# iden3/snarkjs

Hardware: NVIDIA B200
Metric: groth16_proofs_per_sec (higher is better)
Workload: dtype u32x8 (256-bit modular integers, 32-bit limbs)

## Files before the change

profiles/tune_pair.py:

```python
import os, sys
sys.path.insert(0, os.path.dirname(os.path.dirname(os.path.abspath(__file__))))
import numpy as np
import snarkjs_b200
from snarkjs_b200 import synth
c = snarkjs_b200.getCurveFromName("bn128")
lib, h = c.lib, c.handle
n = 1 << 20
rng = np.random.default_rng(1)
sc = rng.integers(0, 256, size=n * 32, dtype=np.uint8); sc.reshape(n, 32)[:, 31] &= 0x1f
for grp in (1, 2):
    bases = synth.gen_points(c, grp, 7, n)
    G = c.G1 if grp == 1 else c.G2
    hb = G.registerBases(bases)
    ref = None
    for off, rounds in ((1, 0), (0, 1), (0, 2), (0, 3), (0, 4), (0, 6)):
        lib.sb_set_tuning(4, off); lib.sb_set_tuning(5, rounds)
        for _ in range(3):
            out = G.multiExpRegistered(hb, sc)
        if ref is None: ref = out.tobytes()
        assert out.tobytes() == ref
        print(f"G{grp} pairing {'off' if off else 'R<=%d' % rounds}: pre-stage {lib.sb_last_stat(h, grp - 1):.3f} ms, msm device total {c.last_ms(2):.3f} ms")
```

snarkjs_b200/csrc/api.cu:

```cuda
#include <cstdio>
#include <cstdlib>
#include <cstring>
#include <string>
#include <vector>
#include <map>
#include <algorithm>
#include <mutex>
#include <future>
#include <thread>
#include <dlfcn.h>
#include <nccl.h>
#include <fcntl.h>
#include <unistd.h>
#include <sys/mman.h>
#include <sys/stat.h>
#include "../../include/snarkb200.h"
#include "ec.cuh"
#include "msm.cuh"
#include "msm_entry.h"
#include "fr_entry.h"

using namespace sb;
namespace sb { double calibrate(int what, cudaStream_t stream); extern int g_ntt_tile_log; }

namespace {

struct DevBuf {
    void* p = nullptr; size_t cap = 0;
    void* get(size_t bytes) {
        if (bytes > cap) { if (p) cudaFree(p); p = nullptr; cap = 0; if (cudaMalloc(&p, bytes ? bytes : 16) != cudaSuccess) return nullptr; cap = bytes; }
        return p;
    }
    void release() { if (p) cudaFree(p); p = nullptr; cap = 0; }
};

struct GroupOps {
    int (*buckets)(const void*, const MsmSorted&, MsmScratch&, cudaStream_t, void*, MsmLaunchStats*, cudaStream_t, cudaEvent_t);
    void (*combine)(const uint8_t*, const MsmGeom&, uint8_t*);
    void (*add)(uint8_t*, const uint8_t*);
    void (*to_jacobian)(const uint8_t*, uint8_t*);
    void (*to_affine)(const uint8_t*, uint8_t*);
    void (*from_affine)(const uint8_t*, uint8_t*);
    void (*times)(const uint8_t*, const uint8_t*, int, uint8_t*);
    int (*gen_points)(const uint8_t*, uint64_t, uint64_t, void*, cudaStream_t);
    int (*precompute)(const void*, uint64_t, int, int, void*, cudaStream_t);
    uint32_t xyzz_bytes;
    uint32_t aff_bytes;
};
#define SB_GROUP_OPS(NAME, AFF) GroupOps{NAME##_buckets, NAME##_combine, NAME##_add, NAME##_to_jacobian, NAME##_to_affine, NAME##_from_affine, NAME##_times, NAME##_gen_points, NAME##_precompute, NAME##_xyzz_bytes(), AFF}

struct NttTab { DevBuf lo, hi; int h = 0; };
struct PreTab { DevBuf lo, hi; int h = 0; std::string key; };

struct BaseSet { int group = 0; uint64_t n = 0; void* d = nullptr; void* table = nullptr; MsmGeom gp{}; };

struct Groth16Key {
    uint32_t nVars = 0, nPublic = 0, domainSize = 0; int power = 0;
    std::vector<uint8_t> alpha1, beta1, beta2, gamma2, delta1, delta2;
    void *dA = nullptr, *dB1 = nullptr, *dB2 = nullptr, *dC = nullptr, *dH = nullptr;
    void *tA = nullptr, *tB1 = nullptr, *tB2 = nullptr, *tC = nullptr, *tH = nullptr;
    MsmGeom gpW{}, gpH{};
    int shard = 0, n_shards = 1; uint64_t wlo = 0, wcnt = 0, hlo = 0, hcnt = 0;
    uint64_t* d_rowptr = nullptr; uint32_t* d_sig = nullptr; void* d_coef = nullptr; uint64_t nCoef = 0;
    bool witness_resident = false;
    void *dW = nullptr, *dA_T = nullptr, *dB_T = nullptr, *dC_T = nullptr, *dTmp = nullptr, *dTmp2 = nullptr, *dTmp3 = nullptr, *dWsum = nullptr;
};

}

namespace { struct PlonkKeyDev; void plonk_free_key(PlonkKeyDev*); }
namespace { struct FflonkKeyDev; void fflonk_free_key(FflonkKeyDev*); }

static constexpr size_t STAGE_BYTES = 8u << 20;

struct sb_ctx {
    std::recursive_mutex mu;
    int curve = 0, device = 0;
    cudaStream_t stream = nullptr;
    std::string err;
    uint32_t n8q = 32;
    GroupOps g1, g2;
    MsmScratch sort_scratch, bucket_scratch;
    MsmScratch sort_scratch2, bscr[5];
    cudaStream_t aux[6] = {nullptr, nullptr, nullptr, nullptr, nullptr, nullptr};
    cudaEvent_t pev[16];
    uint8_t* pinned = nullptr;
    uint8_t* stage[2] = {nullptr, nullptr};
    cudaEvent_t stage_ev[2];
    MsmLaunchStats stats;
    uint64_t launches = 0;
    DevBuf io[4];
    std::map<int, NttTab> ntt_fwd, ntt_inv;
    DevBuf wr_fwd, wr_inv;
    std::map<int, DevBuf> ninv;
    std::vector<PreTab*> pre_cache;
    std::vector<BaseSet> bases;
    std::vector<Groth16Key*> keys;
    std::vector<PlonkKeyDev*> plonk_keys;
    std::vector<FflonkKeyDev*> fflonk_keys;
    cudaEvent_t ev[8];
    float last_ms[8] = {0};
    int fr_s = 0, fr_bits = 254;
    std::vector<std::vector<uint8_t>> roots;
    std::vector<uint8_t> nqr, shift;
    std::vector<uint8_t> gen1, gen2;
    cudaEvent_t prof_ev[256];
    double stat[16] = {0};
    ncclComm_t comm = nullptr; int rank = 0, world = 1;
    void* d_xchg = nullptr; uint8_t* h_xchg = nullptr;
};

namespace {

thread_local const sb_ctx* t_err_ctx = nullptr;
thread_local std::string t_err;
int fail(sb_ctx* c, int code, const std::string& msg) { if (c) { c->err = msg; t_err_ctx = c; t_err = msg; } return code; }
#define SB_LOCK(c) std::unique_lock<std::recursive_mutex> _sb_lk; if (c) _sb_lk = std::unique_lock<std::recursive_mutex>((c)->mu)
int cuda_fail(sb_ctx* c, cudaError_t e, const char* where) {
    return fail(c, e == cudaErrorMemoryAllocation ? SB_ERR_NOMEM : SB_ERR_CUDA, std::string(where) + ": " + cudaGetErrorString(e));
}
#define CU(c, call) do { cudaError_t _e = (call); if (_e != cudaSuccess) return cuda_fail(c, _e, #call); } while (0)

int g_stage_enabled = 1;
bool host_is_pinned(const void* p) {
    cudaPointerAttributes a;
    if (cudaPointerGetAttributes(&a, p) != cudaSuccess) { cudaGetLastError(); return false; }
    return a.type == cudaMemoryTypeHost;
}
cudaError_t h2d(sb_ctx* c, void* dst, const void* src, size_t bytes) {
    if (!bytes) return cudaSuccess;
    if (!g_stage_enabled || bytes < (1u << 20) || !c->stage[0] || !c->stage[1] || host_is_pinned(src))
        return cudaMemcpyAsync(dst, src, bytes, cudaMemcpyHostToDevice, c->stream);
    size_t off = 0; int k = 0; cudaError_t e = cudaSuccess;
    while (off < bytes && e == cudaSuccess) {
        const int b = k & 1; const size_t n = std::min(STAGE_BYTES, bytes - off);
        if (k >= 2) e = cudaEventSynchronize(c->stage_ev[b]);
        if (e != cudaSuccess) break;
        memcpy(c->stage[b], (const uint8_t*)src + off, n);
        e = cudaMemcpyAsync((uint8_t*)dst + off, c->stage[b], n, cudaMemcpyHostToDevice, c->stream);
        if (e == cudaSuccess) e = cudaEventRecord(c->stage_ev[b], c->stream);
        off += n; k++;
    }
    if (e == cudaSuccess) e = cudaEventSynchronize(c->stage_ev[0]);
    if (e == cudaSuccess && k > 1) e = cudaEventSynchronize(c->stage_ev[1]);
    return e;
}
cudaError_t d2h(sb_ctx* c, void* dst, const void* src, size_t bytes) {
    if (!bytes) return cudaSuccess;
    if (!g_stage_enabled || bytes < (1u << 20) || !c->stage[0] || !c->stage[1] || host_is_pinned(dst)) {
        cudaError_t e = cudaMemcpyAsync(dst, src, bytes, cudaMemcpyDeviceToHost, c->stream);
        return e == cudaSuccess ? cudaStreamSynchronize(c->stream) : e;
    }
    size_t off = 0, prev_off = 0, prev_n = 0; int k = 0; cudaError_t e = cudaSuccess;
    while (off < bytes && e == cudaSuccess) {
        const int b = k & 1; const size_t n = std::min(STAGE_BYTES, bytes - off);
        e = cudaMemcpyAsync(c->stage[b], (const uint8_t*)src + off, n, cudaMemcpyDeviceToHost, c->stream);
        if (e == cudaSuccess) e = cudaEventRecord(c->stage_ev[b], c->stream);
        if (e == cudaSuccess && k >= 1) { e = cudaEventSynchronize(c->stage_ev[b ^ 1]); if (e == cudaSuccess) memcpy((uint8_t*)dst + prev_off, c->stage[b ^ 1], prev_n); }
        prev_off = off; prev_n = n; off += n; k++;
    }
    if (e == cudaSuccess && k >= 1) { const int b = (k - 1) & 1; e = cudaEventSynchronize(c->stage_ev[b]); if (e == cudaSuccess) memcpy((uint8_t*)dst + prev_off, c->stage[b], prev_n); }
    return e;
}

template <class P> struct HostFr {
    typedef Fp<P> F;
    static F from_u32(uint32_t x) { F a = F::zero(); a.v[0] = x; return F::to_mont(a); }
    static void roots(int& s, std::vector<F>& w, F& nqr, F& shift) {
        const int N = P::N;
        uint32_t pm1[N]; for (int i = 0; i < N; i++) pm1[i] = P::p(i); pm1[0] -= 1;
        uint32_t half[N]; for (int i = 0; i < N; i++) half[i] = (pm1[i] >> 1) | (i + 1 < N ? pm1[i + 1] << 31 : 0);
        F negone = F::neg(F::one());
        nqr = from_u32(2);
        while (!(F::pow(nqr, half, N) == negone)) nqr = F::add(nqr, F::one());
        shift = F::sqr(nqr);
        uint32_t t[N]; memcpy(t, pm1, sizeof t); s = 0;
        while (!(t[0] & 1)) { for (int i = 0; i < N; i++) t[i] = (t[i] >> 1) | (i + 1 < N ? t[i + 1] << 31 : 0); s++; }
        w.assign(s + 1, F::zero());
        w[s] = F::pow(nqr, t, N);
        for (int i = s - 1; i >= 0; i--) w[i] = F::sqr(w[i + 1]);
    }
    static void pow_tables(const F& base, const F& scale, int h, uint64_t nhi, std::vector<F>& lo, std::vector<F>& hi) {
        lo.resize((size_t)1 << h); hi.resize(nhi ? nhi : 1);
        F t = F::one();
        for (size_t e = 0; e < lo.size(); e++) { lo[e] = t; t = F::mul(t, base); }
        F step = t;
        t = scale;
        for (size_t e = 0; e < hi.size(); e++) { hi[e] = t; t = F::mul(t, step); }
    }
};

template <class P> int init_roots(sb_ctx* c) {
    typedef Fp<P> F;
    std::vector<F> w; F nqr, shift; int s;
    HostFr<P>::roots(s, w, nqr, shift);
    c->fr_s = s;
    c->roots.resize(s + 1);
    for (int i = 0; i <= s; i++) c->roots[i].assign((uint8_t*)&w[i], (uint8_t*)&w[i] + 32);
    c->nqr.assign((uint8_t*)&nqr, (uint8_t*)&nqr + 32);
    c->shift.assign((uint8_t*)&shift, (uint8_t*)&shift + 32);
    F wd = w[NTT_DMAX], wdi = F::inv(wd);
    std::vector<F> lo, hi;
    HostFr<P>::pow_tables(wd, F::one(), NTT_DMAX - 1, 1, lo, hi);
    if (!c->wr_fwd.get(lo.size() * 32)) return SB_ERR_NOMEM;
    cudaMemcpy(c->wr_fwd.p, lo.data(), lo.size() * 32, cudaMemcpyHostToDevice);
    HostFr<P>::pow_tables(wdi, F::one(), NTT_DMAX - 1, 1, lo, hi);
    if (!c->wr_inv.get(lo.size() * 32)) return SB_ERR_NOMEM;
    cudaMemcpy(c->wr_inv.p, lo.data(), lo.size() * 32, cudaMemcpyHostToDevice);
    return 0;
}

template <class P> int build_ntt_tab(sb_ctx* c, int L, bool inverse, NttTab& tab) {
    typedef Fp<P> F;
    F w; memcpy(&w, c->roots[L].data(), 32);
    if (inverse) w = F::inv(w);
    int h = (L + 1) / 2;
    std::vector<F> lo, hi;
    HostFr<P>::pow_tables(w, F::one(), h, (uint64_t)1 << (L - h), lo, hi);
    tab.h = h;
    if (!tab.lo.get(lo.size() * 32) || !tab.hi.get(hi.size() * 32)) return SB_ERR_NOMEM;
    cudaMemcpy(tab.lo.p, lo.data(), lo.size() * 32, cudaMemcpyHostToDevice);
    cudaMemcpy(tab.hi.p, hi.data(), hi.size() * 32, cudaMemcpyHostToDevice);
    return 0;
}

int get_ntt_tab(sb_ctx* c, int L, bool inverse, FrNttTables* out) {
    auto& m = inverse ? c->ntt_inv : c->ntt_fwd;
    auto it = m.find(L);
    if (it == m.end()) {
        NttTab& t = m[L];
        int rc = c->curve == SB_BN254 ? build_ntt_tab<BnFr>(c, L, inverse, t) : build_ntt_tab<BlsFr>(c, L, inverse, t);
        if (rc) { m.erase(L); return fail(c, rc, "ntt table allocation failed"); }
        it = m.find(L);
    }
    out->tw_lo = it->second.lo.p; out->tw_hi = it->second.hi.p; out->h = it->second.h;
    out->wr = inverse ? c->wr_inv.p : c->wr_fwd.p;
    return 0;
}

template <class P> void ninv_bytes(int L, uint8_t* out) {
    typedef Fp<P> F;
    F two = F::add(F::one(), F::one()), n = F::one();
    for (int i = 0; i < L; i++) n = F::mul(n, two);
    F r = F::inv(n); memcpy(out, &r, 32);
}
const void* get_ninv(sb_ctx* c, int L) {
    auto it = c->ninv.find(L);
    if (it == c->ninv.end()) {
        uint8_t b[32];
        if (c->curve == SB_BN254) ninv_bytes<BnFr>(L, b); else ninv_bytes<BlsFr>(L, b);
        DevBuf& d = c->ninv[L];
        if (!d.get(32)) return nullptr;
        cudaMemcpy(d.p, b, 32, cudaMemcpyHostToDevice);
        it = c->ninv.find(L);
    }
    return it->second.p;
}

template <class P> int build_pre(sb_ctx* c, uint64_t n, const uint8_t* first, const uint8_t* inc, PreTab& t) {
    typedef Fp<P> F;
    int bits = 0; while (((uint64_t)1 << bits) < n) bits++;
    int h = (bits + 1) / 2;
    F f, i; memcpy(&f, first, 32); memcpy(&i, inc, 32);
    std::vector<F> lo, hi;
    HostFr<P>::pow_tables(i, f, h, (n + ((uint64_t)1 << h) - 1) >> h, lo, hi);
    t.h = h;
    if (!t.lo.get(lo.size() * 32) || !t.hi.get(hi.size() * 32)) return SB_ERR_NOMEM;
    cudaMemcpy(t.lo.p, lo.data(), lo.size() * 32, cudaMemcpyHostToDevice);
    cudaMemcpy(t.hi.p, hi.data(), hi.size() * 32, cudaMemcpyHostToDevice);
    return 0;
}
int get_pre(sb_ctx* c, uint64_t n, const uint8_t* first, const uint8_t* inc, FrPre* out) {
    std::string key((const char*)&n, 8); key.append((const char*)first, 32); key.append((const char*)inc, 32);
    for (PreTab* t : c->pre_cache) if (t->key == key) { out->lo = t->lo.p; out->hi = t->hi.p; out->h = t->h; return 0; }
    PreTab* t = new PreTab(); t->key = key;
    int rc = c->curve == SB_BN254 ? build_pre<BnFr>(c, n, first, inc, *t) : build_pre<BlsFr>(c, n, first, inc, *t);
    if (rc) { delete t; return fail(c, rc, "apply-key table allocation failed"); }
    if (c->pre_cache.size() >= 16) { delete c->pre_cache.front(); c->pre_cache.erase(c->pre_cache.begin()); }
    c->pre_cache.push_back(t);
    out->lo = t->lo.p; out->hi = t->hi.p; out->h = t->h;
    return 0;
}

template <class P> void hex_to_mont(const char* hex, uint8_t* out) {
    typedef Fp<P> F; F a = F::zero();
    int len = (int)strlen(hex);
    for (int i = 0; i < len; i++) {
        char ch = hex[len - 1 - i];
        uint32_t d = (ch >= '0' && ch <= '9') ? ch - '0' : (ch >= 'a' && ch <= 'f') ? ch - 'a' + 10 : ch - 'A' + 10;
        a.v[i / 8] |= d << (4 * (i % 8));
    }
    a = F::to_mont(a); memcpy(out, &a, sizeof a);
}
void init_generators(sb_ctx* c) {
    if (c->curve == SB_BN254) {
        c->gen1.resize(64); c->gen2.resize(128);
        hex_to_mont<BnFq>("1", c->gen1.data()); hex_to_mont<BnFq>("2", c->gen1.data() + 32);
        hex_to_mont<BnFq>("1800deef121f1e76426a00665e5c4479674322d4f75edadd46debd5cd992f6ed", c->gen2.data());
        hex_to_mont<BnFq>("198e9393920d483a7260bfb731fb5d25f1aa493335a9e71297e485b7aef312c2", c->gen2.data() + 32);
        hex_to_mont<BnFq>("12c85ea5db8c6deb4aab71808dcb408fe3d1e7690c43d37b4ce6cc0166fa7daa", c->gen2.data() + 64);
        hex_to_mont<BnFq>("090689d0585ff075ec9e99ad690c3395bc4b313370b38ef355acdadcd122975b", c->gen2.data() + 96);
    } else {
        c->gen1.resize(96); c->gen2.resize(192);
        hex_to_mont<BlsFq>("17f1d3a73197d7942695638c4fa9ac0fc3688c4f9774b905a14e3a3f171bac586c55e83ff97a1aeffb3af00adb22c6bb", c->gen1.data());
        hex_to_mont<BlsFq>("08b3f481e3aaa0f1a09e30ed741d8ae4fcf5e095d5d00af600db18cb2c04b3edd03cc744a2888ae40caa232946c5e7e1", c->gen1.data() + 48);
        hex_to_mont<BlsFq>("024aa2b2f08f0a91260805272dc51051c6e47ad4fa403b02b4510b647ae3d1770bac0326a805bbefd48056c8c121bdb8", c->gen2.data());
        hex_to_mont<BlsFq>("13e02b6052719f607dacd3a088274f65596bd0d09920b61ab5da61bbdc7f5049334cf11213945d57e5ac7d055d042b7e", c->gen2.data() + 48);
        hex_to_mont<BlsFq>("0ce5d527727d6e118cc9cdc6da2e351aadfd9baa8cbdd3a76d429a695160d12c923ac9cc3baca289e193548608b82801", c->gen2.data() + 96);
        hex_to_mont<BlsFq>("0606c4a02ea734cc32acd2b02bc28b99cb3e287e85a763af267492ab572e99ab3f370d275cec1da1aaa9075ff05f79be", c->gen2.data() + 144);
    }
}

void prof_begin(sb_ctx* c) { c->stats.ev = c->prof_ev; c->stats.nev = 256; c->stats.used = 0; for (double& d : c->stat) d = 0; }
void prof_end(sb_ctx* c) {
    for (int i = 0; i + 1 < c->stats.used; i += 2) {
        float ms = 0; if (cudaEventElapsedTime(&ms, c->prof_ev[i], c->prof_ev[i + 1]) != cudaSuccess) { cudaGetLastError(); continue; }
        const int g = c->stats.tag[i / 2];
        if (g == PROF_ACC_G1) { c->stat[0] += ms; c->stat[2] += 1; c->stat[9] += ms; }
        else if (g == PROF_ACC_G2) { c->stat[1] += ms; c->stat[3] += 1; c->stat[10] += ms; }
        else if (g == PROF_SORT) c->stat[8] += ms;
        else if (g >= PROF_FOLD && g <= PROF_JOIN) c->stat[11 + (g - PROF_FOLD)] += ms;
    }
    c->stats.ev = nullptr; c->stats.used = 0;
}

bool want_precomp(sb_ctx* c, uint64_t n) {
    if (g_msm_tuning[3] != 0 || n < (1ull << 12)) return false;
    MsmGeom g = msm_geometry_precomp(n, 32, c->fr_bits);
    return (uint64_t)g.W * n < (1ull << 31);
}
int build_table(sb_ctx* c, const GroupOps& G, const void* d_bases, uint64_t n, void** table, MsmGeom* gp) {
    MsmGeom g = msm_geometry_precomp(n, 32, c->fr_bits);
    cudaError_t e = cudaMalloc(table, (size_t)g.W * n * G.aff_bytes);
    if (e != cudaSuccess) { *table = nullptr; return cuda_fail(c, e, "precompute table allocation"); }
    int rc = G.precompute(d_bases, n, g.c, g.W, *table, c->stream); c->launches++;
    if (rc) return cuda_fail(c, (cudaError_t)rc, "k_precompute");
    e = cudaStreamSynchronize(c->stream);
    if (e != cudaSuccess) return cuda_fail(c, e, "k_precompute");
    *gp = g;
    return 0;
}

void tick(sb_ctx* c, int i) { cudaEventRecord(c->ev[i], c->stream); }
float elapsed(sb_ctx* c, int a, int b) { float ms = 0; cudaEventElapsedTime(&ms, c->ev[a], c->ev[b]); return ms; }

int msm_dev_accumulate(sb_ctx* c, const GroupOps& G, const void* d_bases, const uint8_t* d_scalars, uint32_t sbytes, uint64_t n,
                       uint8_t* acc_xyzz, const MsmGeom* gp = nullptr, uint64_t first = 0) {
    const uint64_t MAXC = 1ull << (g_msm_tuning[6] > 0 ? g_msm_tuning[6] : 23);
    for (uint64_t off = 0; off < n; off += MAXC) {
        uint64_t cn = std::min(MAXC, n - off);
        MsmGeom g = msm_geometry(cn, sbytes, c->fr_bits);
        if (gp) {
            g = *gp; g.first = first + off; g.W = (int)((8 * sbytes + 1 + g.c - 1) / g.c);
        }
        MsmSorted s;
        int rc = msm_sort_entries(d_scalars + off * sbytes, sbytes, cn, g, c->sort_scratch, c->stream, &s, &c->stats);
        if (rc) return cuda_fail(c, (cudaError_t)rc, "msm_sort_entries");
        void* d_wsum = c->io[3].get((size_t)g.wsum_points() * G.xyzz_bytes);
        if (!d_wsum) return fail(c, SB_ERR_NOMEM, "out of device memory");
        c->stats.cur_tag = (&G == &c->g1) ? SB_G1 : SB_G2;
        rc = G.buckets(gp ? d_bases : (const void*)((const uint8_t*)d_bases + off * G.aff_bytes), s, c->bucket_scratch, c->stream, d_wsum, &c->stats, nullptr, nullptr);
        if (rc) return cuda_fail(c, (cudaError_t)rc, "msm_buckets");
        std::vector<uint8_t> ws((size_t)g.wsum_points() * G.xyzz_bytes);
        uint64_t entries = 0;
        CU(c, cudaMemcpyAsync(ws.data(), d_wsum, ws.size(), cudaMemcpyDeviceToHost, c->stream));
        CU(c, cudaMemcpyAsync(&entries, s.counts, 8, cudaMemcpyDeviceToHost, c->stream));
        CU(c, cudaStreamSynchronize(c->stream));
        c->stat[(&G == &c->g1) ? 4 : 5] += (double)entries;
        G.combine(ws.data(), g, acc_xyzz);
    }
    return 0;
}

int msm_host_inputs(sb_ctx* c, int group, const uint8_t* bases, const void* d_bases_opt, const uint8_t* scalars, uint32_t sbytes,
                    uint64_t n, uint8_t* out_jac, uint8_t* out_partial, const MsmGeom* gp = nullptr, uint64_t first = 0) {
    if (!c) return SB_ERR_ARG;
    const GroupOps& G = group == SB_G1 ? c->g1 : c->g2;
    std::vector<uint8_t> acc(G.xyzz_bytes, 0);
    if (n) {
        if (sbytes == 0 || sbytes > 64) return fail(c, SB_ERR_ARG, "Scalar size does not match");
        cudaSetDevice(c->device);
        tick(c, 0);
        const void* d_bases = d_bases_opt;
        if (!d_bases) {
            void* p = c->io[0].get(n * G.aff_bytes);
            if (!p) return fail(c, SB_ERR_NOMEM, "out of device memory");
            CU(c, h2d(c, p, bases, n * G.aff_bytes));
            d_bases = p;
        }
        uint8_t* d_sc = (uint8_t*)c->io[1].get(n * sbytes);
        if (!d_sc) return fail(c, SB_ERR_NOMEM, "out of device memory");
        CU(c, h2d(c, d_sc, scalars, n * sbytes));
        tick(c, 1);
        prof_begin(c);
        int rc = msm_dev_accumulate(c, G, d_bases, d_sc, sbytes, n, acc.data(), gp, first);
        if (rc) return rc;
        tick(c, 2);
        cudaEventSynchronize(c->ev[2]);
        prof_end(c);
        c->last_ms[0] = elapsed(c, 0, 2); c->last_ms[1] = elapsed(c, 0, 1); c->last_ms[2] = elapsed(c, 1, 2);
    }
    if (out_partial) memcpy(out_partial, acc.data(), acc.size());
    if (out_jac) G.to_jacobian(acc.data(), out_jac);
    return 0;
}

struct Section { uint64_t pos = 0, len = 0; bool present = false; };
int parse_binfile(sb_ctx* c, const uint8_t* d, uint64_t len, const char* magic, uint32_t max_version, std::map<uint32_t, Section>& secs) {
    if (len < 12 || memcmp(d, magic, 4) != 0) return fail(c, SB_ERR_FORMAT, std::string(magic) + ": Invalid File format");
    uint32_t ver, nsec; memcpy(&ver, d + 4, 4); memcpy(&nsec, d + 8, 4);
    if (ver > max_version) return fail(c, SB_ERR_FORMAT, "Version not supported");
    uint64_t pos = 12;
    for (uint32_t i = 0; i < nsec; i++) {
        if (len - pos < 12) return fail(c, SB_ERR_FORMAT, "Invalid file size");
        uint32_t id; uint64_t sl; memcpy(&id, d + pos, 4); memcpy(&sl, d + pos + 4, 8); pos += 12;
        if (sl > len - pos) return fail(c, SB_ERR_FORMAT, "Invalid file size");
        if (secs[id].present) return fail(c, SB_ERR_FORMAT, "Section Duplicated " + std::to_string(id));
        secs[id].pos = pos; secs[id].len = sl; secs[id].present = true;
        pos += sl;
    }
    if (pos != len) return fail(c, SB_ERR_FORMAT, "Invalid file size");
    return 0;
}

bool modulus_matches(const uint8_t* p, uint32_t n8, int curve, bool scalar_field) {
    uint32_t limbs[12] = {0};
    if (curve == SB_BN254) { if (n8 != 32) return false; for (int i = 0; i < 8; i++) limbs[i] = scalar_field ? BnFr::p(i) : BnFq::p(i); }
    else if (scalar_field) { if (n8 != 32) return false; for (int i = 0; i < 8; i++) limbs[i] = BlsFr::p(i); }
    else { if (n8 != 48) return false; for (int i = 0; i < 12; i++) limbs[i] = BlsFq::p(i); }
    return memcmp(p, limbs, n8) == 0;
}

void free_key(Groth16Key* k) {
    for (void* p : {k->tA, k->tB1, k->tB2, k->tC, k->tH, k->dA, k->dB1, k->dB2, k->dC, k->dH, (void*)k->d_rowptr, (void*)k->d_sig, k->d_coef, k->dW, k->dA_T, k->dB_T, k->dC_T, k->dTmp, k->dTmp2, k->dTmp3, k->dWsum})
        if (p) cudaFree(p);
    delete k;
}

template <class PR> static void fr_from_mont_bytes(const uint8_t* in, uint8_t* out) { Fp<PR> a; memcpy(&a, in, 32); a = Fp<PR>::from_mont(a); memcpy(out, &a, 32); }
template <class PR> static void fr_neg_mul_bytes(const uint8_t* r, const uint8_t* s, uint8_t* out) { Fp<PR> a, b; memcpy(&a, r, 32); memcpy(&b, s, 32); a = Fp<PR>::neg(Fp<PR>::mul(a, b)); memcpy(out, &a, 32); }

}

extern "C" {

const char* sb_version(void) { return "snarkb200 0.2 (sm_100a)"; }
int sb_comm_destroy(sb_ctx* c);

int sb_create(int curve, int device_id, sb_ctx** out) {
    if (!out || (curve != SB_BN254 && curve != SB_BLS12_381)) return SB_ERR_ARG;
    int ndev = 0;
    if (cudaGetDeviceCount(&ndev) != cudaSuccess || ndev == 0) return SB_ERR_NODEVICE;
    if (device_id < 0 || device_id >= ndev) return SB_ERR_ARG;
    if (cudaSetDevice(device_id) != cudaSuccess) return SB_ERR_CUDA;
    sb_ctx* c = new sb_ctx();
    c->curve = curve; c->device = device_id;
    c->n8q = curve == SB_BN254 ? 32 : 48;
    c->fr_bits = curve == SB_BN254 ? 254 : 255;
    if (curve == SB_BN254) { c->g1 = SB_GROUP_OPS(bn254_g1, 64); c->g2 = SB_GROUP_OPS(bn254_g2, 128); }
    else { c->g1 = SB_GROUP_OPS(bls12381_g1, 96); c->g2 = SB_GROUP_OPS(bls12381_g2, 192); }
    if (cudaStreamCreate(&c->stream) != cudaSuccess) { delete c; return SB_ERR_CUDA; }
    for (auto& e : c->ev) cudaEventCreate(&e);
    for (auto& e : c->prof_ev) cudaEventCreate(&e);
    for (auto& e : c->pev) cudaEventCreateWithFlags(&e, cudaEventDisableTiming);
    { int lo = 0, hi = 0; cudaDeviceGetStreamPriorityRange(&lo, &hi);
      for (auto& st : c->aux) cudaStreamCreateWithPriority(&st, cudaStreamDefault, hi); }
    if (cudaHostAlloc((void**)&c->pinned, 256 * 1024, cudaHostAllocDefault) != cudaSuccess) c->pinned = nullptr;
    for (int i = 0; i < 2; i++) { if (cudaHostAlloc((void**)&c->stage[i], STAGE_BYTES, cudaHostAllocDefault) != cudaSuccess) c->stage[i] = nullptr; cudaEventCreateWithFlags(&c->stage_ev[i], cudaEventDisableTiming); }
    init_generators(c);
    int rc = curve == SB_BN254 ? init_roots<BnFr>(c) : init_roots<BlsFr>(c);
    if (rc == 0 && fr_configure(curve) != 0) rc = SB_ERR_CUDA;
    if (rc) { sb_destroy(c); return rc; }
    *out = c;
    return SB_OK;
}

void sb_destroy(sb_ctx* c) {
    if (!c) return;
    sb_comm_destroy(c);
    cudaSetDevice(c->device);
    cudaStreamSynchronize(c->stream);
    for (auto* k : c->keys) if (k) free_key(k);
    for (auto* k : c->plonk_keys) if (k) plonk_free_key(k);
    for (auto* k : c->fflonk_keys) if (k) fflonk_free_key(k);
    for (auto& b : c->bases) { if (b.d) cudaFree(b.d); if (b.table) cudaFree(b.table); }
    for (auto* t : c->pre_cache) { t->lo.release(); t->hi.release(); delete t; }
    for (auto& kv : c->ntt_fwd) { kv.second.lo.release(); kv.second.hi.release(); }
    for (auto& kv : c->ntt_inv) { kv.second.lo.release(); kv.second.hi.release(); }
    for (auto& kv : c->ninv) kv.second.release();
    c->wr_fwd.release(); c->wr_inv.release();
    for (auto& b : c->io) b.release();
    c->sort_scratch.release(); c->bucket_scratch.release();
    for (auto& e : c->ev) cudaEventDestroy(e);
    for (auto& e : c->prof_ev) cudaEventDestroy(e);
    for (auto& e : c->pev) cudaEventDestroy(e);
    for (auto& st : c->aux) { if (st) { cudaStreamSynchronize(st); cudaStreamDestroy(st); } }
    if (c->pinned) cudaFreeHost(c->pinned);
    for (int i = 0; i < 2; i++) { if (c->stage[i]) cudaFreeHost(c->stage[i]); cudaEventDestroy(c->stage_ev[i]); }
    c->sort_scratch2.release(); for (auto& b : c->bscr) b.release();
    cudaStreamDestroy(c->stream);
    delete c;
}

const char* sb_last_error(sb_ctx* c) {
    if (!c) return "null context";
    if (t_err_ctx == c) return t_err.c_str();
    SB_LOCK(c); t_err_ctx = c; t_err = c->err; return t_err.c_str();
}
uint64_t sb_launch_count(sb_ctx* c) { SB_LOCK(c); return c ? c->launches + (uint64_t)c->stats.launches : 0; }
float sb_last_ms(sb_ctx* c, int which) { SB_LOCK(c); return (c && which >= 0 && which < 8) ? c->last_ms[which] : 0.f; }
int sb_sync(sb_ctx* c) { SB_LOCK(c); if (!c) return SB_ERR_ARG; cudaSetDevice(c->device); CU(c, cudaStreamSynchronize(c->stream)); return 0; }

int sb_msm_g1_affine(sb_ctx* c, const uint8_t* bases, const uint8_t* scalars, uint32_t sb, uint64_t n, uint8_t* out) { SB_LOCK(c);
    return msm_host_inputs(c, SB_G1, bases, nullptr, scalars, sb, n, out, nullptr);
}
int sb_msm_g2_affine(sb_ctx* c, const uint8_t* bases, const uint8_t* scalars, uint32_t sb, uint64_t n, uint8_t* out) { SB_LOCK(c);
    return msm_host_inputs(c, SB_G2, bases, nullptr, scalars, sb, n, out, nullptr);
}

int sb_bases_register(sb_ctx* c, int group, const uint8_t* bases, uint64_t n, uint64_t* handle) { SB_LOCK(c);
    if (!c || !handle || (group != SB_G1 && group != SB_G2)) return SB_ERR_ARG;
    cudaSetDevice(c->device);
    const GroupOps& G = group == SB_G1 ? c->g1 : c->g2;
    BaseSet b; b.group = group; b.n = n;
    CU(c, cudaMalloc(&b.d, n ? n * G.aff_bytes : 16));
    CU(c, cudaMemcpy(b.d, bases, n * G.aff_bytes, cudaMemcpyHostToDevice));
    if (want_precomp(c, n)) { int rc = build_table(c, G, b.d, n, &b.table, &b.gp); if (rc) { cudaFree(b.d); return rc; } }
    c->bases.push_back(b);
    *handle = c->bases.size();
    return 0;
}
int sb_bases_release(sb_ctx* c, uint64_t h) { SB_LOCK(c);
    if (!c || h == 0 || h > c->bases.size() || !c->bases[h - 1].d) return fail(c, SB_ERR_ARG, "invalid bases handle");
    cudaSetDevice(c->device);
    cudaFree(c->bases[h - 1].d); c->bases[h - 1].d = nullptr; c->bases[h - 1].n = 0;
    if (c->bases[h - 1].table) { cudaFree(c->bases[h - 1].table); c->bases[h - 1].table = nullptr; }
    return 0;
}
static int msm_registered_impl(sb_ctx* c, uint64_t h, uint64_t first, const uint8_t* scalars, uint32_t sb, uint64_t n, uint8_t* out, uint8_t* partial) {
    if (!c || h == 0 || h > c->bases.size() || !c->bases[h - 1].d) return fail(c, SB_ERR_ARG, "invalid bases handle");
    const BaseSet& b = c->bases[h - 1];
    if (first + n > b.n) return fail(c, SB_ERR_ARG, "registered base range out of bounds");
    const GroupOps& G = b.group == SB_G1 ? c->g1 : c->g2;
    if (b.table && sb >= 1 && sb <= 32)
        return msm_host_inputs(c, b.group, nullptr, b.table, scalars, sb, n, out, partial, &b.gp, first);
    return msm_host_inputs(c, b.group, nullptr, (const uint8_t*)b.d + first * G.aff_bytes, scalars, sb, n, out, partial);
}
int sb_msm_registered(sb_ctx* c, uint64_t h, uint64_t first, const uint8_t* scalars, uint32_t sb, uint64_t n, uint8_t* out) { SB_LOCK(c);
    return msm_registered_impl(c, h, first, scalars, sb, n, out, nullptr);
}
int sb_msm_registered_partial(sb_ctx* c, uint64_t h, uint64_t first, const uint8_t* scalars, uint32_t sb, uint64_t n, uint8_t* partial) { SB_LOCK(c);
    return msm_registered_impl(c, h, first, scalars, sb, n, nullptr, partial);
}
uint32_t sb_msm_partial_bytes(sb_ctx* c, int group) { return c ? (group == SB_G1 ? c->g1.xyzz_bytes : c->g2.xyzz_bytes) : 0; }
int sb_msm_sum_partials(sb_ctx* c, int group, const uint8_t* partials, int count, uint8_t* out) { SB_LOCK(c);
    if (!c || (group != SB_G1 && group != SB_G2) || count < 0) return SB_ERR_ARG;
    const GroupOps& G = group == SB_G1 ? c->g1 : c->g2;
    std::vector<uint8_t> acc(G.xyzz_bytes, 0);
    for (int i = 0; i < count; i++) G.add(acc.data(), partials + (size_t)i * G.xyzz_bytes);
    G.to_jacobian(acc.data(), out);
    return 0;
}

int sb_msm_dev(sb_ctx* c, int group, const void* bases_dev, const void* scalars_dev, uint32_t sb, uint64_t n, uint8_t* out) { SB_LOCK(c);
    if (!c || (group != SB_G1 && group != SB_G2)) return SB_ERR_ARG;
    cudaSetDevice(c->device);
    const GroupOps& G = group == SB_G1 ? c->g1 : c->g2;
    std::vector<uint8_t> acc(G.xyzz_bytes, 0);
    tick(c, 0);
    prof_begin(c);
    if (n) { int rc = msm_dev_accumulate(c, G, bases_dev, (const uint8_t*)scalars_dev, sb, n, acc.data()); if (rc) return rc; }
    tick(c, 1); cudaEventSynchronize(c->ev[1]); c->last_ms[0] = elapsed(c, 0, 1);
    prof_end(c);
    G.to_jacobian(acc.data(), out);
    return 0;
}

static int ntt_dev(sb_ctx* c, void* a, void* b, uint64_t n, int inverse, const FrPre* pre, bool scale, void** result) {
    if (n == 0 || (n & (n - 1))) return fail(c, SB_ERR_ARG, "fft must be multiple of 2");
    int L = 0; while (((uint64_t)1 << L) < n) L++;
    if (L > c->fr_s) return fail(c, SB_ERR_ARG, "fft size exceeds the 2-adicity of Fr (fftExt path not supported)");
    if (L == 0) { *result = a; return 0; }
    FrNttTables tb;
    int rc = get_ntt_tab(c, L, inverse != 0, &tb); if (rc) return rc;
    const void* post = nullptr;
    if (inverse && scale) { post = get_ninv(c, L); if (!post) return fail(c, SB_ERR_NOMEM, "out of device memory"); }
    int launches = 0;
    ProfScope pn(&c->stats, PROF_NTT, c->stream);
    rc = fr_ntt(c->curve, a, b, L, &tb, pre, post, c->stream, result, &launches);
    pn.end();
    c->launches += launches;
    if (rc) return cuda_fail(c, (cudaError_t)rc, "fr_ntt");
    return 0;
}

int sb_ntt_fr(sb_ctx* c, const uint8_t* in, uint64_t n, int inverse, uint8_t* out) { SB_LOCK(c);
    if (!c) return SB_ERR_ARG;
    if (n == 0 || (n & (n - 1))) return fail(c, SB_ERR_ARG, "fft must be multiple of 2");
    cudaSetDevice(c->device);
    void* a = c->io[0].get(n * 32); void* b = c->io[1].get(n * 32);
    if (!a || !b) return fail(c, SB_ERR_NOMEM, "out of device memory");
    tick(c, 0);
    CU(c, h2d(c, a, in, n * 32));
    tick(c, 1);
    void* res = nullptr;
    int rc = ntt_dev(c, a, b, n, inverse, nullptr, true, &res); if (rc) return rc;
    tick(c, 2);
    CU(c, d2h(c, out, res, n * 32));
    tick(c, 3);
    CU(c, cudaStreamSynchronize(c->stream));
    c->last_ms[0] = elapsed(c, 0, 3); c->last_ms[1] = elapsed(c, 0, 1); c->last_ms[2] = elapsed(c, 1, 2); c->last_ms[3] = elapsed(c, 2, 3);
    return 0;
}
int sb_ntt_fr_dev(sb_ctx* c, void* data, void* scratch, uint64_t n, int inverse, void** result) { SB_LOCK(c);
    if (!c || !result) return SB_ERR_ARG;
    cudaSetDevice(c->device);
    tick(c, 0);
    int rc = ntt_dev(c, data, scratch, n, inverse, nullptr, true, result); if (rc) return rc;
    tick(c, 1);
    CU(c, cudaStreamSynchronize(c->stream));
    c->last_ms[0] = elapsed(c, 0, 1);
    return 0;
}

int sb_fr_batch_apply_key(sb_ctx* c, const uint8_t* in, uint64_t n, const uint8_t first[32], const uint8_t inc[32], uint8_t* out) { SB_LOCK(c);
    if (!c) return SB_ERR_ARG;
    if (n == 0) return 0;
    cudaSetDevice(c->device);
    FrPre pre; int rc = get_pre(c, n, first, inc, &pre); if (rc) return rc;
    void* a = c->io[0].get(n * 32); void* b = c->io[1].get(n * 32);
    if (!a || !b) return fail(c, SB_ERR_NOMEM, "out of device memory");
    CU(c, h2d(c, a, in, n * 32));
    rc = fr_apply_key(c->curve, a, b, n, &pre, c->stream); c->launches++;
    if (rc) return cuda_fail(c, (cudaError_t)rc, "fr_apply_key");
    CU(c, d2h(c, out, b, n * 32));
    return 0;
}
static int convert_impl(sb_ctx* c, const uint8_t* in, uint64_t n, uint8_t* out, int to_mont) {
    if (!c) return SB_ERR_ARG;
    if (n == 0) return 0;
    cudaSetDevice(c->device);
    void* a = c->io[0].get(n * 32); void* b = c->io[1].get(n * 32);
    if (!a || !b) return fail(c, SB_ERR_NOMEM, "out of device memory");
    CU(c, h2d(c, a, in, n * 32));
    int rc = fr_convert(c->curve, a, b, n, to_mont, c->stream); c->launches++;
    if (rc) return cuda_fail(c, (cudaError_t)rc, "fr_convert");
    CU(c, d2h(c, out, b, n * 32));
    return 0;
}
int sb_fr_batch_to_montgomery(sb_ctx* c, const uint8_t* in, uint64_t n, uint8_t* out) { SB_LOCK(c); return convert_impl(c, in, n, out, 1); }
int sb_fr_batch_from_montgomery(sb_ctx* c, const uint8_t* in, uint64_t n, uint8_t* out) { SB_LOCK(c); return convert_impl(c, in, n, out, 0); }

int sb_qap_join_abc(sb_ctx* c, const uint8_t* a, const uint8_t* b, const uint8_t* cc, uint64_t n, uint8_t* out) { SB_LOCK(c);
    if (!c) return SB_ERR_ARG;
    if (n == 0) return 0;
    cudaSetDevice(c->device);
    void* da = c->io[0].get(n * 32); void* db = c->io[1].get(n * 32); void* dc = c->io[2].get(n * 32); void* dout = c->io[3].get(n * 32);
    if (!da || !db || !dc || !dout) return fail(c, SB_ERR_NOMEM, "out of device memory");
    CU(c, h2d(c, da, a, n * 32));
    CU(c, h2d(c, db, b, n * 32));
    CU(c, h2d(c, dc, cc, n * 32));
    int rc = fr_join_abc(c->curve, da, db, dc, dout, n, c->stream); c->launches++;
    if (rc) return cuda_fail(c, (cudaError_t)rc, "fr_join_abc");
    CU(c, d2h(c, out, dout, n * 32));
    return 0;
}

int sb_fr_root(sb_ctx* c, int what, uint8_t out[32]) { SB_LOCK(c);
    if (!c) return SB_ERR_ARG;
    if (what == -1) memcpy(out, c->shift.data(), 32);
    else if (what == -2) memcpy(out, c->nqr.data(), 32);
    else if (what >= 0 && what <= c->fr_s) memcpy(out, c->roots[what].data(), 32);
    else return fail(c, SB_ERR_ARG, "root index out of range");
    return c->fr_s;
}

int sb_set_tuning(int key, int value) {
    if (key == 8) { g_stage_enabled = value; return 0; }
    if (key == 7) { if (value < 10 || value > 12) return SB_ERR_ARG; g_ntt_tile_log = value; return 0; }
    if (key == 9) { g_msm_tuning[7] = value; return 0; }
    if (key == 12) { g_msm_tuning[10] = value; return 0; }
    if (key == 11) { g_msm_tuning[9] = value; return 0; }
    if (key == 10) { g_msm_tuning[8] = value; return 0; }
    if (key < 0 || key >= 7) return SB_ERR_ARG; g_msm_tuning[key] = value; return 0;
}
double sb_last_stat(sb_ctx* c, int which) { SB_LOCK(c); return (c && which >= 0 && which < 16) ? c->stat[which] : 0.0; }
double sb_calibrate(sb_ctx* c, int what) { SB_LOCK(c); if (!c) return -1; cudaSetDevice(c->device); return calibrate(what, c->stream); }
int sb_gen_points(sb_ctx* c, int group, uint64_t seed, uint64_t n, uint8_t* out) { SB_LOCK(c);
    if (!c || (group != SB_G1 && group != SB_G2)) return SB_ERR_ARG;
    cudaSetDevice(c->device);
    const GroupOps& G = group == SB_G1 ? c->g1 : c->g2;
    void* d = c->io[0].get(n * G.aff_bytes);
    if (!d) return fail(c, SB_ERR_NOMEM, "out of device memory");
    int rc = G.gen_points(group == SB_G1 ? c->gen1.data() : c->gen2.data(), seed, n, d, c->stream); c->launches++;
    if (rc) return cuda_fail(c, (cudaError_t)rc, "gen_points");
    CU(c, d2h(c, out, d, n * G.aff_bytes));
    return 0;
}
int sb_generator(sb_ctx* c, int group, uint8_t* out) { SB_LOCK(c);
    if (!c || (group != SB_G1 && group != SB_G2)) return SB_ERR_ARG;
    const std::vector<uint8_t>& g = group == SB_G1 ? c->gen1 : c->gen2;
    memcpy(out, g.data(), g.size()); return 0;
}

void* sb_dev_alloc(sb_ctx* c, uint64_t bytes) { SB_LOCK(c); if (!c) return nullptr; cudaSetDevice(c->device); void* p = nullptr; if (cudaMalloc(&p, bytes ? bytes : 16) != cudaSuccess) return nullptr; return p; }
int sb_dev_free(sb_ctx* c, void* p) { SB_LOCK(c); if (!c) return SB_ERR_ARG; cudaSetDevice(c->device); CU(c, cudaFree(p)); return 0; }
int sb_dev_upload(sb_ctx* c, void* dst, const uint8_t* src, uint64_t bytes) { SB_LOCK(c); if (!c) return SB_ERR_ARG; cudaSetDevice(c->device); CU(c, h2d(c, dst, src, bytes)); CU(c, cudaStreamSynchronize(c->stream)); return 0; }
int sb_dev_download(sb_ctx* c, uint8_t* dst, const void* src, uint64_t bytes) { SB_LOCK(c); if (!c) return SB_ERR_ARG; cudaSetDevice(c->device); CU(c, d2h(c, dst, src, bytes)); return 0; }

struct ZkeySource {
    const uint8_t* z = nullptr; uint64_t zlen = 0; FILE* f = nullptr;
    std::vector<uint8_t> small[5];
};
static int zkey_section_table(sb_ctx* c, ZkeySource& src, std::map<uint32_t, Section>& secs) {
    if (src.z) return parse_binfile(c, src.z, src.zlen, "zkey", 2, secs);
    uint8_t hd[12];
    if (fseek(src.f, 0, SEEK_END)) return fail(c, SB_ERR_FORMAT, "zkey: seek failed");
    const uint64_t flen = (uint64_t)ftell(src.f);
    fseek(src.f, 0, SEEK_SET);
    if (fread(hd, 1, 12, src.f) != 12 || memcmp(hd, "zkey", 4) != 0) return fail(c, SB_ERR_FORMAT, "zkey: Invalid File format");
    uint32_t ver, nsec; memcpy(&ver, hd + 4, 4); memcpy(&nsec, hd + 8, 4);
    if (ver > 2) return fail(c, SB_ERR_FORMAT, "Version not supported");
    uint64_t pos = 12;
    for (uint32_t i = 0; i < nsec; i++) {
        if (fseek(src.f, (long)pos, SEEK_SET) || fread(hd, 1, 12, src.f) != 12) return fail(c, SB_ERR_FORMAT, "Invalid file size");
        uint32_t id; uint64_t sl; memcpy(&id, hd, 4); memcpy(&sl, hd + 4, 8); pos += 12;
        if (pos > flen || sl > flen - pos) return fail(c, SB_ERR_FORMAT, "Invalid file size");
        if (secs[id].present) return fail(c, SB_ERR_FORMAT, "Section Duplicated " + std::to_string(id));
        secs[id].pos = pos; secs[id].len = sl; secs[id].present = true; pos += sl;
    }
    if (pos != flen) return fail(c, SB_ERR_FORMAT, "Invalid file size");
    return 0;
}
static const uint8_t* zkey_host_section(ZkeySource& src, const std::map<uint32_t, Section>& secs, uint32_t id, int slot) {
    const Section& s = secs.at(id);
    if (src.z) return src.z + s.pos;
    src.small[slot].resize(s.len ? s.len : 1);
    if (fseek(src.f, (long)s.pos, SEEK_SET) || fread(src.small[slot].data(), 1, s.len, src.f) != s.len) return nullptr;
    return src.small[slot].data();
}
static cudaError_t zkey_to_device(sb_ctx* c, ZkeySource& src, const std::map<uint32_t, Section>& secs, uint32_t id, uint64_t off, uint64_t len, void* dst) {
    if (!len) return cudaSuccess;
    const Section& s = secs.at(id);
    if (src.z) return cudaMemcpy(dst, src.z + s.pos + off, len, cudaMemcpyHostToDevice);
    const size_t CH = 16u << 20;
    uint8_t* pin[2] = {nullptr, nullptr}; cudaEvent_t ev[2];
    cudaError_t e = cudaHostAlloc((void**)&pin[0], CH, cudaHostAllocDefault); if (e != cudaSuccess) return e;
    e = cudaHostAlloc((void**)&pin[1], CH, cudaHostAllocDefault); if (e != cudaSuccess) { cudaFreeHost(pin[0]); return e; }
    cudaEventCreateWithFlags(&ev[0], cudaEventDisableTiming); cudaEventCreateWithFlags(&ev[1], cudaEventDisableTiming);
    if (fseek(src.f, (long)(s.pos + off), SEEK_SET)) e = cudaErrorUnknown;
    uint64_t done = 0; int b = 0; bool used[2] = {false, false};
    while (e == cudaSuccess && done < len) {
        const size_t n = (size_t)std::min<uint64_t>(CH, len - done);
        if (used[b]) e = cudaEventSynchronize(ev[b]);
        if (e == cudaSuccess && fread(pin[b], 1, n, src.f) != n) e = cudaErrorUnknown;
        if (e == cudaSuccess) e = cudaMemcpyAsync((uint8_t*)dst + done, pin[b], n, cudaMemcpyHostToDevice, c->stream);
        if (e == cudaSuccess) { cudaEventRecord(ev[b], c->stream); used[b] = true; }
        done += n; b ^= 1;
    }
    cudaStreamSynchronize(c->stream);
    cudaEventDestroy(ev[0]); cudaEventDestroy(ev[1]); cudaFreeHost(pin[0]); cudaFreeHost(pin[1]);
    return e;
}

static int groth16_load_impl(sb_ctx* c, ZkeySource& src, int shard, int n_shards, uint64_t* handle) {
    if (!c || (!src.z && !src.f) || !handle || n_shards < 1 || shard < 0 || shard >= n_shards) return SB_ERR_ARG;
    cudaSetDevice(c->device);
    std::map<uint32_t, Section> secs;
    int rc = zkey_section_table(c, src, secs); if (rc) return rc;
    for (uint32_t id : {1u, 2u, 4u, 5u, 6u, 7u, 8u, 9u}) if (!secs[id].present) return fail(c, SB_ERR_FORMAT, "Missing section " + std::to_string(id));
    const uint8_t* s1 = zkey_host_section(src, secs, 1, 0);
    if (!s1 || secs[1].len < 4) return fail(c, SB_ERR_FORMAT, "zkey: short read");
    uint32_t proto; memcpy(&proto, s1, 4);
    if (proto != 1) return fail(c, SB_ERR_FORMAT, "zkey file is not groth16");
    const uint8_t* h = zkey_host_section(src, secs, 2, 1); uint64_t hl = secs[2].len;
    if (!h) return fail(c, SB_ERR_FORMAT, "zkey: short read");
    const uint32_t n8q = c->n8q, n8r = 32;
    const uint64_t need = 4 + n8q + 4 + n8r + 12 + 3 * 2 * n8q + 3 * 4 * n8q;
    if (hl < need) return fail(c, SB_ERR_FORMAT, "zkey header too short");
    uint32_t v; memcpy(&v, h, 4);
    if (v != n8q || !modulus_matches(h + 4, n8q, c->curve, false)) return fail(c, SB_ERR_FORMAT, "zkey curve does not match the context curve");
    memcpy(&v, h + 4 + n8q, 4);
    if (v != n8r || !modulus_matches(h + 8 + n8q, n8r, c->curve, true)) return fail(c, SB_ERR_FORMAT, "zkey curve does not match the context curve");
    Groth16Key* k = new Groth16Key();
    const uint8_t* q = h + 8 + n8q + n8r;
    memcpy(&k->nVars, q, 4); memcpy(&k->nPublic, q + 4, 4); memcpy(&k->domainSize, q + 8, 4); q += 12;
    const uint32_t sG1 = 2 * n8q, sG2 = 4 * n8q;
    k->alpha1.assign(q, q + sG1); q += sG1; k->beta1.assign(q, q + sG1); q += sG1;
    k->beta2.assign(q, q + sG2); q += sG2; k->gamma2.assign(q, q + sG2); q += sG2;
    k->delta1.assign(q, q + sG1); q += sG1; k->delta2.assign(q, q + sG2);
    const uint64_t n = k->domainSize, nv = k->nVars;
    if (n == 0 || (n & (n - 1))) { delete k; return fail(c, SB_ERR_FORMAT, "domain size is not a power of two"); }
    while (((uint64_t)1 << k->power) < n) k->power++;
    if (k->power > c->fr_s) { delete k; return fail(c, SB_ERR_FORMAT, "Circuit too big for this curve"); }
    if (nv < (uint64_t)k->nPublic + 1) { delete k; return fail(c, SB_ERR_FORMAT, "invalid zkey header"); }
    if (secs[5].len != nv * sG1 || secs[6].len != nv * sG1 || secs[7].len != nv * sG2 ||
        secs[8].len != (nv - k->nPublic - 1) * sG1 || secs[9].len != n * sG1) { delete k; return fail(c, SB_ERR_FORMAT, "zkey section size mismatch"); }
    const uint8_t* s4 = zkey_host_section(src, secs, 4, 2);
    if (!s4 || secs[4].len < 4) { delete k; return fail(c, SB_ERR_FORMAT, "zkey: short read"); }
    uint32_t ncoef; memcpy(&ncoef, s4, 4);
    const uint64_t sCoef = 12 + n8r;
    if (secs[4].len != 4 + ncoef * sCoef) { delete k; return fail(c, SB_ERR_FORMAT, "zkey coefficient section size mismatch"); }
    const uint8_t* cf = s4 + 4;
    std::vector<uint64_t> rowptr(2 * n + 1, 0);
    for (uint64_t i = 0; i < ncoef; i++) {
        uint32_t m, cc, s; memcpy(&m, cf + i * sCoef, 4); memcpy(&cc, cf + i * sCoef + 4, 4); memcpy(&s, cf + i * sCoef + 8, 4);
        if (m > 1 || cc >= n || s >= nv) { delete k; return fail(c, SB_ERR_FORMAT, "zkey coefficient out of range"); }
        rowptr[m * n + cc + 1]++;
    }
    for (uint64_t i = 0; i < 2 * n; i++) rowptr[i + 1] += rowptr[i];
    std::vector<uint64_t> cursor(rowptr.begin(), rowptr.end() - 1);
    std::vector<uint32_t> sig(ncoef ? ncoef : 1); std::vector<uint8_t> coef((size_t)(ncoef ? ncoef : 1) * 32);
    for (uint64_t i = 0; i < ncoef; i++) {
        uint32_t m, cc, s; memcpy(&m, cf + i * sCoef, 4); memcpy(&cc, cf + i * sCoef + 4, 4); memcpy(&s, cf + i * sCoef + 8, 4);
        uint64_t p = cursor[m * n + cc]++;
        sig[p] = s; memcpy(&coef[p * 32], cf + i * sCoef + 12, 32);
    }
    k->nCoef = ncoef;
    cudaError_t e = cudaSuccess;
    auto up = [&](void** d, const void* src, size_t bytes, size_t alloc) {
        if (e != cudaSuccess) return;
        e = cudaMalloc(d, alloc ? alloc : 16); if (e != cudaSuccess) return;
        if (bytes) e = cudaMemcpy(*d, src, bytes, cudaMemcpyHostToDevice);
    };
    k->shard = shard; k->n_shards = n_shards;
    sb_shard_range(nv, shard, n_shards, &k->wlo, &k->wcnt);
    sb_shard_range(n, shard, n_shards, &k->hlo, &k->hcnt);
    const uint64_t wlo = k->wlo, wcnt = k->wcnt, hlo = k->hlo, hcnt = k->hcnt;
    auto upsec = [&](void** d, uint32_t id, uint64_t off, uint64_t len) {
        if (e != cudaSuccess) return;
        e = cudaMalloc(d, len ? len : 16); if (e != cudaSuccess) return;
        e = zkey_to_device(c, src, secs, id, off, len, *d);
    };
    upsec(&k->dA, 5, wlo * sG1, wcnt * sG1);
    upsec(&k->dB1, 6, wlo * sG1, wcnt * sG1);
    upsec(&k->dB2, 7, wlo * sG2, wcnt * sG2);
    if (e == cudaSuccess) {
        const uint64_t np1 = (uint64_t)k->nPublic + 1;
        e = cudaMalloc(&k->dC, wcnt ? wcnt * sG1 : 16);
        if (e == cudaSuccess && wcnt) e = cudaMemset(k->dC, 0, wcnt * sG1);
        const uint64_t g0 = std::max(wlo, np1), g1 = wlo + wcnt;
        if (e == cudaSuccess && g1 > g0) e = zkey_to_device(c, src, secs, 8, (g0 - np1) * sG1, (g1 - g0) * sG1, (uint8_t*)k->dC + (g0 - wlo) * sG1);
    }
    upsec(&k->dH, 9, hlo * sG1, hcnt * sG1);
    up((void**)&k->d_rowptr, rowptr.data(), rowptr.size() * 8, rowptr.size() * 8);
    up((void**)&k->d_sig, sig.data(), (size_t)ncoef * 4, (size_t)ncoef * 4);
    up(&k->d_coef, coef.data(), (size_t)ncoef * 32, (size_t)ncoef * 32);
    up(&k->dW, nullptr, 0, (nv + 64) * 32);
    up(&k->dA_T, nullptr, 0, n * 32); up(&k->dB_T, nullptr, 0, n * 32); up(&k->dC_T, nullptr, 0, n * 32); up(&k->dTmp, nullptr, 0, n * 32);
    up(&k->dTmp2, nullptr, 0, n * 32); up(&k->dTmp3, nullptr, 0, n * 32);
    up(&k->dWsum, nullptr, 0, 8 * 80 * 4 * 96);
    if (e != cudaSuccess) { free_key(k); return cuda_fail(c, e, "sb_groth16_load upload"); }
    if (want_precomp(c, wcnt) && want_precomp(c, hcnt)) {
        int rc2 = build_table(c, c->g1, k->dA, wcnt, &k->tA, &k->gpW);
        if (!rc2) rc2 = build_table(c, c->g1, k->dB1, wcnt, &k->tB1, &k->gpW);
        if (!rc2) rc2 = build_table(c, c->g2, k->dB2, wcnt, &k->tB2, &k->gpW);
        if (!rc2) rc2 = build_table(c, c->g1, k->dC, wcnt, &k->tC, &k->gpW);
        if (!rc2) rc2 = build_table(c, c->g1, k->dH, hcnt, &k->tH, &k->gpH);
        if (rc2) { free_key(k); return rc2; }
    }
    c->keys.push_back(k);
    *handle = c->keys.size();
    return 0;
}

int sb_groth16_load(sb_ctx* c, const uint8_t* z, uint64_t zlen, uint64_t* handle) { SB_LOCK(c);
    if (!z) return SB_ERR_ARG;
    ZkeySource src; src.z = z; src.zlen = zlen; return groth16_load_impl(c, src, 0, 1, handle);
}
int sb_groth16_load_sharded(sb_ctx* c, const uint8_t* z, uint64_t zlen, int shard, int n_shards, uint64_t* handle) { SB_LOCK(c);
    if (!z) return SB_ERR_ARG;
    ZkeySource src; src.z = z; src.zlen = zlen; return groth16_load_impl(c, src, shard, n_shards, handle);
}

int sb_groth16_load_file(sb_ctx* c, const char* path, uint64_t* handle) { SB_LOCK(c);
    if (!c || !path) return SB_ERR_ARG;
    cudaSetDevice(c->device);
    FILE* f = fopen(path, "rb");
    if (!f) return fail(c, SB_ERR_FORMAT, std::string("cannot open ") + path);
    ZkeySource src; src.f = f;
    int rc = groth16_load_impl(c, src, 0, 1, handle);
    fclose(f);
    return rc;
}

static Groth16Key* get_key(sb_ctx* c, uint64_t h) { return (c && h >= 1 && h <= c->keys.size()) ? c->keys[h - 1] : nullptr; }

int sb_groth16_info(sb_ctx* c, uint64_t h, uint32_t* nv, uint32_t* np, uint32_t* ds) { SB_LOCK(c);
    Groth16Key* k = get_key(c, h); if (!k) return fail(c, SB_ERR_ARG, "invalid groth16 handle");
    if (nv) *nv = k->nVars; if (np) *np = k->nPublic; if (ds) *ds = k->domainSize;
    return 0;
}
int sb_groth16_release(sb_ctx* c, uint64_t h) { SB_LOCK(c);
    Groth16Key* k = get_key(c, h); if (!k) return fail(c, SB_ERR_ARG, "invalid groth16 handle");
    cudaSetDevice(c->device); free_key(k); c->keys[h - 1] = nullptr; return 0;
}
uint32_t sb_groth16_partials_bytes(sb_ctx* c) { return c ? 4 * c->g1.xyzz_bytes + c->g2.xyzz_bytes : 0; }

struct NcclApi {
    void* so = nullptr;
    ncclResult_t (*GetUniqueId)(ncclUniqueId*) = nullptr;
    ncclResult_t (*CommInitRank)(ncclComm_t*, int, ncclUniqueId, int) = nullptr;
    ncclResult_t (*CommDestroy)(ncclComm_t) = nullptr;
    ncclResult_t (*AllGather)(const void*, void*, size_t, ncclDataType_t, ncclComm_t, cudaStream_t) = nullptr;
    ncclResult_t (*Send)(const void*, size_t, ncclDataType_t, int, ncclComm_t, cudaStream_t) = nullptr;
    ncclResult_t (*Recv)(void*, size_t, ncclDataType_t, int, ncclComm_t, cudaStream_t) = nullptr;
    ncclResult_t (*GroupStart)() = nullptr;
    ncclResult_t (*GroupEnd)() = nullptr;
    const char* (*GetErrorString)(ncclResult_t) = nullptr;
};
static NcclApi* nccl_api(std::string* why) {
    static std::mutex mu; static NcclApi api; static bool tried = false; static std::string err;
    std::lock_guard<std::mutex> lk(mu);
    if (!tried) {
        tried = true;
        const char* env = getenv("SB_NCCL_LIB");
        void* so = env ? dlopen(env, RTLD_NOW | RTLD_LOCAL) : nullptr;
        if (!so) so = dlopen("libnccl.so.2", RTLD_NOW | RTLD_NOLOAD);
        if (!so) so = dlopen("libnccl.so.2", RTLD_NOW | RTLD_LOCAL);
        if (!so) so = dlopen("libnccl.so", RTLD_NOW | RTLD_LOCAL);
        if (!so) err = std::string("cannot load libnccl.so.2: ") + dlerror();
        else {
            api.so = so;
            bool ok = true;
            auto sym = [&](const char* n) { void* p = dlsym(so, n); if (!p) { ok = false; err = std::string("libnccl: missing symbol ") + n; } return p; };
            api.GetUniqueId = (decltype(api.GetUniqueId))sym("ncclGetUniqueId");
            api.CommInitRank = (decltype(api.CommInitRank))sym("ncclCommInitRank");
            api.CommDestroy = (decltype(api.CommDestroy))sym("ncclCommDestroy");
            api.AllGather = (decltype(api.AllGather))sym("ncclAllGather");
            api.Send = (decltype(api.Send))sym("ncclSend");
            api.Recv = (decltype(api.Recv))sym("ncclRecv");
            api.GroupStart = (decltype(api.GroupStart))sym("ncclGroupStart");
            api.GroupEnd = (decltype(api.GroupEnd))sym("ncclGroupEnd");
            api.GetErrorString = (decltype(api.GetErrorString))sym("ncclGetErrorString");
            if (!ok) api.so = nullptr;
        }
    }
    if (!api.so) { if (why) *why = err; return nullptr; }
    return &api;
}
#define NC(c, api, call) do { ncclResult_t _r = (call); if (_r != ncclSuccess) return fail(c, SB_ERR_CUDA, std::string(#call) + ": " + (api)->GetErrorString(_r)); } while (0)

int sb_comm_unique_id(uint8_t out[128]) {
    static_assert(sizeof(ncclUniqueId) == 128, "ncclUniqueId is 128 bytes");
    if (!out) return SB_ERR_ARG;
    NcclApi* nc = nccl_api(nullptr); if (!nc) return SB_ERR_CUDA;
    ncclUniqueId id; if (nc->GetUniqueId(&id) != ncclSuccess) return SB_ERR_CUDA;
    memcpy(out, &id, 128); return 0;
}
int sb_comm_init_rank(sb_ctx* c, int world, int rank, const uint8_t id_bytes[128]) { SB_LOCK(c);
    if (!c || !id_bytes || world < 1 || world > 64 || rank < 0 || rank >= world) return fail(c, SB_ERR_ARG, "invalid communicator arguments");
    if (c->comm) return fail(c, SB_ERR_ARG, "context already belongs to a communicator");
    std::string why; NcclApi* nc = nccl_api(&why); if (!nc) return fail(c, SB_ERR_CUDA, why);
    cudaSetDevice(c->device);
    ncclUniqueId id; memcpy(&id, id_bytes, 128);
    NC(c, nc, nc->CommInitRank(&c->comm, world, id, rank));
    c->rank = rank; c->world = world;
    const size_t pb = (size_t)sb_groth16_partials_bytes(c);
    CU(c, cudaMalloc(&c->d_xchg, pb * world));
    CU(c, cudaHostAlloc((void**)&c->h_xchg, pb * (world + 1), cudaHostAllocDefault));
    return 0;
}
int sb_comm_info(sb_ctx* c, int* rank, int* world) { SB_LOCK(c);
    if (!c) return SB_ERR_ARG;
    if (rank) *rank = c->rank; if (world) *world = c->comm ? c->world : 0;
    return 0;
}
int sb_comm_destroy(sb_ctx* c) { SB_LOCK(c);
    if (!c) return SB_ERR_ARG;
    if (c->comm) {
        cudaSetDevice(c->device); cudaStreamSynchronize(c->stream);
        if (NcclApi* nc = nccl_api(nullptr)) nc->CommDestroy(c->comm);
        c->comm = nullptr; c->rank = 0; c->world = 1;
        if (c->d_xchg) cudaFree(c->d_xchg); if (c->h_xchg) cudaFreeHost(c->h_xchg);
        c->d_xchg = nullptr; c->h_xchg = nullptr;
    }
    return 0;
}
int sb_dist_chain_owner(int chain, int world) { return world > 0 ? chain % world : 0; }

struct ProofScalars { uint8_t rp[32], sp[32]; };

static int groth16_device(sb_ctx* c, Groth16Key* k, const uint8_t* witness, uint64_t n_witness, int shard, int n_shards, uint8_t* partials,
                          const ProofScalars* ps = nullptr, bool dist = false) {
    if (witness && n_witness != k->nVars) return fail(c, SB_ERR_ARG, "Invalid witness length. Circuit: " + std::to_string(k->nVars) + ", witness: " + std::to_string(n_witness));
    cudaSetDevice(c->device);
    const uint64_t n = k->domainSize, nv = k->nVars;
    const int cv = c->curve;
    NcclApi* nc = nullptr;
    if (dist) {
        if (!c->comm) return fail(c, SB_ERR_ARG, "context has no communicator: call sb_comm_init_rank first");
        nc = nccl_api(nullptr);
        shard = c->rank; n_shards = c->world;
    }
    const int world = n_shards, rank = shard;
    int rc;
    tick(c, 0);
    if (witness) {
        k->witness_resident = false;
        if (dist && world > 1) {
            const uint64_t per = (nv + world - 1) / world, lo = std::min(nv, per * (uint64_t)rank), cnt = std::min(nv - lo, per);
            CU(c, h2d(c, (uint8_t*)k->dW + lo * 32, witness + lo * 32, cnt * 32));
            NC(c, nc, nc->AllGather((const uint8_t*)k->dW + per * rank * 32, k->dW, per * 32, ncclUint8, c->comm, c->stream));
        } else CU(c, h2d(c, k->dW, witness, nv * 32));
        k->witness_resident = true;
    } else if (!k->witness_resident) return fail(c, SB_ERR_ARG, "no witness resident for this proving key: call sb_groth16_prove first");
    tick(c, 1);
    prof_begin(c);
    auto range_of = [&](uint64_t total, int sh, uint64_t& lo, uint64_t& cnt) { sb_shard_range(total, sh, n_shards, &lo, &cnt); };
    uint64_t wlo, wcnt; range_of(nv, rank, wlo, wcnt);
    uint64_t hlo, hcnt; range_of(n, rank, hlo, hcnt);
    auto owner = [&](int j) { return (dist && world > 1) ? sb_dist_chain_owner(j, world) : rank; };
    void* bufs[3] = {k->dA_T, k->dB_T, k->dC_T}; void* scr[3] = {k->dTmp, k->dTmp2, k->dTmp3};
    const int np = fr_ntt_passes(k->power);
    void* odd[3]; void* tmp;
    { const bool x_scr = (np & 1) != 0;
      for (int j = 0; j < 3; j++) { void* X = x_scr ? scr[j] : bufs[j]; void* Y = x_scr ? bufs[j] : scr[j]; odd[j] = (np & 1) ? Y : X; }
      tmp = (odd[0] == bufs[0]) ? scr[0] : bufs[0]; }
    auto run_qap_ntt = [&]() -> int {
        int my[3], m = 0;
        for (int j = 0; j < 3; j++) if (owner(j) == rank) my[m++] = j;
        if (m) {
            { ProfScope pq(&c->stats, PROF_QAP, c->stream);
              rc = fr_qap_rows(cv, k->d_rowptr, k->d_sig, k->d_coef, k->dW, k->dA_T, k->dB_T, k->dC_T, n, c->stream); c->launches++;
              pq.end(); }
            if (rc) return cuda_fail(c, (cudaError_t)rc, "fr_qap_rows");
            const uint8_t* inc = (k->power == c->fr_s) ? c->shift.data() : c->roots[k->power + 1].data();
            uint8_t ninv[32];
            if (cv == SB_BN254) ninv_bytes<BnFr>(k->power, ninv); else ninv_bytes<BlsFr>(k->power, ninv);
            FrPre pre; rc = get_pre(c, n, ninv, inc, &pre); if (rc) return rc;
            void* a[3]; void* b[3];
            for (int i = 0; i < m; i++) { a[i] = bufs[my[i]]; b[i] = scr[my[i]]; }
            FrNttTables tbi, tbf;
            rc = get_ntt_tab(c, k->power, true, &tbi); if (rc) return rc;
            rc = get_ntt_tab(c, k->power, false, &tbf); if (rc) return rc;
            int side = 0, launches = 0;
            ProfScope pn(&c->stats, PROF_NTT, c->stream);
            rc = fr_ntt_batch(cv, a, b, m, k->power, &tbi, nullptr, nullptr, c->stream, &side, &launches);
            if (rc) return cuda_fail(c, (cudaError_t)rc, "fr_ntt_batch");
            void** src = side ? b : a; void** dst = side ? a : b;
            int side2 = 0;
            rc = fr_ntt_batch(cv, src, dst, m, k->power, &tbf, &pre, nullptr, c->stream, &side2, &launches);
            if (rc) return cuda_fail(c, (cudaError_t)rc, "fr_ntt_batch");
            pn.end();
            c->launches += launches;
            void** res = side2 ? dst : src;
            for (int i = 0; i < m; i++) if (res[i] != odd[my[i]]) return fail(c, SB_ERR_CUDA, "internal: NTT result buffer mismatch");
        }
        if (dist && world > 1) {
            NC(c, nc, nc->GroupStart());
            for (int j = 0; j < 3; j++) {
                const int o = owner(j);
                if (o == rank) {
                    for (int q = 0; q < world; q++) {
                        if (q == rank) continue;
                        uint64_t qlo, qcnt; range_of(n, q, qlo, qcnt);
                        if (qcnt) NC(c, nc, nc->Send((const uint8_t*)odd[j] + qlo * 32, qcnt * 32, ncclUint8, q, c->comm, c->stream));
                    }
                } else if (hcnt) NC(c, nc, nc->Recv((uint8_t*)odd[j] + hlo * 32, hcnt * 32, ncclUint8, o, c->comm, c->stream));
            }
            NC(c, nc, nc->GroupEnd());
        }
        if (hcnt) {
            ProfScope pj(&c->stats, PROF_JOIN, c->stream);
            rc = fr_join_abc(cv, (const uint8_t*)odd[0] + hlo * 32, (const uint8_t*)odd[1] + hlo * 32, (const uint8_t*)odd[2] + hlo * 32,
                             (uint8_t*)tmp + hlo * 32, hcnt, c->stream); c->launches++;
            pj.end();
            if (rc) return cuda_fail(c, (cudaError_t)rc, "fr_join_abc");
        }
        return 0;
    };
    const GroupOps& G1 = c->g1; const GroupOps& G2 = c->g2;
    uint8_t* pA = partials; uint8_t* pB1 = pA + G1.xyzz_bytes; uint8_t* pC = pB1 + G1.xyzz_bytes; uint8_t* pH = pC + G1.xyzz_bytes; uint8_t* pB2 = pH + G1.xyzz_bytes;
    memset(partials, 0, 4 * G1.xyzz_bytes + G2.xyzz_bytes);
    std::vector<uint8_t> sA(G1.xyzz_bytes, 0), rB1(G1.xyzz_bytes, 0);
    const uint64_t MAXC = 1ull << (g_msm_tuning[6] > 0 ? g_msm_tuning[6] : 23);
    const bool local = k->n_shards > 1;
    if (local && (shard != k->shard || n_shards != k->n_shards)) return fail(c, SB_ERR_ARG, "proving key was loaded for a different shard");
    const uint64_t wb = local ? 0 : wlo, hb = local ? 0 : hlo;
    const bool overlapped = wcnt <= MAXC && hcnt <= MAXC && wcnt > 0 && hcnt > 0 && c->pinned;
    if (dist && world > 1 && !overlapped) return fail(c, SB_ERR_ARG, "distributed proving needs at least one point per rank and shards of at most 2^23 points");
    if (overlapped) {
        const bool serial = g_msm_tuning[2] != 0;
        cudaStream_t s0 = c->stream;
        cudaStream_t sN = serial ? s0 : c->aux[5];
        MsmGeom gw = msm_geometry(wcnt, 32, c->fr_bits), gh = msm_geometry(hcnt, 32, c->fr_bits);
        const bool pre = k->tA != nullptr;
        if (pre) { gw = k->gpW; gw.first = wb; gh = k->gpH; gh.first = hb; }
        const size_t w1 = (size_t)gw.wsum_points() * G1.xyzz_bytes, w2 = (size_t)gw.wsum_points() * G2.xyzz_bytes, wh = (size_t)gh.wsum_points() * G1.xyzz_bytes;
        if (3 * w1 + w2 + wh + 64 > 256 * 1024 || 3 * w1 + w2 + wh > (size_t)8 * 80 * 4 * 96) return fail(c, SB_ERR_ARG, "window buffer too small");
        uint8_t* dws = (uint8_t*)k->dWsum; uint8_t* hws = c->pinned;
        uint64_t* hcounts = (uint64_t*)(c->pinned + 3 * w1 + w2 + wh);
        CU(c, cudaEventRecord(c->pev[0], s0));
        if (sN != s0) CU(c, cudaStreamWaitEvent(sN, c->pev[0], 0));
        cudaStream_t saved = c->stream; c->stream = sN;
        rc = run_qap_ntt();
        MsmSorted sh;
        if (!rc) { rc = msm_sort_entries((const uint8_t*)tmp + hlo * 32, 32, hcnt, gh, c->sort_scratch2, sN, &sh, &c->stats); if (rc) rc = cuda_fail(c, (cudaError_t)rc, "msm_sort_entries"); }
        c->stream = saved;
        if (rc) return rc;
        CU(c, cudaEventRecord(c->pev[1], sN));
        MsmSorted sw;
        rc = msm_sort_entries((const uint8_t*)k->dW + wlo * 32, 32, wcnt, gw, c->sort_scratch, s0, &sw, &c->stats);
        if (rc) return cuda_fail(c, (cudaError_t)rc, "msm_sort_entries");
        tick(c, 2);
        struct Job { const GroupOps* G; const void* bases; size_t off; size_t len; uint8_t* dst; int tag; const MsmSorted* srt; const MsmGeom* g; };
        Job jobs[5] = {{&G1, pre ? k->tA : (const void*)((const uint8_t*)k->dA + wb * G1.aff_bytes), 0, w1, pA, SB_G1, &sw, &gw},
                       {&G1, pre ? k->tB1 : (const void*)((const uint8_t*)k->dB1 + wb * G1.aff_bytes), w1, w1, pB1, SB_G1, &sw, &gw},
                       {&G2, pre ? k->tB2 : (const void*)((const uint8_t*)k->dB2 + wb * G2.aff_bytes), 3 * w1, w2, pB2, SB_G2, &sw, &gw},
                       {&G1, pre ? k->tC : (const void*)((const uint8_t*)k->dC + wb * G1.aff_bytes), 2 * w1, w1, pC, SB_G1, &sw, &gw},
                       {&G1, pre ? k->tH : (const void*)((const uint8_t*)k->dH + hb * G1.aff_bytes), 3 * w1 + w2, wh, pH, SB_G1, &sh, &gh}};
        for (int i = 0; i < 5; i++) {
            cudaStream_t st = serial ? s0 : c->aux[i];
            if (i == 4 && sN != s0) CU(c, cudaStreamWaitEvent(s0, c->pev[1], 0));
            c->stats.cur_tag = jobs[i].tag;
            rc = jobs[i].G->buckets(jobs[i].bases, *jobs[i].srt, c->bscr[i], s0, dws + jobs[i].off, &c->stats, st, c->pev[8 + i]);
            if (rc) return cuda_fail(c, (cudaError_t)rc, "msm_buckets");
            CU(c, cudaMemcpyAsync(hws + jobs[i].off, dws + jobs[i].off, jobs[i].len, cudaMemcpyDeviceToHost, st));
            if (i == 0) CU(c, cudaMemcpyAsync(&hcounts[0], sw.counts, 8, cudaMemcpyDeviceToHost, st));
            if (i == 4) CU(c, cudaMemcpyAsync(&hcounts[1], sh.counts, 8, cudaMemcpyDeviceToHost, st));
            CU(c, cudaEventRecord(c->pev[2 + i], st));
        }
        tick(c, 3);
        for (int i = 0; i < 5; i++) {
            CU(c, cudaEventSynchronize(c->pev[2 + i]));
            jobs[i].G->combine(hws + jobs[i].off, *jobs[i].g, jobs[i].dst);
            if (ps && i == 0) G1.times(pA, ps->sp, 32, sA.data());
            if (ps && i == 1) G1.times(pB1, ps->rp, 32, rB1.data());
        }
        if (!serial) { for (int i = 0; i < 5; i++) CU(c, cudaStreamWaitEvent(s0, c->pev[2 + i], 0)); CU(c, cudaStreamWaitEvent(s0, c->pev[1], 0)); }
        c->stat[4] += 3.0 * (double)hcounts[0] + (double)hcounts[1]; c->stat[5] += (double)hcounts[0];
    } else {
    rc = run_qap_ntt(); if (rc) return rc;
    tick(c, 2);
    for (uint64_t off = 0; off < wcnt; off += MAXC) {
        uint64_t cn = std::min(MAXC, wcnt - off), base = wb + off;
        MsmGeom g = msm_geometry(cn, 32, c->fr_bits);
        MsmSorted s;
        rc = msm_sort_entries((const uint8_t*)k->dW + (wlo + off) * 32, 32, cn, g, c->sort_scratch, c->stream, &s, &c->stats);
        if (rc) return cuda_fail(c, (cudaError_t)rc, "msm_sort_entries");
        uint8_t* ws = (uint8_t*)k->dWsum;
        size_t w1 = (size_t)g.wsum_points() * G1.xyzz_bytes, w2 = (size_t)g.wsum_points() * G2.xyzz_bytes;
        if (3 * w1 + w2 > (size_t)8 * 80 * 4 * 96) return fail(c, SB_ERR_ARG, "window buffer too small");
        c->stats.cur_tag = SB_G1;
        rc = G1.buckets((const uint8_t*)k->dA + base * G1.aff_bytes, s, c->bucket_scratch, c->stream, ws, &c->stats, nullptr, nullptr); if (rc) return cuda_fail(c, (cudaError_t)rc, "msm A");
        rc = G1.buckets((const uint8_t*)k->dB1 + base * G1.aff_bytes, s, c->bucket_scratch, c->stream, ws + w1, &c->stats, nullptr, nullptr); if (rc) return cuda_fail(c, (cudaError_t)rc, "msm B1");
        rc = G1.buckets((const uint8_t*)k->dC + base * G1.aff_bytes, s, c->bucket_scratch, c->stream, ws + 2 * w1, &c->stats, nullptr, nullptr); if (rc) return cuda_fail(c, (cudaError_t)rc, "msm C");
        c->stats.cur_tag = SB_G2;
        rc = G2.buckets((const uint8_t*)k->dB2 + base * G2.aff_bytes, s, c->bucket_scratch, c->stream, ws + 3 * w1, &c->stats, nullptr, nullptr); if (rc) return cuda_fail(c, (cudaError_t)rc, "msm B2");
        std::vector<uint8_t> hw(3 * w1 + w2);
        uint64_t entries = 0;
        CU(c, cudaMemcpyAsync(hw.data(), ws, hw.size(), cudaMemcpyDeviceToHost, c->stream));
        CU(c, cudaMemcpyAsync(&entries, s.counts, 8, cudaMemcpyDeviceToHost, c->stream));
        CU(c, cudaStreamSynchronize(c->stream));
        c->stat[4] += 3.0 * (double)entries; c->stat[5] += (double)entries;
        G1.combine(hw.data(), g, pA); G1.combine(hw.data() + w1, g, pB1); G1.combine(hw.data() + 2 * w1, g, pC); G2.combine(hw.data() + 3 * w1, g, pB2);
    }
    tick(c, 3);
    if (hcnt) {
        rc = msm_dev_accumulate(c, G1, (const uint8_t*)k->dH + hb * G1.aff_bytes, (const uint8_t*)tmp + hlo * 32, 32, hcnt, pH);
        if (rc) return rc;
    }
    if (ps) { G1.times(pA, ps->sp, 32, sA.data()); G1.times(pB1, ps->rp, 32, rB1.data()); }
    }
    if (ps) {
        G1.add(pC, pH); G1.add(pC, sA.data()); G1.add(pC, rB1.data());
        memset(pB1, 0, G1.xyzz_bytes); memset(pH, 0, G1.xyzz_bytes);
    }
    tick(c, 4);
    cudaEventSynchronize(c->ev[4]);
    prof_end(c);
    c->last_ms[0] = elapsed(c, 0, 4); c->last_ms[1] = elapsed(c, 0, 1); c->last_ms[2] = elapsed(c, 1, 2); c->last_ms[3] = elapsed(c, 2, 3); c->last_ms[4] = elapsed(c, 3, 4);
    return 0;
}


struct VkPoints { const uint8_t *alpha1, *beta1, *beta2, *delta1, *delta2; };
static void plain_scalars(int curve, const uint8_t r[32], const uint8_t s[32], uint8_t rp[32], uint8_t sp[32], uint8_t rsp[32], bool negate_rs) {
    uint8_t rs[32];
    if (curve == SB_BN254) {
        fr_from_mont_bytes<BnFr>(r, rp); fr_from_mont_bytes<BnFr>(s, sp);
        Fp<BnFr> a, b; memcpy(&a, r, 32); memcpy(&b, s, 32); a = Fp<BnFr>::mul(a, b); if (negate_rs) a = Fp<BnFr>::neg(a); memcpy(rs, &a, 32);
        fr_from_mont_bytes<BnFr>(rs, rsp);
    } else {
        fr_from_mont_bytes<BlsFr>(r, rp); fr_from_mont_bytes<BlsFr>(s, sp);
        Fp<BlsFr> a, b; memcpy(&a, r, 32); memcpy(&b, s, 32); a = Fp<BlsFr>::mul(a, b); if (negate_rs) a = Fp<BlsFr>::neg(a); memcpy(rs, &a, 32);
        fr_from_mont_bytes<BlsFr>(rs, rsp);
    }
}
static int groth16_assemble_host(int curve, const GroupOps& G1, const GroupOps& G2, const VkPoints& vk, const uint8_t* partials,
                                 const uint8_t r[32], const uint8_t s[32], uint8_t* proof);
static int groth16_assemble(sb_ctx* c, Groth16Key* k, const uint8_t* partials, const uint8_t r[32], const uint8_t s[32], uint8_t* proof) {
    VkPoints vk{k->alpha1.data(), k->beta1.data(), k->beta2.data(), k->delta1.data(), k->delta2.data()};
    return groth16_assemble_host(c->curve, c->g1, c->g2, vk, partials, r, s, proof);
}
static int groth16_assemble_host(int curve, const GroupOps& G1, const GroupOps& G2, const VkPoints& vk, const uint8_t* partials,
                                 const uint8_t r[32], const uint8_t s[32], uint8_t* proof) {
    const uint32_t x1 = G1.xyzz_bytes, x2 = G2.xyzz_bytes;
    std::vector<uint8_t> A(partials, partials + x1), B1(partials + x1, partials + 2 * x1), C(partials + 2 * x1, partials + 3 * x1),
        H(partials + 3 * x1, partials + 4 * x1), B2(partials + 4 * x1, partials + 4 * x1 + x2);
    uint8_t rp[32], sp[32], rsp[32];
    plain_scalars(curve, r, s, rp, sp, rsp, true);
    std::vector<uint8_t> t1(x1), t2(x2), d1(x1), d2(x2), pt(x1), pt2(x2);
    G1.from_affine(vk.delta1, d1.data()); G2.from_affine(vk.delta2, d2.data());
    G1.from_affine(vk.alpha1, pt.data()); G1.add(A.data(), pt.data());
    G1.times(d1.data(), rp, 32, t1.data()); G1.add(A.data(), t1.data());
    G2.from_affine(vk.beta2, pt2.data()); G2.add(B2.data(), pt2.data());
    G2.times(d2.data(), sp, 32, t2.data()); G2.add(B2.data(), t2.data());
    G1.from_affine(vk.beta1, pt.data()); G1.add(B1.data(), pt.data());
    G1.times(d1.data(), sp, 32, t1.data()); G1.add(B1.data(), t1.data());
    G1.add(C.data(), H.data());
    G1.times(A.data(), sp, 32, t1.data()); G1.add(C.data(), t1.data());
    G1.times(B1.data(), rp, 32, t1.data()); G1.add(C.data(), t1.data());
    G1.times(d1.data(), rsp, 32, t1.data()); G1.add(C.data(), t1.data());
    G1.to_affine(A.data(), proof);
    G2.to_affine(B2.data(), proof + G1.aff_bytes);
    G1.to_affine(C.data(), proof + G1.aff_bytes + G2.aff_bytes);
    return 0;
}

struct FixedParts { std::vector<uint8_t> Fa, Fb, Fc; };
static FixedParts groth16_fixed_parts(int curve, const GroupOps& G1, const GroupOps& G2, const VkPoints vk, const uint8_t* r, const uint8_t* s) {
    const uint32_t x1 = G1.xyzz_bytes, x2 = G2.xyzz_bytes;
    uint8_t rp[32], sp[32], rsp[32];
    plain_scalars(curve, r, s, rp, sp, rsp, false);
    FixedParts f; f.Fa.assign(x1, 0); f.Fb.assign(x2, 0); f.Fc.assign(x1, 0);
    std::vector<uint8_t> a1(x1), b1(x1), d1(x1), b2(x2), d2(x2), t1(x1), t2(x2);
    G1.from_affine(vk.alpha1, a1.data()); G1.from_affine(vk.beta1, b1.data()); G1.from_affine(vk.delta1, d1.data());
    G2.from_affine(vk.beta2, b2.data()); G2.from_affine(vk.delta2, d2.data());
    std::future<void> g2 = std::async(std::launch::async, [&]() { G2.times(d2.data(), sp, 32, t2.data()); });
    G1.times(d1.data(), rp, 32, t1.data()); f.Fa = a1; G1.add(f.Fa.data(), t1.data());
    G1.times(a1.data(), sp, 32, f.Fc.data());
    G1.times(b1.data(), rp, 32, t1.data()); G1.add(f.Fc.data(), t1.data());
    G1.times(d1.data(), rsp, 32, t1.data()); G1.add(f.Fc.data(), t1.data());
    g2.get();
    f.Fb = b2; G2.add(f.Fb.data(), t2.data());
    return f;
}
static void groth16_finish_folded(const GroupOps& G1, const GroupOps& G2, const FixedParts& f, const uint8_t* partials, uint8_t* proof) {
    const uint32_t x1 = G1.xyzz_bytes, x2 = G2.xyzz_bytes;
    std::vector<uint8_t> A(partials, partials + x1), C(partials + 2 * x1, partials + 3 * x1), B2(partials + 4 * x1, partials + 4 * x1 + x2);
    G1.add(A.data(), f.Fa.data()); G2.add(B2.data(), f.Fb.data()); G1.add(C.data(), f.Fc.data());
    G1.to_affine(A.data(), proof);
    G2.to_affine(B2.data(), proof + G1.aff_bytes);
    G1.to_affine(C.data(), proof + G1.aff_bytes + G2.aff_bytes);
}
static int groth16_prove_folded(sb_ctx* c, Groth16Key* k, const uint8_t* witness, uint64_t n_witness, const uint8_t r[32], const uint8_t s[32], uint8_t* proof) {
    VkPoints vk{k->alpha1.data(), k->beta1.data(), k->beta2.data(), k->delta1.data(), k->delta2.data()};
    const int curve = c->curve; const GroupOps G1 = c->g1, G2 = c->g2;
    std::future<FixedParts> fixed = std::async(std::launch::async, [=]() { return groth16_fixed_parts(curve, G1, G2, vk, r, s); });
    ProofScalars ps; uint8_t rsp[32]; plain_scalars(curve, r, s, ps.rp, ps.sp, rsp, false);
    std::vector<uint8_t> partials(sb_groth16_partials_bytes(c));
    int rc = groth16_device(c, k, witness, n_witness, 0, 1, partials.data(), &ps, false);
    FixedParts f = fixed.get();
    if (rc) return rc;
    groth16_finish_folded(c->g1, c->g2, f, partials.data(), proof);
    return 0;
}

int sb_groth16_prove(sb_ctx* c, uint64_t h, const uint8_t* witness, uint64_t n_witness, const uint8_t r[32], const uint8_t s[32], uint8_t* proof) { SB_LOCK(c);
    Groth16Key* k = get_key(c, h); if (!k) return fail(c, SB_ERR_ARG, "invalid groth16 handle");
    if (k->n_shards > 1) return fail(c, SB_ERR_ARG, "proving key was loaded sharded: use sb_groth16_prove_shard + sb_groth16_finish");
    if (!witness || !r || !s || !proof) return fail(c, SB_ERR_ARG, "null argument");
    return groth16_prove_folded(c, k, witness, n_witness, r, s, proof);
}
int sb_groth16_prove_resident(sb_ctx* c, uint64_t h, const uint8_t r[32], const uint8_t s[32], uint8_t* proof) { SB_LOCK(c);
    Groth16Key* k = get_key(c, h); if (!k) return fail(c, SB_ERR_ARG, "invalid groth16 handle");
    if (k->n_shards > 1) return fail(c, SB_ERR_ARG, "proving key was loaded sharded: use sb_groth16_prove_shard + sb_groth16_finish");
    if (!r || !s || !proof) return fail(c, SB_ERR_ARG, "null argument");
    return groth16_prove_folded(c, k, nullptr, k->nVars, r, s, proof);
}
int sb_groth16_prove_shard(sb_ctx* c, uint64_t h, const uint8_t* witness, uint64_t n_witness, int shard, int n_shards, uint8_t* partials_out) { SB_LOCK(c);
    Groth16Key* k = get_key(c, h); if (!k) return fail(c, SB_ERR_ARG, "invalid groth16 handle");
    if (n_shards < 1 || shard < 0 || shard >= n_shards) return fail(c, SB_ERR_ARG, "invalid shard");
    return groth16_device(c, k, witness, n_witness, shard, n_shards, partials_out);
}
int sb_groth16_finish(sb_ctx* c, uint64_t h, const uint8_t* all, int n_shards, const uint8_t r[32], const uint8_t s[32], uint8_t* proof) { SB_LOCK(c);
    Groth16Key* k = get_key(c, h); if (!k) return fail(c, SB_ERR_ARG, "invalid groth16 handle");
    const GroupOps& G1 = c->g1; const GroupOps& G2 = c->g2;
    const uint32_t x1 = G1.xyzz_bytes, pb = sb_groth16_partials_bytes(c);
    std::vector<uint8_t> acc(pb, 0);
    for (int i = 0; i < n_shards; i++) {
        const uint8_t* p = all + (size_t)i * pb;
        for (int j = 0; j < 4; j++) G1.add(acc.data() + j * x1, p + j * x1);
        G2.add(acc.data() + 4 * x1, p + 4 * x1);
    }
    return groth16_assemble(c, k, acc.data(), r, s, proof);
}

int sb_groth16_prove_dist(sb_ctx* c, uint64_t h, const uint8_t* witness, uint64_t n_witness, const uint8_t r[32], const uint8_t s[32], uint8_t* proof) { SB_LOCK(c);
    Groth16Key* k = get_key(c, h); if (!k) return fail(c, SB_ERR_ARG, "invalid groth16 handle");
    if (!c->comm) return fail(c, SB_ERR_ARG, "context has no communicator: call sb_comm_init_rank first");
    if (!r || !s) return fail(c, SB_ERR_ARG, "null argument");
    NcclApi* nc = nccl_api(nullptr);
    VkPoints vk{k->alpha1.data(), k->beta1.data(), k->beta2.data(), k->delta1.data(), k->delta2.data()};
    const int curve = c->curve; const GroupOps G1 = c->g1, G2 = c->g2;
    std::future<FixedParts> fixed;
    if (proof) fixed = std::async(std::launch::async, [=]() { return groth16_fixed_parts(curve, G1, G2, vk, r, s); });
    ProofScalars ps; uint8_t rsp[32]; plain_scalars(curve, r, s, ps.rp, ps.sp, rsp, false);
    const size_t pb = sb_groth16_partials_bytes(c);
    uint8_t* mine = c->h_xchg + pb * c->world;
    int rc = groth16_device(c, k, witness, n_witness, c->rank, c->world, mine, &ps, true);
    if (rc) { if (proof) fixed.get(); return rc; }
    cudaError_t e = cudaMemcpyAsync((uint8_t*)c->d_xchg + pb * c->rank, mine, pb, cudaMemcpyHostToDevice, c->stream);
    ncclResult_t nr = ncclSuccess;
    if (e == cudaSuccess) nr = nc->AllGather((const uint8_t*)c->d_xchg + pb * c->rank, c->d_xchg, pb, ncclUint8, c->comm, c->stream);
    if (e == cudaSuccess && nr == ncclSuccess && proof) e = cudaMemcpyAsync(c->h_xchg, c->d_xchg, pb * c->world, cudaMemcpyDeviceToHost, c->stream);
    if (e == cudaSuccess) e = cudaStreamSynchronize(c->stream);
    if (proof) {
        FixedParts f = fixed.get();
        if (e == cudaSuccess && nr == ncclSuccess) {
            const uint32_t x1 = G1.xyzz_bytes;
            std::vector<uint8_t> acc(pb, 0);
            for (int i = 0; i < c->world; i++) {
                const uint8_t* p = c->h_xchg + (size_t)i * pb;
                G1.add(acc.data(), p); G1.add(acc.data() + 2 * x1, p + 2 * x1); G2.add(acc.data() + 4 * x1, p + 4 * x1);
            }
            groth16_finish_folded(G1, G2, f, acc.data(), proof);
        }
    }
    if (nr != ncclSuccess) return fail(c, SB_ERR_CUDA, std::string("ncclAllGather: ") + nc->GetErrorString(nr));
    if (e != cudaSuccess) return cuda_fail(c, e, "partial exchange");
    return 0;
}

int sb_create_multi(int curve, const int* device_ids, int n_devices, sb_ctx** out) {
    if (!device_ids || !out || n_devices < 1 || n_devices > 64) return SB_ERR_ARG;
    for (int i = 0; i < n_devices; i++) out[i] = nullptr;
    int rc = 0;
    for (int i = 0; i < n_devices && !rc; i++) rc = sb_create(curve, device_ids[i], &out[i]);
    uint8_t id[128];
    if (!rc && n_devices > 1) rc = sb_comm_unique_id(id);
    if (!rc && n_devices > 1) {
        std::vector<std::future<int>> f;
        for (int i = 0; i < n_devices; i++) f.push_back(std::async(std::launch::async, [=]() { return sb_comm_init_rank(out[i], n_devices, i, id); }));
        for (auto& x : f) { int r = x.get(); if (r && !rc) rc = r; }
    }
    if (rc) { for (int i = 0; i < n_devices; i++) { if (out[i]) sb_destroy(out[i]); out[i] = nullptr; } }
    return rc;
}
int sb_groth16_load_multi(sb_ctx* const* ctxs, int n, const uint8_t* zkey, uint64_t zkey_len, uint64_t* handles) {
    if (!ctxs || !zkey || !handles || n < 1) return SB_ERR_ARG;
    std::vector<std::future<int>> f;
    for (int i = 0; i < n; i++) f.push_back(std::async(std::launch::async, [=]() { return sb_groth16_load_sharded(ctxs[i], zkey, zkey_len, i, n, &handles[i]); }));
    int rc = 0; for (auto& x : f) { int r = x.get(); if (r && !rc) rc = r; }
    return rc;
}
int sb_groth16_prove_multi(sb_ctx* const* ctxs, const uint64_t* handles, int n, const uint8_t* witness, uint64_t n_witness,
                           const uint8_t r[32], const uint8_t s[32], uint8_t* proof_affine_out) {
    if (!ctxs || !handles || n < 1 || !proof_affine_out) return SB_ERR_ARG;
    if (n == 1) return sb_groth16_prove(ctxs[0], handles[0], witness, n_witness, r, s, proof_affine_out);
    std::vector<std::future<int>> f;
    for (int i = 0; i < n; i++)
        f.push_back(std::async(std::launch::async, [=]() { return sb_groth16_prove_dist(ctxs[i], handles[i], witness, n_witness, r, s, i == 0 ? proof_affine_out : nullptr); }));
    int rc = 0; for (auto& x : f) { int r2 = x.get(); if (r2 && !rc) rc = r2; }
    return rc;
}

static void host_ops(int curve, GroupOps& g1, GroupOps& g2) {
    if (curve == SB_BN254) { g1 = SB_GROUP_OPS(bn254_g1, 64); g2 = SB_GROUP_OPS(bn254_g2, 128); }
    else { g1 = SB_GROUP_OPS(bls12381_g1, 96); g2 = SB_GROUP_OPS(bls12381_g2, 192); }
}
int sb_host_sum_partials(int curve, int group, const uint8_t* partials, int count, uint8_t* out_jacobian) {
    if ((curve != SB_BN254 && curve != SB_BLS12_381) || (group != SB_G1 && group != SB_G2) || count < 0) return SB_ERR_ARG;
    GroupOps g1, g2; host_ops(curve, g1, g2);
    const GroupOps& G = group == SB_G1 ? g1 : g2;
    std::vector<uint8_t> acc(G.xyzz_bytes, 0);
    for (int i = 0; i < count; i++) G.add(acc.data(), partials + (size_t)i * G.xyzz_bytes);
    G.to_jacobian(acc.data(), out_jacobian);
    return 0;
}
int sb_host_partial_from_affine(int curve, int group, const uint8_t* affine, uint8_t* partial_out) {
    if ((curve != SB_BN254 && curve != SB_BLS12_381) || (group != SB_G1 && group != SB_G2)) return SB_ERR_ARG;
    GroupOps g1, g2; host_ops(curve, g1, g2);
    (group == SB_G1 ? g1 : g2).from_affine(affine, partial_out);
    return 0;
}
uint32_t sb_host_partial_bytes(int curve, int group) {
    GroupOps g1, g2; if (curve != SB_BN254 && curve != SB_BLS12_381) return 0; host_ops(curve, g1, g2);
    return group == SB_G1 ? g1.xyzz_bytes : g2.xyzz_bytes;
}
int sb_host_groth16_finish(int curve, const uint8_t* vk_alpha1, const uint8_t* vk_beta1, const uint8_t* vk_beta2,
                           const uint8_t* vk_delta1, const uint8_t* vk_delta2, const uint8_t* partials_all_ranks, int n_shards,
                           const uint8_t r[32], const uint8_t s[32], uint8_t* proof_affine_out) {
    if ((curve != SB_BN254 && curve != SB_BLS12_381) || n_shards < 1) return SB_ERR_ARG;
    GroupOps G1, G2; host_ops(curve, G1, G2);
    const uint32_t x1 = G1.xyzz_bytes, pb = 4 * G1.xyzz_bytes + G2.xyzz_bytes;
    std::vector<uint8_t> acc(pb, 0);
    for (int i = 0; i < n_shards; i++) {
        const uint8_t* p = partials_all_ranks + (size_t)i * pb;
        for (int j = 0; j < 4; j++) G1.add(acc.data() + j * x1, p + j * x1);
        G2.add(acc.data() + 4 * x1, p + 4 * x1);
    }
    VkPoints vk{vk_alpha1, vk_beta1, vk_beta2, vk_delta1, vk_delta2};
    return groth16_assemble_host(curve, G1, G2, vk, acc.data(), r, s, proof_affine_out);
}
void sb_shard_range(uint64_t total, int shard, int n_shards, uint64_t* first, uint64_t* count) {
    uint64_t per = (total + n_shards - 1) / n_shards, lo = std::min(total, per * (uint64_t)shard);
    *first = lo; *count = std::min(total - lo, per);
}

int sb_groth16_prove_wtns(sb_ctx* c, uint64_t h, const uint8_t* w, uint64_t wlen, const uint8_t r[32], const uint8_t s[32], uint8_t* proof) { SB_LOCK(c);
    Groth16Key* k = get_key(c, h); if (!k) return fail(c, SB_ERR_ARG, "invalid groth16 handle");
    std::map<uint32_t, Section> secs;
    int rc = parse_binfile(c, w, wlen, "wtns", 2, secs); if (rc) return rc;
    if (!secs[1].present || !secs[2].present) return fail(c, SB_ERR_FORMAT, "Missing section");
    const uint8_t* hd = w + secs[1].pos;
    if (secs[1].len < 4) return fail(c, SB_ERR_FORMAT, "wtns header too short");
    uint32_t n8; memcpy(&n8, hd, 4);
    if (secs[1].len < 8 + (uint64_t)n8) return fail(c, SB_ERR_FORMAT, "wtns header too short");
    if (!modulus_matches(hd + 4, n8, c->curve, true)) return fail(c, SB_ERR_ARG, "Curve of the witness does not match the curve of the proving key");
    uint32_t nw; memcpy(&nw, hd + 4 + n8, 4);
    if (secs[2].len != (uint64_t)nw * n8) return fail(c, SB_ERR_FORMAT, "Invalid witness section size");
    return sb_groth16_prove(c, h, w + secs[2].pos, nw, r, s, proof);
}

}

#include "api_plonk.inl"
#include "api_fflonk.inl"

extern "C" {

int sb_plonk_load(sb_ctx* c, const uint8_t* zkey, uint64_t len, uint64_t* handle) { SB_LOCK(c);
    if (!c || !zkey || !handle) return SB_ERR_ARG;
    cudaSetDevice(c->device);
    return c->curve == SB_BN254 ? plonk_load_impl<BnFr>(c, zkey, len, handle) : plonk_load_impl<BlsFr>(c, zkey, len, handle);
}
static int load_mapped(sb_ctx* c, const char* path, uint64_t* handle, int (*load)(sb_ctx*, const uint8_t*, uint64_t, uint64_t*)) {
    if (!c || !path || !handle) return SB_ERR_ARG;
    int fd = open(path, O_RDONLY);
    if (fd < 0) return fail(c, SB_ERR_FORMAT, std::string("cannot open ") + path);
    struct stat st;
    if (fstat(fd, &st) != 0 || st.st_size <= 0) { close(fd); return fail(c, SB_ERR_FORMAT, std::string("cannot stat ") + path); }
    void* p = mmap(nullptr, (size_t)st.st_size, PROT_READ, MAP_PRIVATE, fd, 0);
    close(fd);
    if (p == MAP_FAILED) return fail(c, SB_ERR_FORMAT, std::string("cannot map ") + path);
    madvise(p, (size_t)st.st_size, MADV_SEQUENTIAL);
    int rc = load(c, (const uint8_t*)p, (uint64_t)st.st_size, handle);
    munmap(p, (size_t)st.st_size);
    return rc;
}
int sb_plonk_load_file(sb_ctx* c, const char* path, uint64_t* handle) { SB_LOCK(c); return load_mapped(c, path, handle, sb_plonk_load); }
static PlonkKeyDev* get_plonk_key(sb_ctx* c, uint64_t h) { return (c && h >= 1 && h <= c->plonk_keys.size()) ? c->plonk_keys[h - 1] : nullptr; }
int sb_plonk_info(sb_ctx* c, uint64_t h, uint32_t* n_vars, uint32_t* n_public, uint32_t* domain_size, uint32_t* n_additions) { SB_LOCK(c);
    PlonkKeyDev* k = get_plonk_key(c, h); if (!k) return fail(c, SB_ERR_ARG, "invalid plonk handle");
    if (n_vars) *n_vars = k->z.nVars; if (n_public) *n_public = k->z.nPublic; if (domain_size) *domain_size = k->z.n; if (n_additions) *n_additions = k->z.nAdditions;
    return 0;
}
uint32_t sb_plonk_proof_bytes(sb_ctx* c) { return c ? 9 * c->g1.aff_bytes + 6 * 32 : 0; }
int sb_plonk_prove(sb_ctx* c, uint64_t h, const uint8_t* witness, uint64_t n_witness, const uint8_t* blinders, uint8_t* proof) { SB_LOCK(c);
    PlonkKeyDev* k = get_plonk_key(c, h); if (!k) return fail(c, SB_ERR_ARG, "invalid plonk handle");
    if (!witness || !blinders || !proof) return fail(c, SB_ERR_ARG, "null argument");
    cudaSetDevice(c->device);
    return c->curve == SB_BN254 ? plonk_prove_impl<BnFq, BnFr>(c, k, witness, n_witness, blinders, proof)
                                : plonk_prove_impl<BlsFq, BlsFr>(c, k, witness, n_witness, blinders, proof);
}
int sb_plonk_prove_resident(sb_ctx* c, uint64_t h, const uint8_t* blinders, uint8_t* proof) { SB_LOCK(c);
    PlonkKeyDev* k = get_plonk_key(c, h); if (!k) return fail(c, SB_ERR_ARG, "invalid plonk handle");
    if (!blinders || !proof) return fail(c, SB_ERR_ARG, "null argument");
    if (!k->n_wit_resident) return fail(c, SB_ERR_ARG, "no witness resident for this proving key: call sb_plonk_prove first");
    cudaSetDevice(c->device);
    return c->curve == SB_BN254 ? plonk_prove_impl<BnFq, BnFr>(c, k, nullptr, 0, blinders, proof)
                                : plonk_prove_impl<BlsFq, BlsFr>(c, k, nullptr, 0, blinders, proof);
}
int sb_plonk_release(sb_ctx* c, uint64_t h) { SB_LOCK(c);
    PlonkKeyDev* k = get_plonk_key(c, h); if (!k) return fail(c, SB_ERR_ARG, "invalid plonk handle");
    cudaSetDevice(c->device); cudaStreamSynchronize(c->stream);
    plonk_free_key(k); c->plonk_keys[h - 1] = nullptr;
    return 0;
}

int sb_fflonk_load(sb_ctx* c, const uint8_t* zkey, uint64_t len, uint64_t* handle) { SB_LOCK(c);
    if (!c || !zkey || !handle) return SB_ERR_ARG;
    if (c->curve != SB_BN254) return fail(c, SB_ERR_ARG, "fflonk is defined on bn128 only (src/fflonk_setup.js:534-557)");
    cudaSetDevice(c->device);
    return fflonk_load_impl<BnFr>(c, zkey, len, handle);
}
int sb_fflonk_load_file(sb_ctx* c, const char* path, uint64_t* handle) { SB_LOCK(c); return load_mapped(c, path, handle, sb_fflonk_load); }
static FflonkKeyDev* get_fflonk_key(sb_ctx* c, uint64_t h) { return (c && h >= 1 && h <= c->fflonk_keys.size()) ? c->fflonk_keys[h - 1] : nullptr; }
int sb_fflonk_info(sb_ctx* c, uint64_t h, uint32_t* n_vars, uint32_t* n_public, uint32_t* domain_size, uint32_t* n_additions) { SB_LOCK(c);
    FflonkKeyDev* k = get_fflonk_key(c, h); if (!k) return fail(c, SB_ERR_ARG, "invalid fflonk handle");
    if (n_vars) *n_vars = k->z.nVars; if (n_public) *n_public = k->z.nPublic; if (domain_size) *domain_size = k->z.n; if (n_additions) *n_additions = k->z.nAdditions;
    return 0;
}
uint32_t sb_fflonk_proof_bytes(sb_ctx* c) { return c ? 4 * c->g1.aff_bytes + 16 * 32 : 0; }
int sb_fflonk_prove(sb_ctx* c, uint64_t h, const uint8_t* witness, uint64_t n_witness, const uint8_t* blinders, uint8_t* proof) { SB_LOCK(c);
    FflonkKeyDev* k = get_fflonk_key(c, h); if (!k) return fail(c, SB_ERR_ARG, "invalid fflonk handle");
    if (!witness || !blinders || !proof) return fail(c, SB_ERR_ARG, "null argument");
    cudaSetDevice(c->device);
    return fflonk_prove_impl<BnFq, BnFr>(c, k, witness, n_witness, blinders, proof);
}
int sb_fflonk_prove_resident(sb_ctx* c, uint64_t h, const uint8_t* blinders, uint8_t* proof) { SB_LOCK(c);
    FflonkKeyDev* k = get_fflonk_key(c, h); if (!k) return fail(c, SB_ERR_ARG, "invalid fflonk handle");
    if (!blinders || !proof) return fail(c, SB_ERR_ARG, "null argument");
    if (!k->n_wit_resident) return fail(c, SB_ERR_ARG, "no witness resident for this proving key: call sb_fflonk_prove first");
    cudaSetDevice(c->device);
    return fflonk_prove_impl<BnFq, BnFr>(c, k, nullptr, 0, blinders, proof);
}
int sb_fflonk_release(sb_ctx* c, uint64_t h) { SB_LOCK(c);
    FflonkKeyDev* k = get_fflonk_key(c, h); if (!k) return fail(c, SB_ERR_ARG, "invalid fflonk handle");
    cudaSetDevice(c->device); cudaStreamSynchronize(c->stream);
    fflonk_free_key(k); c->fflonk_keys[h - 1] = nullptr;
    return 0;
}

}
```

snarkjs_b200/csrc/msm.cuh:

```cuda
#pragma once
#include <cuda_runtime.h>
#include "ec.cuh"
#include "msm_geom.h"

namespace sb {

static constexpr int MSM_SEG = 32;
static constexpr int MSM_ACC_THREADS = 128;
static constexpr int MSM_RED_CHUNK = 16;
static constexpr uint32_t MSM_INVALID_KEY = 0xffffffffu;
static constexpr int MSM_COUNTS_SEG = 8;


__host__ inline MsmGeom msm_choose(uint64_t n, uint32_t scalar_bytes, int fr_bits, bool precomp) {
    int eff = (int)(8 * scalar_bytes) < fr_bits ? (int)(8 * scalar_bytes) : fr_bits;
    int best_c = 3; double best = 1e300;
    for (int c = 3; c <= 22; c++) {
        int weff = (eff + 1 + c - 1) / c, top = eff + 1 - (weff - 1) * c;
        if (weff > 1 && top < c - 5) continue;
        double buckets = (precomp ? 1.0 : (double)weff) * (double)(1u << (c - 1));
        double cost = (double)weff * (double)n * 10.0 + buckets * 60.0;
        if (cost < best) { best = cost; best_c = c; }
    }
    MsmGeom g; g.c = best_c; g.W = (int)((8 * scalar_bytes + 1 + best_c - 1) / best_c); g.B = 1u << (best_c - 1);
    return g;
}
__host__ inline MsmGeom msm_geometry_precomp(uint64_t n_set, uint32_t scalar_bytes, int fr_bits = 254) {
    int l2 = 0; while ((1ull << (l2 + 1)) <= n_set) l2++;
    int cmax = l2; if (cmax > 22) cmax = 22; if (cmax < 8) cmax = 8;
    int c = 8;
    for (int cc = cmax; cc >= 8; cc--) {
        int weff = (fr_bits + 1 + cc - 1) / cc, top = fr_bits + 1 - (weff - 1) * cc;
        if (weff > 1 && top < cc - 5) continue;
        c = cc; break;
    }
    MsmGeom g; g.c = c; g.W = (int)((8 * scalar_bytes + 1 + c - 1) / c); g.B = 1u << (c - 1);
    g.precomp = 1; g.stride = n_set; g.first = 0;
    return g;
}
__host__ inline MsmGeom msm_geometry(uint64_t n, uint32_t scalar_bytes, int fr_bits = 254) {
    return msm_choose(n, scalar_bytes, fr_bits, false);
}

template <class F> __device__ __forceinline__ void load_affine(const Affine<F>* __restrict__ bases, uint32_t idx, F& x, F& y) {
    constexpr int NV = sizeof(F) / 16;
    const uint4* p = reinterpret_cast<const uint4*>(bases + idx);
    uint4* dx = reinterpret_cast<uint4*>(&x);
    uint4* dy = reinterpret_cast<uint4*>(&y);
#pragma unroll
    for (int k = 0; k < NV; k++) dx[k] = __ldg(p + k);
#pragma unroll
    for (int k = 0; k < NV; k++) dy[k] = __ldg(p + NV + k);
}
template <class T> __device__ __forceinline__ void store_vec(T* dst, const T& v) {
    constexpr int NV = sizeof(T) / 16;
    const uint4* s = reinterpret_cast<const uint4*>(&v);
    uint4* d = reinterpret_cast<uint4*>(dst);
#pragma unroll
    for (int k = 0; k < NV; k++) d[k] = s[k];
}
template <class T> __device__ __forceinline__ T load_vec(const T* src) {
    constexpr int NV = sizeof(T) / 16;
    T v; const uint4* s = reinterpret_cast<const uint4*>(src);
    uint4* d = reinterpret_cast<uint4*>(&v);
#pragma unroll
    for (int k = 0; k < NV; k++) d[k] = s[k];
    return v;
}

template <class P> __device__ __forceinline__ Fp<P> PairInvF(const Fp<P>& a) { return Fp<P>::inv_binary(a); }
template <class P> __device__ __forceinline__ Fp2<P> PairInvF(const Fp2<P>& a) { return Fp2<P>::inv(a); }

template <class F, int MINB>
__global__ void __launch_bounds__(MSM_ACC_THREADS, MINB)
k_accumulate(const Affine<F>* __restrict__ bases, const uint32_t* __restrict__ keys, const uint32_t* __restrict__ vals,
             const uint64_t* __restrict__ counts, XYZZ<F>* __restrict__ buckets,
             XYZZ<F>* __restrict__ heads, uint32_t* __restrict__ head_keys) {
    const uint64_t M = counts[0];
    const uint32_t seg = (uint32_t)counts[MSM_COUNTS_SEG];
    uint64_t t = blockIdx.x * (uint64_t)blockDim.x + threadIdx.x;
    uint64_t lo = t * seg;
    if (lo >= M) return;
    uint64_t hi = lo + seg < M ? lo + seg : M;
    const F one = F::one();
    XYZZ<F> acc = XYZZ<F>::inf();
    uint32_t cur = keys[lo];
    bool first = true;
    for (uint64_t e = lo; e < hi; e++) {
        uint32_t k = keys[e], v = vals ? vals[e] : (uint32_t)e;
        if (k != cur) {
            if (first) { store_vec(heads + t, acc); head_keys[t] = cur; first = false; }
            else store_vec(buckets + cur, acc);
            acc = XYZZ<F>::inf(); cur = k;
        }
        F px, py;
        load_affine<F>(bases, v & 0x7fffffffu, px, py);
        if (!(px.is_zero() & py.is_zero())) {
            py = F::cneg(py, (v >> 31) != 0);
            acc.add_affine(px, py, one);
        }
    }
    if (first) { store_vec(heads + t, acc); head_keys[t] = cur; }
    else store_vec(buckets + cur, acc);
}

template <class T> struct fp2_param;
template <class P> struct fp2_param<Fp2<P>> { typedef P type; };
template <class P, int MINB>
__global__ void __launch_bounds__(MSM_ACC_THREADS, MINB)
k_accumulate_pair(const Affine<Fp2<P>>* __restrict__ bases, const uint32_t* __restrict__ keys, const uint32_t* __restrict__ vals,
                  const uint64_t* __restrict__ counts, XYZZ<Fp2<P>>* __restrict__ buckets,
                  XYZZ<Fp2<P>>* __restrict__ heads, uint32_t* __restrict__ head_keys) {
    typedef Fp2L<P> F; typedef Fp<P> B;
    const uint64_t M = counts[0];
    const uint32_t seg = (uint32_t)counts[MSM_COUNTS_SEG];
    const uint64_t t = (blockIdx.x * (uint64_t)blockDim.x + threadIdx.x) >> 1;
    const uint32_t par = threadIdx.x & 1u;
    uint64_t lo = t * seg;
    if (lo >= M) return;
    uint64_t hi = lo + seg < M ? lo + seg : M;
    const F one = F::one();
    XYZZ<F> acc = XYZZ<F>::inf();
    auto put = [&](XYZZ<Fp2<P>>* dst, const XYZZ<F>& a) {
        B* q = reinterpret_cast<B*>(dst);
        store_vec(q + par, a.x.m); store_vec(q + 2 + par, a.y.m); store_vec(q + 4 + par, a.zz.m); store_vec(q + 6 + par, a.zzz.m);
    };
    uint32_t cur = keys[lo];
    bool first = true;
    for (uint64_t e = lo; e < hi; e++) {
        uint32_t k = keys[e], v = vals ? vals[e] : (uint32_t)e;
        if (k != cur) {
            if (first) { put(heads + t, acc); if (!par) head_keys[t] = cur; first = false; }
            else put(buckets + cur, acc);
            acc = XYZZ<F>::inf(); cur = k;
        }
        F px, py;
        {
            constexpr int NV = sizeof(B) / 16;
            const uint4* p = reinterpret_cast<const uint4*>(reinterpret_cast<const B*>(bases + (v & 0x7fffffffu)) + par);
            uint4* dx = reinterpret_cast<uint4*>(&px.m); uint4* dy = reinterpret_cast<uint4*>(&py.m);
#pragma unroll
            for (int i = 0; i < NV; i++) dx[i] = __ldg(p + i);
#pragma unroll
            for (int i = 0; i < NV; i++) dy[i] = __ldg(p + 2 * NV + i);
        }
        if (!(px.is_zero() & py.is_zero())) {
            py = F::cneg(py, (v >> 31) != 0);
            acc.add_affine(px, py, one);
        }
    }
    if (first) { put(heads + t, acc); if (!par) head_keys[t] = cur; }
    else put(buckets + cur, acc);
}

static constexpr int MSM_SHORT_RUN = 8;
template <class F>
__global__ void __launch_bounds__(MSM_ACC_THREADS)
k_fold_short(const XYZZ<F>* __restrict__ heads, const uint32_t* __restrict__ keys_in, uint32_t* __restrict__ keys_out,
             const uint64_t* __restrict__ counts, XYZZ<F>* __restrict__ buckets) {
    const uint64_t M = counts[1];
    uint64_t t = blockIdx.x * (uint64_t)blockDim.x + threadIdx.x;
    if (t >= M) return;
    const uint32_t k = keys_in[t];
    uint64_t start = t; int back = 0;
    while (start > 0 && back < MSM_SHORT_RUN && keys_in[start - 1] == k) { start--; back++; }
    bool is_short = back < MSM_SHORT_RUN;
    uint64_t len = 0;
    if (is_short) {
        len = 1;
        while (start + len < M && len <= (uint64_t)MSM_SHORT_RUN && keys_in[start + len] == k) len++;
        is_short = len <= (uint64_t)MSM_SHORT_RUN;
    }
    keys_out[t] = is_short ? MSM_INVALID_KEY : k;
    if (!is_short || start != t) return;
    XYZZ<F> acc = load_vec(buckets + k);
    for (uint64_t e = 0; e < len; e++) { XYZZ<F> p = load_vec(heads + t + e); acc.add(p); }
    store_vec(buckets + k, acc);
}

template <class F>
__global__ void __launch_bounds__(MSM_ACC_THREADS)
k_fold(const XYZZ<F>* __restrict__ in, const uint32_t* __restrict__ in_keys, const uint64_t* __restrict__ counts, int level,
       XYZZ<F>* __restrict__ buckets, XYZZ<F>* __restrict__ heads, uint32_t* __restrict__ head_keys) {
    const uint64_t M = counts[level];
    const bool last = M <= MSM_SEG;
    uint64_t t = blockIdx.x * (uint64_t)blockDim.x + threadIdx.x;
    uint64_t lo = t * MSM_SEG;
    if (lo >= M) return;
    uint64_t hi = lo + MSM_SEG < M ? lo + MSM_SEG : M;
    XYZZ<F> acc = XYZZ<F>::inf();
    uint32_t cur = in_keys[lo];
    bool first = !last;
    auto flush = [&]() {
        if (first) { store_vec(heads + t, acc); head_keys[t] = cur; first = false; }
        else if (cur != MSM_INVALID_KEY) { XYZZ<F> b = load_vec(buckets + cur); b.add(acc); store_vec(buckets + cur, b); }
    };
    for (uint64_t e = lo; e < hi; e++) {
        uint32_t k = in_keys[e];
        if (k != cur) { flush(); acc = XYZZ<F>::inf(); cur = k; }
        if (k != MSM_INVALID_KEY) { XYZZ<F> p = load_vec(in + e); acc.add(p); }
    }
    flush();
}

template <class F>
__global__ void __launch_bounds__(128)
k_reduce(const XYZZ<F>* __restrict__ buckets, MsmGeom g, XYZZ<F>* __restrict__ partials, uint32_t ctas_per_window) {
    extern __shared__ uint4 smem_raw[];
    XYZZ<F>* sm = reinterpret_cast<XYZZ<F>*>(smem_raw);
    const uint32_t w = blockIdx.x / ctas_per_window, cta = blockIdx.x % ctas_per_window;
    const uint32_t L = g.B < (uint32_t)MSM_RED_CHUNK ? g.B : MSM_RED_CHUNK;
    const uint32_t chunks = g.B / L;
    const uint32_t j = cta * blockDim.x + threadIdx.x;
    XYZZ<F> part = XYZZ<F>::inf();
    if (j < chunks) {
        const XYZZ<F>* bk = buckets + (uint64_t)w * g.B + (uint64_t)j * L;
        XYZZ<F> run = XYZZ<F>::inf(), sum = XYZZ<F>::inf();
        for (int b = (int)L - 1; b >= 0; b--) {
            XYZZ<F> p = load_vec(bk + b);
            run.add(p);
            sum.add(run);
        }
        uint32_t k = j * L;
        if (k) {
            int top = 31 - __clz(k);
            part = run;
            for (int bit = top - 1; bit >= 0; bit--) {
                part = XYZZ<F>::dbl(part);
                if ((k >> bit) & 1) part.add(run);
            }
        }
        part.add(sum);
    }
    store_vec(sm + threadIdx.x, part);
    __syncthreads();
    for (uint32_t s = blockDim.x >> 1; s > 0; s >>= 1) {
        if (threadIdx.x < s) {
            XYZZ<F> a = load_vec(sm + threadIdx.x), b = load_vec(sm + threadIdx.x + s);
            a.add(b);
            store_vec(sm + threadIdx.x, a);
        }
        __syncthreads();
    }
    if (threadIdx.x == 0) store_vec(partials + (uint64_t)w * ctas_per_window + cta, load_vec(sm));
}

template <class F>
__device__ __forceinline__ void combine_children(const XYZZ<F>* Rin, const XYZZ<F>* Sin, int m, int log_n, XYZZ<F>& Rout, XYZZ<F>& Sout) {
    XYZZ<F> t = XYZZ<F>::inf(), acc = XYZZ<F>::inf(), ssum = load_vec(Sin);
    for (int i = m - 1; i >= 1; i--) {
        XYZZ<F> r = load_vec(Rin + i), s = load_vec(Sin + i);
        t.add(r); acc.add(t); ssum.add(s);
    }
    for (int k = 0; k < log_n; k++) acc = XYZZ<F>::dbl(acc);
    ssum.add(acc);
    XYZZ<F> r0 = load_vec(Rin); t.add(r0);
    Rout = t; Sout = ssum;
}

static constexpr int RED2_L = 16, RED2_THREADS = 128, RED2_BUCKETS = RED2_L * RED2_THREADS;

template <class F>
__global__ void __launch_bounds__(RED2_THREADS)
k_reduce2(const XYZZ<F>* __restrict__ buckets, MsmGeom g, XYZZ<F>* __restrict__ outR, XYZZ<F>* __restrict__ outS) {
    extern __shared__ uint4 smem_raw[];
    XYZZ<F>* sm = reinterpret_cast<XYZZ<F>*>(smem_raw);
    XYZZ<F>* R1 = sm; XYZZ<F>* S1 = sm + 128; XYZZ<F>* R2 = sm + 256; XYZZ<F>* S2 = sm + 272; XYZZ<F>* R3 = sm + 288; XYZZ<F>* S3 = sm + 292;
    const uint32_t tid = threadIdx.x;
    const XYZZ<F>* bk = buckets + (uint64_t)blockIdx.x * RED2_BUCKETS + (uint64_t)tid * RED2_L;
    {
        XYZZ<F> run = XYZZ<F>::inf(), sum = XYZZ<F>::inf();
        for (int b = RED2_L - 1; b >= 0; b--) { XYZZ<F> p = load_vec(bk + b); run.add(p); sum.add(run); }
        store_vec(R1 + tid, run); store_vec(S1 + tid, sum);
    }
    __syncthreads();
    if (tid < 16) { XYZZ<F> r, s; combine_children<F>(R1 + 8 * tid, S1 + 8 * tid, 8, 4, r, s); store_vec(R2 + tid, r); store_vec(S2 + tid, s); }
    __syncthreads();
    if (tid < 4) { XYZZ<F> r, s; combine_children<F>(R2 + 4 * tid, S2 + 4 * tid, 4, 7, r, s); store_vec(R3 + tid, r); store_vec(S3 + tid, s); }
    __syncthreads();
    if (tid == 0) { XYZZ<F> r, s; combine_children<F>(R3, S3, 4, 9, r, s); store_vec(outR + blockIdx.x, r); store_vec(outS + blockIdx.x, s); }
}

template <class F>
__global__ void __launch_bounds__(128)
k_window_sum2(const XYZZ<F>* __restrict__ inR, const XYZZ<F>* __restrict__ inS, uint32_t NC, XYZZ<F>* __restrict__ out) {
    extern __shared__ uint4 smem_raw[];
    XYZZ<F>* sm = reinterpret_cast<XYZZ<F>*>(smem_raw);
    const uint32_t tid = threadIdx.x;
    const XYZZ<F>* Rin = inR + (uint64_t)blockIdx.x * NC; const XYZZ<F>* Sin = inS + (uint64_t)blockIdx.x * NC;
    uint32_t n = NC; int log_block = 11;
    int ping = 0;
    while (n > 1) {
        const uint32_t m = n >= 8 ? 8 : n, parents = n / m;
        XYZZ<F>* Rout = sm + ping * 256; XYZZ<F>* Sout = Rout + 128;
        for (uint32_t p = tid; p < parents; p += blockDim.x) {
            XYZZ<F> r, s; combine_children<F>(Rin + (uint64_t)p * m, Sin + (uint64_t)p * m, (int)m, log_block, r, s);
            store_vec(Rout + p, r); store_vec(Sout + p, s);
        }
        __syncthreads();
        Rin = Rout; Sin = Sout; n = parents; ping ^= 1;
        log_block += (m == 8 ? 3 : m == 4 ? 2 : 1);
    }
    if (tid == 0) store_vec(out + blockIdx.x, load_vec(Sin));
}

template <class F>
__global__ void __launch_bounds__(32)
k_window_sum(const XYZZ<F>* __restrict__ partials, uint32_t per_window, XYZZ<F>* __restrict__ out) {
    extern __shared__ uint4 smem_raw[];
    XYZZ<F>* sm = reinterpret_cast<XYZZ<F>*>(smem_raw);
    XYZZ<F> acc = XYZZ<F>::inf();
    for (uint32_t i = threadIdx.x; i < per_window; i += 32) { XYZZ<F> p = load_vec(partials + (uint64_t)blockIdx.x * per_window + i); acc.add(p); }
    store_vec(sm + threadIdx.x, acc);
    __syncwarp();
    for (uint32_t s = 16; s > 0; s >>= 1) {
        if (threadIdx.x < s) { XYZZ<F> a = load_vec(sm + threadIdx.x), b = load_vec(sm + threadIdx.x + s); a.add(b); store_vec(sm + threadIdx.x, a); }
        __syncwarp();
    }
    if (threadIdx.x == 0) store_vec(out + blockIdx.x, load_vec(sm));
}

template <class F> __device__ __noinline__ void padd(XYZZ<F>& a, const XYZZ<F>& b) { a.add(b); }

struct AxisJob { const void* in; void* out; uint64_t total; uint32_t S; uint32_t log_inner; };

template <class F>
__global__ void __launch_bounds__(128)
k_axis_sum(AxisJob j0, AxisJob j1) {
    const AxisJob j = blockIdx.y ? j1 : j0;
    const uint64_t gid = blockIdx.x * (uint64_t)blockDim.x + threadIdx.x;
    if (gid >= j.total) return;
    const uint64_t o = gid >> j.log_inner, i = gid & ((1ull << j.log_inner) - 1);
    const XYZZ<F>* p = (const XYZZ<F>*)j.in + ((o * j.S) << j.log_inner) + i;
    XYZZ<F> acc = load_vec(p);
#pragma unroll 1
    for (uint32_t s = 1; s < j.S; s++) { XYZZ<F> v = load_vec(p + ((uint64_t)s << j.log_inner)); acc.add(v); }
    store_vec((XYZZ<F>*)j.out + gid, acc);
}

template <class F> __device__ __forceinline__ XYZZ<F> shfl_down_pt(const XYZZ<F>& v, int d) {
    constexpr int NW32 = sizeof(XYZZ<F>) / 4;
    union U { XYZZ<F> p; uint32_t w[NW32]; __device__ U() {} };
    U a, r; a.p = v;
#pragma unroll
    for (int k = 0; k < NW32; k++) r.w[k] = __shfl_down_sync(0xffffffffu, a.w[k], d);
    return r.p;
}
template <class F> __device__ __forceinline__ void warp_weighted_sum(XYZZ<F> v, XYZZ<F>& T, XYZZ<F>& W) {
    const int lane = threadIdx.x & 31;
#pragma unroll 1
    for (int d = 1; d < 32; d <<= 1) { XYZZ<F> o = shfl_down_pt<F>(v, d); if (lane + d < 32) v.add(o); }
    T = v;
    XYZZ<F> x = lane ? v : XYZZ<F>::inf();
#pragma unroll 1
    for (int d = 16; d >= 1; d >>= 1) { XYZZ<F> o = shfl_down_pt<F>(x, d); if (lane < d) x.add(o); }
    W = x;
}
template <class F> __device__ __forceinline__ XYZZ<F> warp_sum(XYZZ<F> x) {
    const int lane = threadIdx.x & 31;
#pragma unroll 1
    for (int d = 16; d >= 1; d >>= 1) { XYZZ<F> o = shfl_down_pt<F>(x, d); if (lane < d) x.add(o); }
    return x;
}

template <class F>
__global__ void __launch_bounds__(128)
k_ws_chunks(const XYZZ<F>* __restrict__ vecR, uint32_t lenR, const XYZZ<F>* __restrict__ vecC, uint32_t lenC, uint32_t NW, XYZZ<F>* __restrict__ tw) {
    const uint32_t nR = (lenR + 31) / 32, nC = (lenC + 31) / 32, per = nR + nC;
    const uint32_t wid = blockIdx.x * (blockDim.x >> 5) + (threadIdx.x >> 5), lane = threadIdx.x & 31;
    if (wid >= NW * per) return;
    const uint32_t w = wid / per, jj = wid % per;
    const bool isR = jj < nR;
    const uint32_t j = isR ? jj : jj - nR, len = isR ? lenR : lenC, idx = j * 32 + lane;
    const XYZZ<F>* vec = (isR ? vecR : vecC) + (uint64_t)w * len;
    XYZZ<F> v = XYZZ<F>::inf();
    if (idx < len) v = load_vec(vec + idx);
    XYZZ<F> T, W;
    warp_weighted_sum<F>(v, T, W);
    if (lane == 0) { store_vec(tw + 2 * (uint64_t)wid, T); store_vec(tw + 2 * (uint64_t)wid + 1, W); }
}

template <class F>
__global__ void __launch_bounds__(128)
k_ws_final(const XYZZ<F>* __restrict__ tw, uint32_t nR, uint32_t nC, XYZZ<F>* __restrict__ out) {
    const uint32_t warp = threadIdx.x >> 5, lane = threadIdx.x & 31, per = nR + nC;
    const XYZZ<F>* base = tw + 2 * (uint64_t)blockIdx.x * per;
    const bool r_side = warp < 2;
    const uint32_t cnt = r_side ? nR : nC, off = r_side ? 0 : nR;
    XYZZ<F> v = XYZZ<F>::inf();
    if (lane < cnt) v = load_vec(base + 2 * (uint64_t)(off + lane) + (warp & 1));
    XYZZ<F>* o = out + 5 * (uint64_t)blockIdx.x;
    if ((warp & 1) == 0) {
        XYZZ<F> tot, res;
        warp_weighted_sum<F>(v, tot, res);
        if (lane == 0) { store_vec(o + (r_side ? 0 : 2), res); if (!r_side) store_vec(o + 4, tot); }
    } else {
        XYZZ<F> res = warp_sum<F>(v);
        if (lane == 0) store_vec(o + (r_side ? 1 : 3), res);
    }
}

template <class F>
__global__ void __launch_bounds__(128)
k_axis_tree(AxisJob j0, AxisJob j1) {
    const AxisJob j = blockIdx.y ? j1 : j0;
    const uint64_t wid = blockIdx.x * (uint64_t)(blockDim.x >> 5) + (threadIdx.x >> 5);
    const uint32_t lane = threadIdx.x & 31;
    if (wid >= j.total) return;
    const uint64_t o = wid >> j.log_inner, i = wid & ((1ull << j.log_inner) - 1);
    const XYZZ<F>* p = (const XYZZ<F>*)j.in + ((o * j.S) << j.log_inner) + i;
    XYZZ<F> acc = XYZZ<F>::inf();
#pragma unroll 1
    for (uint32_t s = lane; s < j.S; s += 32) { XYZZ<F> v = load_vec(p + ((uint64_t)s << j.log_inner)); acc.add(v); }
    acc = warp_sum<F>(acc);
    if (lane == 0) store_vec((XYZZ<F>*)j.out + wid, acc);
}

static constexpr int WS_COL_BITS = 10;
struct WsPlan {
    bool ok = false;
    int m = 0, er = 0, ec = 0;
    int levels = 0; int br[8] = {0}, bc[8] = {0};
    uint32_t lenR = 0, lenC = 0, nR = 0, nC = 0;
    size_t rowA = 0, rowB = 0, colA = 0, colB = 0, tw = 0;
    size_t elems() const { return rowA + rowB + colA + colB + tw + 8; }
};
__host__ inline WsPlan ws_plan(const MsmGeom& g) {
    WsPlan p; const int cbits = g.c - 1; const size_t NW = g.windows();
    if (cbits > 2 * WS_COL_BITS || cbits < 0) return p;
    p.ok = true;
    if (cbits > WS_COL_BITS) { p.m = WS_COL_BITS; p.er = p.m; p.ec = cbits - p.m; p.lenR = 1u << p.ec; p.lenC = 1u << p.m; }
    else { p.lenR = 0; p.lenC = g.B; }
    int rr = p.er, rc = p.ec;
    for (int l = 0; l < 2 && (rr > 0 || rc > 0); l++) {
        p.levels++;
        p.br[l] = l == 0 ? (rr < 3 ? rr : 3) : rr; p.bc[l] = l == 0 ? (rc < 3 ? rc : 3) : rc; rr -= p.br[l]; rc -= p.bc[l];
        const size_t orow = p.br[l] ? (NW * g.B) >> (p.er - rr) : 0, ocol = p.bc[l] ? (NW * g.B) >> (p.ec - rc) : 0;
        if (l & 1) { p.rowB = orow; p.colB = ocol; } else { p.rowA = orow; p.colA = ocol; }
    }
    p.nR = (p.lenR + 31) / 32; p.nC = (p.lenC + 31) / 32;
    p.tw = 2 * NW * (p.nR + p.nC);
    return p;
}
__host__ inline size_t msm_reduce_scratch_elems(const MsmGeom& g) {
    const uint32_t NW = g.windows();
    const uint32_t L = g.B < (uint32_t)MSM_RED_CHUNK ? g.B : MSM_RED_CHUNK;
    const uint32_t ctas_per_window = (g.B / L + 127) / 128;
    const size_t legacy = (size_t)2 * NW * ctas_per_window;
    const WsPlan p = ws_plan(g);
    return (p.ok && p.elems() > legacy) ? p.elems() : legacy;
}

template <class F>
__global__ void __launch_bounds__(128) k_precompute(const Affine<F>* __restrict__ bases, uint64_t n, int c, int W, Affine<F>* __restrict__ table) {
    uint64_t i = blockIdx.x * (uint64_t)blockDim.x + threadIdx.x;
    if (i >= n) return;
    Affine<F> a = load_vec(bases + i);
    store_vec(table + i, a);
    if (a.is_inf()) {
        for (int w = 1; w < W; w++) store_vec(table + (uint64_t)w * n + i, a);
        return;
    }
    XYZZ<F> p; p.x = a.x; p.y = a.y; p.zz = F::one(); p.zzz = F::one();
    for (int w = 1; w < W; w++) {
        for (int j = 0; j < c; j++) p = XYZZ<F>::dbl(p);
        Affine<F> o;
        if (p.is_inf()) { o.x = F::zero(); o.y = F::zero(); }
        else { F t = PairInvF(F::mul(p.zz, p.zzz)); o.x = F::mul(p.x, F::mul(t, p.zzz)); o.y = F::mul(p.y, F::mul(t, p.zz)); p.x = o.x; p.y = o.y; p.zz = F::one(); p.zzz = F::one(); }
        store_vec(table + (uint64_t)w * n + i, o);
    }
}

__host__ __device__ inline uint64_t splitmix64(uint64_t x) {
    x += 0x9E3779B97F4A7C15ull; x = (x ^ (x >> 30)) * 0xBF58476D1CE4E5B9ull; x = (x ^ (x >> 27)) * 0x94D049BB133111EBull; return x ^ (x >> 31);
}
static constexpr uint64_t GEN_CHUNK = 4096;
template <class F>
__global__ void __launch_bounds__(128) k_gen_points(Affine<F> g, uint64_t seed, uint64_t n, Affine<F>* __restrict__ out) {
    uint64_t i = blockIdx.x * (uint64_t)blockDim.x + threadIdx.x;
    if (i >= n) return;
    const uint64_t c = i / GEN_CHUNK, j = i % GEN_CHUNK;
    const uint64_t k0 = (seed ^ 0x9E3779B97F4A7C15ull) + c * 0xD1B54A32D192ED03ull, kd = seed * 2654435761ull + 12345ull;
    uint64_t lo = j * kd, hi = __umul64hi(j, kd);
    lo += k0; hi += lo < k0 ? 1 : 0;
    const F one = F::one();
    XYZZ<F> r = XYZZ<F>::inf();
    for (int bit = 79; bit >= 0; bit--) {
        r = XYZZ<F>::dbl(r);
        const uint64_t wd = bit >= 64 ? hi : lo;
        if ((wd >> (bit & 63)) & 1) r.add_affine(g.x, g.y, one);
    }
    Affine<F> a;
    if (r.is_inf()) { a.x = F::zero(); a.y = F::zero(); }
    else { F t = PairInvF(F::mul(r.zz, r.zzz)); a.x = F::mul(r.x, F::mul(t, r.zzz)); a.y = F::mul(r.y, F::mul(t, r.zz)); }
    store_vec(out + i, a);
}

}
#include "msm_pair.cuh"
namespace sb {

struct MsmScratch {
    void* p = nullptr; size_t cap = 0;
    void* get(size_t bytes) {
        if (bytes > cap) { if (p) cudaFree(p); p = nullptr; cap = 0; if (cudaMalloc(&p, bytes) != cudaSuccess) return nullptr; cap = bytes; }
        return p;
    }
    void release() { if (p) cudaFree(p); p = nullptr; cap = 0; }
};

extern int g_msm_tuning[12];

struct MsmLaunchStats {
    int launches = 0;
    cudaEvent_t* ev = nullptr; int nev = 0; int used = 0; int tag[128] = {0}; int cur_tag = 0;
};
enum { PROF_ACC_G1 = 1, PROF_ACC_G2 = 2, PROF_SORT = 3, PROF_FOLD = 4, PROF_REDUCE = 5, PROF_QAP = 6, PROF_NTT = 7, PROF_JOIN = 8 };
struct ProfScope {
    MsmLaunchStats* s; cudaStream_t st; int idx = -1;
    ProfScope(MsmLaunchStats* s_, int tag, cudaStream_t st_) : s(s_), st(st_) {
        if (s && s->ev && s->used + 2 <= s->nev && s->used / 2 < 128) { idx = s->used; s->used += 2; s->tag[idx / 2] = tag; cudaEventRecord(s->ev[idx], st); }
    }
    void end() { if (idx >= 0) { cudaEventRecord(s->ev[idx + 1], st); idx = -1; } }
    void end(cudaStream_t other) { st = other; end(); }
};

struct MsmSorted {
    const uint32_t* keys = nullptr; const uint32_t* vals = nullptr; const uint64_t* counts = nullptr;
    uint64_t n = 0, total = 0; MsmGeom g{};
    uint32_t seg_lo = MSM_SEG;
};

size_t msm_pair_scan_tmp_bytes(uint32_t NB);
int msm_pair_offsets(const uint32_t* keys, const uint64_t* counts, uint32_t NB, uint32_t* off, cudaStream_t stream);
int msm_pair_next_offsets(const uint32_t* off_in, uint32_t NB, uint32_t* sizes, uint32_t* off_out, void* tmp, size_t tmp_bytes, cudaStream_t stream);
int msm_pair_counts(const uint32_t* off, uint32_t NB, uint64_t* counts, cudaStream_t stream);

int msm_sort_entries(const uint8_t* d_scalars, uint32_t sbytes, uint64_t n, MsmGeom g, MsmScratch& scratch,
                     cudaStream_t stream, MsmSorted* out, MsmLaunchStats* stats);

template <class F>
int msm_buckets_impl(const Affine<F>* d_bases, const MsmSorted& s, MsmScratch& scratch, size_t scratch_off, cudaStream_t stream,
                     XYZZ<F>* d_wsum, MsmLaunchStats* stats, cudaStream_t tail_stream, cudaEvent_t ev_acc);

template <class F>
int msm_buckets(const Affine<F>* d_bases, const MsmSorted& s, MsmScratch& scratch, cudaStream_t stream,
                XYZZ<F>* d_wsum, MsmLaunchStats* stats, cudaStream_t tail_stream = nullptr, cudaEvent_t ev_acc = nullptr) {
    const MsmGeom g = s.g;
    const uint64_t NBl = (uint64_t)g.windows() * g.B;
    const double avg = NBl ? (double)s.total / (double)NBl : 0.0;
    if (g_msm_tuning[4] != 2 || avg < 4.0 || NBl >= (1ull << 31) || s.total >= (1ull << 31))
        return msm_buckets_impl<F>(d_bases, s, scratch, 0, stream, d_wsum, stats, tail_stream, ev_acc);
    const uint32_t NB = (uint32_t)NBl;
    int R = 1; while ((1u << R) < 2.0 * avg && R < 8) R++;
    if (g_msm_tuning[5] > 0 && g_msm_tuning[5] < R) R = g_msm_tuning[5];
    auto al = [](size_t x) { return (x + 255) & ~(size_t)255; };
    const uint64_t ub1 = (s.total + NB + 1) / 2;
    const size_t scan_tmp = msm_pair_scan_tmp_bytes(NB);
    const uint64_t pthreads = ((ub1 + PAIR_K - 1) / PAIR_K + PAIR_THREADS - 1) / PAIR_THREADS * PAIR_THREADS;
    size_t o_offA = 0, o_offB = o_offA + al((size_t)(NB + 1) * 4), o_sizes = o_offB + al((size_t)(NB + 1) * 4);
    size_t o_tmp = o_sizes + al((size_t)(NB + 1) * 4), o_cnt = o_tmp + al(scan_tmp);
    size_t o_PA = o_cnt + 256, o_PB = o_PA + al(ub1 * sizeof(Affine<F>)), o_KA = o_PB + al(ub1 * sizeof(Affine<F>));
    size_t o_KB = o_KA + al(ub1 * 4), o_L = o_KB + al(ub1 * 4), o_rest = o_L + al(pthreads * PAIR_K * sizeof(F));
    uint64_t ub = s.total; for (int r = 0; r < R; r++) ub = (ub + NB + 1) / 2;
    MsmSorted s2 = s; s2.total = ub; s2.vals = nullptr; s2.seg_lo = MSM_SEG;
    {
        const uint64_t heads0 = (ub + MSM_SEG - 1) / MSM_SEG, heads1 = (heads0 + MSM_SEG - 1) / MSM_SEG;
        const uint32_t L = g.B < (uint32_t)MSM_RED_CHUNK ? g.B : MSM_RED_CHUNK;
        const uint32_t ctas_per_window = (g.B / L + 127) / 128;
        size_t need = al(NBl * sizeof(XYZZ<F>)) + al(heads0 * sizeof(XYZZ<F>)) + al(heads0 * 4) + al(heads1 * sizeof(XYZZ<F>)) + al(heads1 * 4) +
                      al(heads0 * 4) + al(msm_reduce_scratch_elems(g) * sizeof(XYZZ<F>));
        need += need / 8 + (1u << 20);
        if (!scratch.get(o_rest + need)) return (int)cudaErrorMemoryAllocation;
    }
    uint8_t* base = (uint8_t*)scratch.p;
    uint32_t* offA = (uint32_t*)(base + o_offA); uint32_t* offB = (uint32_t*)(base + o_offB); uint32_t* sizes = (uint32_t*)(base + o_sizes);
    uint64_t* counts2 = (uint64_t*)(base + o_cnt);
    Affine<F>* P[2] = {(Affine<F>*)(base + o_PA), (Affine<F>*)(base + o_PB)};
    uint32_t* K[2] = {(uint32_t*)(base + o_KA), (uint32_t*)(base + o_KB)};
    F* Ls = (F*)(base + o_L);
    int launches = 0;
    ProfScope prof(stats, stats ? stats->cur_tag : 0, stream);
    int rc = msm_pair_offsets(s.keys, s.counts, NB, offA, stream); launches++;
    if (rc) return rc;
    const Affine<F>* src = d_bases; uint32_t* in = offA; uint32_t* out = offB;
    uint64_t ubr = s.total;
    for (int r = 0; r < R; r++) {
        rc = msm_pair_next_offsets(in, NB, sizes, out, base + o_tmp, scan_tmp, stream); launches += 3;
        if (rc) return rc;
        ubr = (ubr + NB + 1) / 2;
        const unsigned grid = (unsigned)(((ubr + PAIR_K - 1) / PAIR_K + PAIR_THREADS - 1) / PAIR_THREADS);
        if (r == 0) k_pair_round<F, true><<<grid, PAIR_THREADS, 0, stream>>>(src, s.vals, in, out, NB, P[0], K[0], Ls);
        else k_pair_round<F, false><<<grid, PAIR_THREADS, 0, stream>>>(src, nullptr, in, out, NB, P[r & 1], K[r & 1], Ls);
        launches++;
        src = P[r & 1]; s2.keys = K[r & 1];
        uint32_t* t = in; in = out; out = t;
    }
    rc = msm_pair_counts(in, NB, counts2, stream); launches++;
    if (rc) return rc;
    s2.counts = counts2;
    prof.end();
    if (stats) stats->launches += launches;
    cudaEvent_t* sev = stats ? stats->ev : nullptr; if (stats) stats->ev = nullptr;
    rc = msm_buckets_impl<F>(src, s2, scratch, o_rest, stream, d_wsum, stats, tail_stream, ev_acc);
    if (stats) stats->ev = sev;
    return rc;
}

template <class F>
int msm_buckets_impl(const Affine<F>* d_bases, const MsmSorted& s, MsmScratch& scratch, size_t scratch_off, cudaStream_t stream,
                     XYZZ<F>* d_wsum, MsmLaunchStats* stats, cudaStream_t tail_stream, cudaEvent_t ev_acc) {
    const MsmGeom g = s.g;
    const uint32_t NW = g.windows();
    const uint64_t nbuckets = (uint64_t)NW * g.B;
    const uint64_t heads0 = (s.total + s.seg_lo - 1) / s.seg_lo;
    const uint64_t heads1 = (heads0 + MSM_SEG - 1) / MSM_SEG;
    const uint32_t L = g.B < (uint32_t)MSM_RED_CHUNK ? g.B : MSM_RED_CHUNK;
    const uint32_t chunks = g.B / L;
    const uint32_t red_threads = 128;
    const uint32_t ctas_per_window = (chunks + red_threads - 1) / red_threads;
    auto al = [](size_t x) { return (x + 255) & ~(size_t)255; };
    size_t o_buckets = 0;
    size_t o_headsA = o_buckets + al(nbuckets * sizeof(XYZZ<F>)), o_hkA = o_headsA + al(heads0 * sizeof(XYZZ<F>));
    size_t o_headsB = o_hkA + al(heads0 * 4), o_hkB = o_headsB + al(heads1 * sizeof(XYZZ<F>));
    size_t o_hkM = o_hkB + al(heads1 * 4);
    size_t o_part = o_hkM + al(heads0 * 4);
    size_t bytes = o_part + al(msm_reduce_scratch_elems(g) * sizeof(XYZZ<F>));
    uint8_t* base = (uint8_t*)scratch.get(scratch_off + bytes);
    if (!base) return (int)cudaErrorMemoryAllocation;
    base += scratch_off;
    XYZZ<F>* buckets = (XYZZ<F>*)(base + o_buckets);
    XYZZ<F>* headsA = (XYZZ<F>*)(base + o_headsA); uint32_t* hkA = (uint32_t*)(base + o_hkA);
    XYZZ<F>* headsB = (XYZZ<F>*)(base + o_headsB); uint32_t* hkB = (uint32_t*)(base + o_hkB);
    XYZZ<F>* partials = (XYZZ<F>*)(base + o_part);
    uint32_t* hkM = (uint32_t*)(base + o_hkM);
    int launches = 0;
    cudaMemsetAsync(buckets, 0, nbuckets * sizeof(XYZZ<F>), stream);
    if (heads0) {
        ProfScope prof(stats, stats ? stats->cur_tag : 0, stream);
        {
            const unsigned grid = (unsigned)((heads0 + MSM_ACC_THREADS - 1) / MSM_ACC_THREADS);
            constexpr bool ext = sizeof(F) > 48 && (sizeof(F) % 64 == 0 || sizeof(F) == 96);
            if constexpr (ext) {
                typedef typename fp2_param<F>::type FP;
                const unsigned pgrid = (unsigned)((2 * heads0 + MSM_ACC_THREADS - 1) / MSM_ACC_THREADS);
                if (g_msm_tuning[9] == 4) k_accumulate_pair<FP, 4><<<pgrid, MSM_ACC_THREADS, 0, stream>>>(d_bases, s.keys, s.vals, s.counts, buckets, headsA, hkA);
                else if (g_msm_tuning[9] == 3) k_accumulate_pair<FP, 3><<<pgrid, MSM_ACC_THREADS, 0, stream>>>(d_bases, s.keys, s.vals, s.counts, buckets, headsA, hkA);
                else switch (g_msm_tuning[0]) {
                case 3: k_accumulate<F, 3><<<grid, MSM_ACC_THREADS, 0, stream>>>(d_bases, s.keys, s.vals, s.counts, buckets, headsA, hkA); break;
                case 4: k_accumulate<F, 4><<<grid, MSM_ACC_THREADS, 0, stream>>>(d_bases, s.keys, s.vals, s.counts, buckets, headsA, hkA); break;
                default: k_accumulate<F, 2><<<grid, MSM_ACC_THREADS, 0, stream>>>(d_bases, s.keys, s.vals, s.counts, buckets, headsA, hkA); break;
                }
            } else if constexpr (sizeof(F) > 32) {
                switch (g_msm_tuning[8]) {
                case 4: k_accumulate<F, 4><<<grid, MSM_ACC_THREADS, 0, stream>>>(d_bases, s.keys, s.vals, s.counts, buckets, headsA, hkA); break;
                case 3: k_accumulate<F, 3><<<grid, MSM_ACC_THREADS, 0, stream>>>(d_bases, s.keys, s.vals, s.counts, buckets, headsA, hkA); break;
                default: k_accumulate<F, 2><<<grid, MSM_ACC_THREADS, 0, stream>>>(d_bases, s.keys, s.vals, s.counts, buckets, headsA, hkA); break;
                }
            } else {
                switch (g_msm_tuning[10]) {
                case 3: k_accumulate<F, 3><<<grid, MSM_ACC_THREADS, 0, stream>>>(d_bases, s.keys, s.vals, s.counts, buckets, headsA, hkA); break;
                case 2: k_accumulate<F, 2><<<grid, MSM_ACC_THREADS, 0, stream>>>(d_bases, s.keys, s.vals, s.counts, buckets, headsA, hkA); break;
                default: k_accumulate<F, 4><<<grid, MSM_ACC_THREADS, 0, stream>>>(d_bases, s.keys, s.vals, s.counts, buckets, headsA, hkA); break;
                }
            }
            launches++;
        }
        prof.end();
        if (tail_stream && tail_stream != stream && ev_acc) {
            cudaEventRecord(ev_acc, stream); cudaStreamWaitEvent(tail_stream, ev_acc, 0); stream = tail_stream;
        }
        ProfScope pfold(stats, PROF_FOLD, stream);
        k_fold_short<F><<<(unsigned)((heads0 + MSM_ACC_THREADS - 1) / MSM_ACC_THREADS), MSM_ACC_THREADS, 0, stream>>>(
            headsA, hkA, hkM, s.counts, buckets); launches++;
        uint64_t m = heads0; int level = 1;
        XYZZ<F>* hin = headsA; uint32_t* kin = hkM; XYZZ<F>* hout = headsB; uint32_t* kout = hkB;
        while (true) {
            uint64_t threads = (m + MSM_SEG - 1) / MSM_SEG;
            k_fold<F><<<(unsigned)((threads + MSM_ACC_THREADS - 1) / MSM_ACC_THREADS), MSM_ACC_THREADS, 0, stream>>>(
                hin, kin, s.counts, level, buckets, hout, kout); launches++;
            if (m <= (uint64_t)MSM_SEG) break;
            m = threads; level++;
            XYZZ<F>* th = hin; hin = hout; hout = th; uint32_t* tk = kin; kin = kout; kout = tk;
            if (level >= 8) return (int)cudaErrorUnknown;
        }
        pfold.end();
    }
    if (!heads0 && tail_stream && tail_stream != stream && ev_acc) { cudaEventRecord(ev_acc, stream); cudaStreamWaitEvent(tail_stream, ev_acc, 0); stream = tail_stream; }
    ProfScope pred(stats, PROF_REDUCE, stream);
    const WsPlan wp = ws_plan(g);
    if (wp.ok && g_msm_tuning[1] == 0) {
        XYZZ<F>* rowb[2] = {partials, partials + wp.rowA};
        XYZZ<F>* colb[2] = {partials + wp.rowA + wp.rowB, partials + wp.rowA + wp.rowB + wp.colA};
        XYZZ<F>* tw = partials + wp.rowA + wp.rowB + wp.colA + wp.colB;
        const XYZZ<F>* rin = buckets; const XYZZ<F>* cin = buckets;
        int rr = wp.er, rc = wp.ec;
        for (int l = 0; l < wp.levels; l++) {
            AxisJob jr{nullptr, nullptr, 0, 1, 0}, jc{nullptr, nullptr, 0, 1, 0};
            if (wp.br[l]) { rr -= wp.br[l]; jr = AxisJob{rin, rowb[l & 1], (uint64_t)nbuckets >> (wp.er - rr), 1u << wp.br[l], (uint32_t)rr}; rin = rowb[l & 1]; }
            if (wp.bc[l]) { rc -= wp.bc[l]; jc = AxisJob{cin, colb[l & 1], (uint64_t)nbuckets >> (wp.ec - rc), 1u << wp.bc[l], (uint32_t)wp.m}; cin = colb[l & 1]; }
            const uint64_t mx = jr.total > jc.total ? jr.total : jc.total;
            if (l == 0) k_axis_sum<F><<<dim3((unsigned)((mx + 127) / 128), 2), 128, 0, stream>>>(jr, jc);
            else k_axis_tree<F><<<dim3((unsigned)((mx + 3) / 4), 2), 128, 0, stream>>>(jr, jc);
            launches++;
        }
        const uint32_t per = wp.nR + wp.nC;
        k_ws_chunks<F><<<(NW * per + 3) / 4, 128, 0, stream>>>(wp.lenR ? rin : nullptr, wp.lenR, cin, wp.lenC, NW, tw); launches++;
        k_ws_final<F><<<NW, 128, 0, stream>>>(tw, wp.nR, wp.nC, d_wsum); launches++;
    } else if (g.B >= (uint32_t)RED2_BUCKETS && g.B / RED2_BUCKETS <= 1024 && g_msm_tuning[1] == 2) {
        const uint32_t NC = g.B / RED2_BUCKETS;
        XYZZ<F>* pR = partials; XYZZ<F>* pS = partials + (size_t)NW * NC;
        static bool configured = false;
        if (!configured) {
            cudaFuncSetAttribute(k_reduce2<F>, cudaFuncAttributeMaxDynamicSharedMemorySize, (int)(296 * sizeof(XYZZ<F>)));
            cudaFuncSetAttribute(k_window_sum2<F>, cudaFuncAttributeMaxDynamicSharedMemorySize, (int)(512 * sizeof(XYZZ<F>)));
            configured = true;
        }
        k_reduce2<F><<<NW * NC, RED2_THREADS, 296 * sizeof(XYZZ<F>), stream>>>(buckets, g, pR, pS); launches++;
        k_window_sum2<F><<<NW, 128, 512 * sizeof(XYZZ<F>), stream>>>(pR, pS, NC, d_wsum); launches++;
    } else {
        k_reduce<F><<<NW * ctas_per_window, red_threads, red_threads * sizeof(XYZZ<F>), stream>>>(buckets, g, partials, ctas_per_window); launches++;
        k_window_sum<F><<<NW, 32, 32 * sizeof(XYZZ<F>), stream>>>(partials, ctas_per_window, d_wsum); launches++;
    }
    pred.end();
    if (stats) stats->launches += launches;
    return (int)cudaGetLastError();
}

}
```

snarkjs_b200/csrc/msm_pair.cuh:

```cuda
#pragma once
#include <cuda_runtime.h>
#include "ec.cuh"
#include "msm_geom.h"

namespace sb {

static constexpr int PAIR_K = 32;
static constexpr int PAIR_THREADS = 128;

__global__ void k_bucket_offsets(const uint32_t* __restrict__ keys, const uint64_t* __restrict__ counts, uint32_t NB, uint32_t* __restrict__ off);
__global__ void k_halve_sizes(const uint32_t* __restrict__ off, uint32_t NB, uint32_t* __restrict__ sizes);
__global__ void k_counts_from_offsets(const uint32_t* __restrict__ off, uint32_t NB, uint64_t* __restrict__ counts);

template <class F> struct PairInv;
template <class P> struct PairInv<Fp<P>> { __device__ static Fp<P> inv(const Fp<P>& a) { return Fp<P>::inv_binary(a); } };
template <class P> struct PairInv<Fp2<P>> { __device__ static Fp2<P> inv(const Fp2<P>& a) { return Fp2<P>::inv(a); } };

template <class F> __device__ __forceinline__ F pair_load_x(const Affine<F>* p) { return load_vec(&p->x); }
template <class F> __device__ __forceinline__ F pair_load_y(const Affine<F>* p) { return load_vec(&p->y); }

enum { PAIR_COPY = 0, PAIR_ADD = 1, PAIR_DBL = 2, PAIR_INF = 3, PAIR_TAKE2 = 4, PAIR_NONE = 5 };

template <class F, bool FIRST>
__device__ __forceinline__ const Affine<F>* pair_src(const Affine<F>* __restrict__ pts, const uint32_t* __restrict__ vals, uint32_t s, bool& neg) {
    if (FIRST) { uint32_t v = vals[s]; neg = (v >> 31) != 0; return pts + (v & 0x7fffffffu); }
    neg = false; return pts + s;
}

template <class F, bool FIRST>
__device__ __forceinline__ int pair_classify(const Affine<F>* __restrict__ pts, const uint32_t* __restrict__ vals, uint32_t s0, bool has_pair, F& den) {
    den = F::one();
    if (!has_pair) return PAIR_COPY;
    bool n1, n2;
    const Affine<F>* p1 = pair_src<F, FIRST>(pts, vals, s0, n1);
    const Affine<F>* p2 = pair_src<F, FIRST>(pts, vals, s0 + 1, n2);
    F x1 = pair_load_x<F>(p1), x2 = pair_load_x<F>(p2);
    if (x1.is_zero()) { if (pair_load_y<F>(p1).is_zero()) return PAIR_TAKE2; }
    if (x2.is_zero()) { if (pair_load_y<F>(p2).is_zero()) return PAIR_COPY; }
    if (x1 == x2) {
        F y1 = F::cneg(pair_load_y<F>(p1), n1), y2 = F::cneg(pair_load_y<F>(p2), n2);
        if (y1 == y2 && !y1.is_zero()) { den = F::dbl(y1); return PAIR_DBL; }
        return PAIR_INF;
    }
    den = F::sub(x2, x1);
    return PAIR_ADD;
}

template <class F, bool FIRST>
__global__ void __launch_bounds__(PAIR_THREADS)
k_pair_round(const Affine<F>* __restrict__ src, const uint32_t* __restrict__ vals, const uint32_t* __restrict__ off_in,
             const uint32_t* __restrict__ off_out, uint32_t NB, Affine<F>* __restrict__ dst, uint32_t* __restrict__ dst_keys,
             F* __restrict__ scratch) {
    __shared__ F sP[PAIR_THREADS];
    __shared__ F sS[PAIR_THREADS];
    __shared__ F sInv;
    const uint32_t total_out = off_out[NB];
    const uint32_t tid = threadIdx.x;
    const uint64_t gt = blockIdx.x * (uint64_t)blockDim.x + tid;
    const uint64_t nthreads = gridDim.x * (uint64_t)blockDim.x;
    const uint64_t o0 = gt * PAIR_K;
    if ((uint64_t)blockIdx.x * blockDim.x * PAIR_K >= total_out) return;
    uint32_t b0 = 0;
    if (o0 < total_out) {
        uint32_t lo = 0, hi = NB;
        while (hi - lo > 1) { uint32_t mid = (lo + hi) >> 1; if (off_out[mid] <= o0) lo = mid; else hi = mid; }
        b0 = lo;
    }
    F pre = F::one();
    {
        uint32_t b = b0;
        for (int k = 0; k < PAIR_K; k++) {
            uint64_t o = o0 + k;
            F den = F::one();
            if (o < total_out) {
                while (off_out[b + 1] <= o) b++;
                uint32_t j = (uint32_t)o - off_out[b], s0 = off_in[b] + 2 * j, m = off_in[b + 1] - off_in[b];
                pair_classify<F, FIRST>(src, vals, s0, 2 * j + 1 < m, den);
            }
            store_vec(scratch + (uint64_t)k * nthreads + gt, pre);
            pre = F::mul(pre, den);
        }
    }
    store_vec(&sP[tid], pre); store_vec(&sS[tid], pre);
    __syncthreads();
    for (int d = 1; d < PAIR_THREADS; d <<= 1) {
        F a, c; bool ha = tid >= (uint32_t)d, hc = tid + d < PAIR_THREADS;
        if (ha) a = F::mul(load_vec(&sP[tid - d]), load_vec(&sP[tid]));
        if (hc) c = F::mul(load_vec(&sS[tid]), load_vec(&sS[tid + d]));
        __syncthreads();
        if (ha) store_vec(&sP[tid], a);
        if (hc) store_vec(&sS[tid], c);
        __syncthreads();
    }
    if (tid < 32) {
        F t = PairInv<F>::inv(load_vec(&sP[PAIR_THREADS - 1]));
        if (tid == 0) store_vec(&sInv, t);
    }
    __syncthreads();
    F running = load_vec(&sInv);
    if (tid > 0) running = F::mul(running, load_vec(&sP[tid - 1]));
    if (tid + 1 < PAIR_THREADS) running = F::mul(running, load_vec(&sS[tid + 1]));
    if (o0 >= total_out) return;
    uint32_t b = b0;
    {
        uint64_t olast = o0 + PAIR_K - 1; if (olast >= total_out) olast = total_out - 1;
        while (off_out[b + 1] <= olast) b++;
    }
    for (int k = PAIR_K - 1; k >= 0; k--) {
        uint64_t o = o0 + k;
        if (o >= total_out) continue;
        while (off_out[b] > o) b--;
        uint32_t j = (uint32_t)o - off_out[b], s0 = off_in[b] + 2 * j, m = off_in[b + 1] - off_in[b];
        F den;
        int kind = pair_classify<F, FIRST>(src, vals, s0, 2 * j + 1 < m, den);
        Affine<F> out;
        bool n1, n2;
        if (kind == PAIR_ADD || kind == PAIR_DBL) {
            F inv = F::mul(running, load_vec(scratch + (uint64_t)k * nthreads + gt));
            running = F::mul(running, den);
            const Affine<F>* p1 = pair_src<F, FIRST>(src, vals, s0, n1);
            const Affine<F>* p2 = pair_src<F, FIRST>(src, vals, s0 + 1, n2);
            F x1 = pair_load_x<F>(p1), y1 = F::cneg(pair_load_y<F>(p1), n1);
            F x2 = pair_load_x<F>(p2);
            F lam;
            if (kind == PAIR_ADD) { F y2 = F::cneg(pair_load_y<F>(p2), n2); lam = F::mul(F::sub(y2, y1), inv); }
            else { F xx = F::sqr(x1); lam = F::mul(F::add(F::dbl(xx), xx), inv); }
            F x3 = F::sub(F::sub(F::sqr(lam), x1), x2);
            out.x = x3; out.y = F::sub(F::mul(lam, F::sub(x1, x3)), y1);
        } else if (kind == PAIR_INF) {
            out.x = F::zero(); out.y = F::zero();
        } else {
            const Affine<F>* p = pair_src<F, FIRST>(src, vals, kind == PAIR_TAKE2 ? s0 + 1 : s0, n1);
            out.x = pair_load_x<F>(p); out.y = F::cneg(pair_load_y<F>(p), n1);
        }
        store_vec(dst + o, out);
        dst_keys[o] = b;
    }
}

}
```

snarkjs_b200/csrc/msm_sort.cu:

```cuda
#include <cub/device/device_radix_sort.cuh>
#include <cub/device/device_scan.cuh>
#include "msm.cuh"

namespace sb {

int g_msm_tuning[12] = {0};

__global__ void k_digits(const uint8_t* __restrict__ scalars, uint32_t sbytes, uint64_t n, MsmGeom g,
                         uint32_t* __restrict__ keys, uint32_t* __restrict__ vals) {
    uint64_t i = blockIdx.x * (uint64_t)blockDim.x + threadIdx.x;
    if (i >= n) return;
    uint32_t w32[17];
    const uint8_t* s = scalars + i * sbytes;
    if (sbytes == 32 && ((uintptr_t)scalars & 15) == 0) {
        const uint4* p = reinterpret_cast<const uint4*>(s);
        uint4 a = __ldg(p), b = __ldg(p + 1);
        w32[0] = a.x; w32[1] = a.y; w32[2] = a.z; w32[3] = a.w; w32[4] = b.x; w32[5] = b.y; w32[6] = b.z; w32[7] = b.w;
#pragma unroll
        for (int k = 8; k < 17; k++) w32[k] = 0;
    } else {
#pragma unroll
        for (int k = 0; k < 17; k++) w32[k] = 0;
        for (uint32_t k = 0; k < sbytes; k++) w32[k >> 2] |= (uint32_t)s[k] << (8 * (k & 3));
    }
    const uint32_t cmask = (1u << g.c) - 1, half = 1u << (g.c - 1);
    uint32_t carry = 0;
    for (int w = 0; w < g.W; w++) {
        uint32_t bit = (uint32_t)w * g.c, wi = bit >> 5, sh = bit & 31;
        uint64_t two = (uint64_t)w32[wi] | ((uint64_t)(wi + 1 < 17 ? w32[wi + 1] : 0) << 32);
        uint32_t raw = ((uint32_t)(two >> sh) & cmask) + carry;
        uint32_t key, val = (uint32_t)i;
        if (raw > half) { raw = (1u << g.c) - raw; carry = 1; val |= 0x80000000u; } else carry = 0;
        if (g.precomp) { key = raw ? raw - 1 : MSM_INVALID_KEY; val = (uint32_t)((uint64_t)w * g.stride + g.first + i) | (val & 0x80000000u); }
        else key = raw ? (uint32_t)w * g.B + raw - 1 : MSM_INVALID_KEY;
        keys[(uint64_t)w * n + i] = key;
        vals[(uint64_t)w * n + i] = val;
    }
}

__global__ void k_count_valid(const uint32_t* __restrict__ keys, uint64_t total, uint64_t* __restrict__ out, uint32_t T, uint32_t seg_lo, uint64_t wave) {
    if (blockIdx.x | threadIdx.x) return;
    uint64_t lo = 0, hi = total;
    while (lo < hi) { uint64_t mid = (lo + hi) >> 1; if (keys[mid] == MSM_INVALID_KEY) hi = mid; else lo = mid + 1; }
    out[0] = lo;
    uint64_t seg = T;
    if (wave) {
        const uint64_t k = (lo + wave * T - 1) / (wave * T);
        if (k && k <= 3) seg = (lo + k * wave - 1) / (k * wave);
        if (seg < seg_lo) seg = seg_lo;
        if (seg > T) seg = T;
    }
    out[MSM_COUNTS_SEG] = seg;
    uint64_t m = (lo + seg - 1) / seg;
    out[1] = m;
    for (int l = 2; l < 8; l++) { m = (m <= MSM_SEG) ? 0 : (m + MSM_SEG - 1) / MSM_SEG; out[l] = m; }
}


__global__ void k_bucket_offsets(const uint32_t* __restrict__ keys, const uint64_t* __restrict__ counts, uint32_t NB, uint32_t* __restrict__ off) {
    uint32_t b = blockIdx.x * blockDim.x + threadIdx.x;
    if (b > NB) return;
    const uint64_t M = counts[0];
    uint64_t lo = 0, hi = M;
    while (lo < hi) { uint64_t mid = (lo + hi) >> 1; if (keys[mid] < b) lo = mid + 1; else hi = mid; }
    off[b] = (uint32_t)lo;
}
__global__ void k_halve_sizes(const uint32_t* __restrict__ off, uint32_t NB, uint32_t* __restrict__ sizes) {
    uint32_t b = blockIdx.x * blockDim.x + threadIdx.x;
    if (b > NB) return;
    sizes[b] = b < NB ? (off[b + 1] - off[b] + 1) / 2 : 0;
}
__global__ void k_counts_from_offsets(const uint32_t* __restrict__ off, uint32_t NB, uint64_t* __restrict__ counts) {
    if (blockIdx.x | threadIdx.x) return;
    uint64_t m = off[NB];
    counts[0] = m;
    m = (m + MSM_SEG - 1) / MSM_SEG; counts[1] = m;
    for (int l = 2; l < 8; l++) { m = (m <= (uint64_t)MSM_SEG) ? 0 : (m + MSM_SEG - 1) / MSM_SEG; counts[l] = m; }
    counts[MSM_COUNTS_SEG] = MSM_SEG;
}
size_t msm_pair_scan_tmp_bytes(uint32_t NB) {
    size_t bytes = 0;
    cub::DeviceScan::ExclusiveSum(nullptr, bytes, (const uint32_t*)nullptr, (uint32_t*)nullptr, (int)(NB + 1));
    return bytes;
}
int msm_pair_offsets(const uint32_t* keys, const uint64_t* counts, uint32_t NB, uint32_t* off, cudaStream_t stream) {
    k_bucket_offsets<<<(NB + 1 + 255) / 256, 256, 0, stream>>>(keys, counts, NB, off);
    return (int)cudaGetLastError();
}
int msm_pair_next_offsets(const uint32_t* off_in, uint32_t NB, uint32_t* sizes, uint32_t* off_out, void* tmp, size_t tmp_bytes, cudaStream_t stream) {
    k_halve_sizes<<<(NB + 1 + 255) / 256, 256, 0, stream>>>(off_in, NB, sizes);
    cudaError_t e = cub::DeviceScan::ExclusiveSum(tmp, tmp_bytes, sizes, off_out, (int)(NB + 1), stream);
    return (int)(e != cudaSuccess ? e : cudaGetLastError());
}
int msm_pair_counts(const uint32_t* off, uint32_t NB, uint64_t* counts, cudaStream_t stream) {
    k_counts_from_offsets<<<1, 1, 0, stream>>>(off, NB, counts);
    return (int)cudaGetLastError();
}

int msm_sort_entries(const uint8_t* d_scalars, uint32_t sbytes, uint64_t n, MsmGeom g, MsmScratch& scratch,
                     cudaStream_t stream, MsmSorted* out, MsmLaunchStats* stats) {
    const uint64_t total = n * (uint64_t)g.W;
    const uint64_t nbuckets = (uint64_t)g.windows() * g.B;
    if (sbytes == 0 || sbytes > 64) return (int)cudaErrorInvalidValue;
    int key_bits = 1; while ((1ull << key_bits) < nbuckets) key_bits++;
    int end_bit = key_bits + 1 > 32 ? 32 : key_bits + 1;
    size_t sort_tmp = 0;
    cub::DoubleBuffer<uint32_t> kb(nullptr, nullptr), vb(nullptr, nullptr);
    cub::DeviceRadixSort::SortPairs(nullptr, sort_tmp, kb, vb, (uint64_t)total, 0, end_bit, stream);
    auto al = [](size_t x) { return (x + 255) & ~(size_t)255; };
    size_t o_keys0 = 0, o_keys1 = o_keys0 + al(total * 4), o_vals0 = o_keys1 + al(total * 4), o_vals1 = o_vals0 + al(total * 4);
    size_t o_tmp = o_vals1 + al(total * 4), o_counts = o_tmp + al(sort_tmp);
    uint8_t* base = (uint8_t*)scratch.get(o_counts + 256);
    if (!base) return (int)cudaErrorMemoryAllocation;
    uint32_t* keys0 = (uint32_t*)(base + o_keys0); uint32_t* keys1 = (uint32_t*)(base + o_keys1);
    uint32_t* vals0 = (uint32_t*)(base + o_vals0); uint32_t* vals1 = (uint32_t*)(base + o_vals1);
    uint64_t* counts = (uint64_t*)(base + o_counts);
    int launches = 0;
    ProfScope prof(stats, PROF_SORT, stream);
    k_digits<<<(unsigned)((n + 255) / 256), 256, 0, stream>>>(d_scalars, sbytes, n, g, keys0, vals0); launches++;
    kb = cub::DoubleBuffer<uint32_t>(keys0, keys1); vb = cub::DoubleBuffer<uint32_t>(vals0, vals1);
    cudaError_t e = cub::DeviceRadixSort::SortPairs(base + o_tmp, sort_tmp, kb, vb, (uint64_t)total, 0, end_bit, stream);
    if (e != cudaSuccess) return (int)e;
    launches += 2 + (end_bit + 7) / 8;
    uint32_t T = MSM_SEG;
    const bool adaptive = g_msm_tuning[5] >= 0 && g_msm_tuning[7] <= 0;
    if (adaptive) { const uint64_t avg = nbuckets ? total / nbuckets : 0; while (T < 256 && avg > 2ull * T) T <<= 1; }
    if (g_msm_tuning[7] > 0) T = (uint32_t)g_msm_tuning[7];
    static int sm_count = 0;
    if (!sm_count) { int dev = 0; cudaGetDevice(&dev); if (cudaDeviceGetAttribute(&sm_count, cudaDevAttrMultiProcessorCount, dev) != cudaSuccess || sm_count <= 0) sm_count = 148; }
    const uint64_t wave = adaptive ? (uint64_t)sm_count * 4 * MSM_ACC_THREADS : 0;
    const uint32_t seg_lo = adaptive ? (T == (uint32_t)MSM_SEG ? 16u : T / 2) : T;
    k_count_valid<<<1, 1, 0, stream>>>(kb.Current(), total, counts, T, seg_lo, wave); launches++;
    prof.end();
    out->seg_lo = seg_lo;
    out->keys = kb.Current(); out->vals = vb.Current(); out->counts = counts; out->n = n; out->total = total; out->g = g;
    if (stats) stats->launches += launches;
    return (int)cudaGetLastError();
}

}
```

Before: 45.20.

## Rework batch-affine pair-reduction into prefix/invert/apply stages, default-on for G2

Replaces the per-bucket-offset pair reduction rounds with a three-kernel scheme per round. A prefix kernel builds products of denominators, a kernel inverts them with a warp-level batched inversion, and an apply kernel writes the affine pair sums, with a CUB scan compacting output positions. Round counts and slot counts now come from an estimated density, and the path is enabled by default for BN254 G2 when bucket density is high. The aim is to cut the expensive XYZZ bucket accumulation by pre-halving the points with cheap affine adds. The cost is extra launches and scratch memory, and the path may lose when density is marginal.

```diff
diff --git a/profiles/ab_batch_affine.py b/profiles/ab_batch_affine.py
--- /dev/null
+++ b/profiles/ab_batch_affine.py
@@ -0,0 +1,57 @@
+import argparse
+import json
+import os
+import subprocess
+import sys
+
+sys.path.insert(0, os.path.dirname(os.path.dirname(os.path.abspath(__file__))))
+import numpy as np
+
+import snarkjs_b200
+from snarkjs_b200 import synth
+
+ap = argparse.ArgumentParser()
+ap.add_argument("--reps", type=int, default=7)
+ap.add_argument("--log2n", type=int, default=20)
+ap.add_argument("--rounds", default="1,2,3,4,5")
+ap.add_argument("--out", default=None)
+args = ap.parse_args()
+
+c = snarkjs_b200.getCurveFromName("bn128")
+lib, h = c.lib, c.handle
+n = 1 << args.log2n
+rng = np.random.default_rng(1)
+sc = rng.integers(0, 256, size=n * 32, dtype=np.uint8)
+sc.reshape(n, 32)[:, 31] &= 0x1f
+settings = [("xyzz", 1, 0), ("default", 0, 0)] + [(f"R={k}", 2, int(k)) for k in args.rounds.split(",")]
+try:
+    gpu = subprocess.run(["nvidia-smi", "--query-gpu=name,power.limit", "--format=csv,noheader"], capture_output=True, text=True).stdout.strip()
+except OSError:
+    gpu = "unknown"
+lines = []
+for grp in (1, 2):
+    G = c.G1 if grp == 1 else c.G2
+    hb = G.registerBases(synth.gen_points(c, grp, 7, n))
+    dev = {s[0]: [] for s in settings}; acc = {s[0]: [] for s in settings}
+    ref = None
+    for rep in range(args.reps + 1):
+        for name, mode, cap in settings:
+            lib.sb_set_tuning(4, mode); lib.sb_set_tuning(5, cap)
+            out = G.multiExpRegistered(hb, sc).tobytes()
+            if ref is None:
+                ref = out
+            assert out == ref, f"G{grp} {name}: result differs"
+            if rep:
+                dev[name].append(c.last_ms(2)); acc[name].append(lib.sb_last_stat(h, grp - 1))
+    lib.sb_set_tuning(4, 0); lib.sb_set_tuning(5, 0)
+    for name, _, _ in settings:
+        d, a = np.array(dev[name]), np.array(acc[name])
+        rec = {"group": f"G{grp}", "setting": name, "n": n, "reps": args.reps, "gpu": gpu,
+               "msm_device_ms": float(np.median(d)), "msm_device_ms_min": float(d.min()), "msm_device_ms_max": float(d.max()),
+               "accumulate_ms": float(np.median(a)), "accumulate_ms_min": float(a.min()), "accumulate_ms_max": float(a.max())}
+        lines.append(rec)
+        print(json.dumps(rec), flush=True)
+if args.out:
+    with open(args.out, "w") as f:
+        f.write("".join(json.dumps(r) + "\n" for r in lines))
+c.terminate()
diff --git a/profiles/tune_pair.py b/profiles/tune_pair.py
--- a/profiles/tune_pair.py
+++ /dev/null
@@ -1,22 +0,0 @@
-import os, sys
-sys.path.insert(0, os.path.dirname(os.path.dirname(os.path.abspath(__file__))))
-import numpy as np
-import snarkjs_b200
-from snarkjs_b200 import synth
-c = snarkjs_b200.getCurveFromName("bn128")
-lib, h = c.lib, c.handle
-n = 1 << 20
-rng = np.random.default_rng(1)
-sc = rng.integers(0, 256, size=n * 32, dtype=np.uint8); sc.reshape(n, 32)[:, 31] &= 0x1f
-for grp in (1, 2):
-    bases = synth.gen_points(c, grp, 7, n)
-    G = c.G1 if grp == 1 else c.G2
-    hb = G.registerBases(bases)
-    ref = None
-    for off, rounds in ((1, 0), (0, 1), (0, 2), (0, 3), (0, 4), (0, 6)):
-        lib.sb_set_tuning(4, off); lib.sb_set_tuning(5, rounds)
-        for _ in range(3):
-            out = G.multiExpRegistered(hb, sc)
-        if ref is None: ref = out.tobytes()
-        assert out.tobytes() == ref
-        print(f"G{grp} pairing {'off' if off else 'R<=%d' % rounds}: pre-stage {lib.sb_last_stat(h, grp - 1):.3f} ms, msm device total {c.last_ms(2):.3f} ms")
diff --git a/snarkjs_b200/csrc/api.cu b/snarkjs_b200/csrc/api.cu
--- a/snarkjs_b200/csrc/api.cu
+++ b/snarkjs_b200/csrc/api.cu
@@ -318,6 +318,8 @@
         const int g = c->stats.tag[i / 2];
         if (g == PROF_ACC_G1) { c->stat[0] += ms; c->stat[2] += 1; c->stat[9] += ms; }
         else if (g == PROF_ACC_G2) { c->stat[1] += ms; c->stat[3] += 1; c->stat[10] += ms; }
+        else if (g == PROF_PAIR_G1) { c->stat[0] += ms; c->stat[9] += ms; }
+        else if (g == PROF_PAIR_G2) { c->stat[1] += ms; c->stat[10] += ms; }
         else if (g == PROF_SORT) c->stat[8] += ms;
         else if (g >= PROF_FOLD && g <= PROF_JOIN) c->stat[11 + (g - PROF_FOLD)] += ms;
     }
diff --git a/snarkjs_b200/csrc/msm.cuh b/snarkjs_b200/csrc/msm.cuh
--- a/snarkjs_b200/csrc/msm.cuh
+++ b/snarkjs_b200/csrc/msm.cuh
@@ -1,4 +1,5 @@
 #pragma once
+#include <algorithm>
 #include <cuda_runtime.h>
 #include "ec.cuh"
 #include "msm_geom.h"
@@ -10,6 +11,21 @@
 static constexpr int MSM_RED_CHUNK = 16;
 static constexpr uint32_t MSM_INVALID_KEY = 0xffffffffu;
 static constexpr int MSM_COUNTS_SEG = 8;
+
+__device__ inline void msm_fill_counts(uint64_t* out, uint64_t M, uint32_t T, uint32_t seg_lo, uint64_t wave) {
+    out[0] = M;
+    uint64_t seg = T;
+    if (wave) {
+        const uint64_t k = (M + wave * T - 1) / (wave * T);
+        if (k && k <= 3) seg = (M + k * wave - 1) / (k * wave);
+        if (seg < seg_lo) seg = seg_lo;
+        if (seg > T) seg = T;
+    }
+    out[MSM_COUNTS_SEG] = seg;
+    uint64_t m = (M + seg - 1) / seg;
+    out[1] = m;
+    for (int l = 2; l < 8; l++) { m = (m <= MSM_SEG) ? 0 : (m + MSM_SEG - 1) / MSM_SEG; out[l] = m; }
+}
 
 
 __host__ inline MsmGeom msm_choose(uint64_t n, uint32_t scalar_bytes, int fr_bits, bool precomp) {
@@ -515,7 +531,8 @@
     int launches = 0;
     cudaEvent_t* ev = nullptr; int nev = 0; int used = 0; int tag[128] = {0}; int cur_tag = 0;
 };
-enum { PROF_ACC_G1 = 1, PROF_ACC_G2 = 2, PROF_SORT = 3, PROF_FOLD = 4, PROF_REDUCE = 5, PROF_QAP = 6, PROF_NTT = 7, PROF_JOIN = 8 };
+enum { PROF_ACC_G1 = 1, PROF_ACC_G2 = 2, PROF_SORT = 3, PROF_FOLD = 4, PROF_REDUCE = 5, PROF_QAP = 6, PROF_NTT = 7, PROF_JOIN = 8,
+       PROF_PAIR_G1 = 9, PROF_PAIR_G2 = 10 };
 struct ProfScope {
     MsmLaunchStats* s; cudaStream_t st; int idx = -1;
     ProfScope(MsmLaunchStats* s_, int tag, cudaStream_t st_) : s(s_), st(st_) {
@@ -531,80 +548,100 @@
     uint32_t seg_lo = MSM_SEG;
 };
 
-size_t msm_pair_scan_tmp_bytes(uint32_t NB);
-int msm_pair_offsets(const uint32_t* keys, const uint64_t* counts, uint32_t NB, uint32_t* off, cudaStream_t stream);
-int msm_pair_next_offsets(const uint32_t* off_in, uint32_t NB, uint32_t* sizes, uint32_t* off_out, void* tmp, size_t tmp_bytes, cudaStream_t stream);
-int msm_pair_counts(const uint32_t* off, uint32_t NB, uint64_t* counts, cudaStream_t stream);
+int msm_sm_count();
+size_t msm_pair_scan_tmp_bytes(uint64_t items);
+int msm_pair_scan(const uint32_t* counts, uint32_t* pos, uint64_t items, void* tmp, size_t tmp_bytes, cudaStream_t stream);
 
 int msm_sort_entries(const uint8_t* d_scalars, uint32_t sbytes, uint64_t n, MsmGeom g, MsmScratch& scratch,
                      cudaStream_t stream, MsmSorted* out, MsmLaunchStats* stats);
 
+struct MsmBucketLayout { uint64_t heads0 = 0; size_t headsA = 0, hkA = 0, headsB = 0, hkB = 0, hkM = 0, part = 0, bytes = 0; };
+template <class F>
+MsmBucketLayout msm_bucket_layout(const MsmGeom& g, uint64_t total, uint32_t seg_lo) {
+    auto al = [](size_t x) { return (x + 255) & ~(size_t)255; };
+    MsmBucketLayout L;
+    L.heads0 = (total + seg_lo - 1) / seg_lo;
+    const uint64_t heads1 = (L.heads0 + MSM_SEG - 1) / MSM_SEG;
+    L.headsA = al((uint64_t)g.windows() * g.B * sizeof(XYZZ<F>)); L.hkA = L.headsA + al(L.heads0 * sizeof(XYZZ<F>));
+    L.headsB = L.hkA + al(L.heads0 * 4); L.hkB = L.headsB + al(heads1 * sizeof(XYZZ<F>));
+    L.hkM = L.hkB + al(heads1 * 4);
+    L.part = L.hkM + al(L.heads0 * 4);
+    L.bytes = L.part + al(msm_reduce_scratch_elems(g) * sizeof(XYZZ<F>));
+    return L;
+}
+
 template <class F>
 int msm_buckets_impl(const Affine<F>* d_bases, const MsmSorted& s, MsmScratch& scratch, size_t scratch_off, cudaStream_t stream,
                      XYZZ<F>* d_wsum, MsmLaunchStats* stats, cudaStream_t tail_stream, cudaEvent_t ev_acc);
+
+static constexpr double PAIR_STOP_DENSITY = 8.0;
+static constexpr double PAIR_FORCED_STOP_DENSITY = 2.0;
+static constexpr uint64_t PAIR_MIN_ENTRIES = 1ull << 20;
+static constexpr int PAIR_MAX_ROUNDS = 8;
+static constexpr uint64_t PAIR_MAX_SLOTS = 64;
+template <class F> struct PairDefault { static constexpr bool value = false; };
+template <> struct PairDefault<Fp2<BnFq>> { static constexpr bool value = true; };
 
 template <class F>
 int msm_buckets(const Affine<F>* d_bases, const MsmSorted& s, MsmScratch& scratch, cudaStream_t stream,
                 XYZZ<F>* d_wsum, MsmLaunchStats* stats, cudaStream_t tail_stream = nullptr, cudaEvent_t ev_acc = nullptr) {
     const MsmGeom g = s.g;
-    const uint64_t NBl = (uint64_t)g.windows() * g.B;
-    const double avg = NBl ? (double)s.total / (double)NBl : 0.0;
-    if (g_msm_tuning[4] != 2 || avg < 4.0 || NBl >= (1ull << 31) || s.total >= (1ull << 31))
+    const uint64_t NB = (uint64_t)g.windows() * g.B;
+    const int mode = g_msm_tuning[4];
+    const double stop = mode == 2 ? PAIR_FORCED_STOP_DENSITY : PAIR_STOP_DENSITY;
+    const bool dense = NB && (double)s.total > PAIR_STOP_DENSITY * (double)NB;
+    const bool use = mode == 2 || (mode == 0 && PairDefault<F>::value && s.total >= PAIR_MIN_ENTRIES && dense);
+    if (!use || s.total == 0 || NB >= (1ull << 31) || s.total >= (1ull << 31))
         return msm_buckets_impl<F>(d_bases, s, scratch, 0, stream, d_wsum, stats, tail_stream, ev_acc);
-    const uint32_t NB = (uint32_t)NBl;
-    int R = 1; while ((1u << R) < 2.0 * avg && R < 8) R++;
+    uint64_t ub[PAIR_MAX_ROUNDS + 1], Jub[PAIR_MAX_ROUNDS], T[PAIR_MAX_ROUNDS]; uint32_t K[PAIR_MAX_ROUNDS];
+    const uint64_t target = (uint64_t)msm_sm_count() * 2048;
+    double est = (double)s.total;
+    int R = 0; ub[0] = s.total;
+    while (R < PAIR_MAX_ROUNDS && (est > stop * (double)NB || (R == 0 && mode == 2))) {
+        Jub[R] = (ub[R] + 1) / 2;
+        uint64_t k = (Jub[R] + target) / target; if (k > PAIR_MAX_SLOTS) k = PAIR_MAX_SLOTS;
+        K[R] = (uint32_t)k;
+        T[R] = ((Jub[R] + k) / k + PAIR_THREADS - 1) / PAIR_THREADS * PAIR_THREADS;
+        ub[R + 1] = std::min(ub[R], (ub[R] + 1) / 2 + std::min(NB, ub[R]));
+        est = est / 2 + (double)NB / 2;
+        R++;
+    }
     if (g_msm_tuning[5] > 0 && g_msm_tuning[5] < R) R = g_msm_tuning[5];
+    uint64_t Tmax = 0; for (int r = 0; r < R; r++) Tmax = std::max(Tmax, T[r]);
     auto al = [](size_t x) { return (x + 255) & ~(size_t)255; };
-    const uint64_t ub1 = (s.total + NB + 1) / 2;
-    const size_t scan_tmp = msm_pair_scan_tmp_bytes(NB);
-    const uint64_t pthreads = ((ub1 + PAIR_K - 1) / PAIR_K + PAIR_THREADS - 1) / PAIR_THREADS * PAIR_THREADS;
-    size_t o_offA = 0, o_offB = o_offA + al((size_t)(NB + 1) * 4), o_sizes = o_offB + al((size_t)(NB + 1) * 4);
-    size_t o_tmp = o_sizes + al((size_t)(NB + 1) * 4), o_cnt = o_tmp + al(scan_tmp);
-    size_t o_PA = o_cnt + 256, o_PB = o_PA + al(ub1 * sizeof(Affine<F>)), o_KA = o_PB + al(ub1 * sizeof(Affine<F>));
-    size_t o_KB = o_KA + al(ub1 * 4), o_L = o_KB + al(ub1 * 4), o_rest = o_L + al(pthreads * PAIR_K * sizeof(F));
-    uint64_t ub = s.total; for (int r = 0; r < R; r++) ub = (ub + NB + 1) / 2;
-    MsmSorted s2 = s; s2.total = ub; s2.vals = nullptr; s2.seg_lo = MSM_SEG;
-    {
-        const uint64_t heads0 = (ub + MSM_SEG - 1) / MSM_SEG, heads1 = (heads0 + MSM_SEG - 1) / MSM_SEG;
-        const uint32_t L = g.B < (uint32_t)MSM_RED_CHUNK ? g.B : MSM_RED_CHUNK;
-        const uint32_t ctas_per_window = (g.B / L + 127) / 128;
-        size_t need = al(NBl * sizeof(XYZZ<F>)) + al(heads0 * sizeof(XYZZ<F>)) + al(heads0 * 4) + al(heads1 * sizeof(XYZZ<F>)) + al(heads1 * 4) +
-                      al(heads0 * 4) + al(msm_reduce_scratch_elems(g) * sizeof(XYZZ<F>));
-        need += need / 8 + (1u << 20);
-        if (!scratch.get(o_rest + need)) return (int)cudaErrorMemoryAllocation;
-    }
+    const size_t scan_tmp = msm_pair_scan_tmp_bytes(Jub[0] + 1);
+    const size_t o_outc = al((size_t)R * 128), o_pos = o_outc + al((Jub[0] + 1) * 4), o_tmp = o_pos + al((Jub[0] + 1) * 4);
+    const size_t o_pre = o_tmp + al(scan_tmp), o_tp = o_pre + al(Jub[0] * sizeof(F)), o_inv = o_tp + al(Tmax * sizeof(F));
+    const size_t o_P0 = o_inv + al(Tmax * sizeof(F)), o_P1 = o_P0 + al(ub[1] * sizeof(Affine<F>)), o_K0 = o_P1 + al(ub[1] * sizeof(Affine<F>));
+    const size_t o_K1 = o_K0 + al(ub[1] * 4), o_rest = o_K1 + al(ub[1] * 4);
+    MsmSorted s2 = s; s2.total = ub[R]; s2.vals = nullptr; s2.seg_lo = MSM_SEG / 2;
+    if (!scratch.get(o_rest + msm_bucket_layout<F>(g, s2.total, s2.seg_lo).bytes)) return (int)cudaErrorMemoryAllocation;
     uint8_t* base = (uint8_t*)scratch.p;
-    uint32_t* offA = (uint32_t*)(base + o_offA); uint32_t* offB = (uint32_t*)(base + o_offB); uint32_t* sizes = (uint32_t*)(base + o_sizes);
-    uint64_t* counts2 = (uint64_t*)(base + o_cnt);
-    Affine<F>* P[2] = {(Affine<F>*)(base + o_PA), (Affine<F>*)(base + o_PB)};
-    uint32_t* K[2] = {(uint32_t*)(base + o_KA), (uint32_t*)(base + o_KB)};
-    F* Ls = (F*)(base + o_L);
+    uint32_t* outc = (uint32_t*)(base + o_outc); uint32_t* pos = (uint32_t*)(base + o_pos);
+    F* pre = (F*)(base + o_pre); F* tprod = (F*)(base + o_tp); F* invp = (F*)(base + o_inv);
+    Affine<F>* P[2] = {(Affine<F>*)(base + o_P0), (Affine<F>*)(base + o_P1)};
+    uint32_t* Kb[2] = {(uint32_t*)(base + o_K0), (uint32_t*)(base + o_K1)};
+    const uint64_t wave = (uint64_t)msm_sm_count() * 4 * MSM_ACC_THREADS;
     int launches = 0;
-    ProfScope prof(stats, stats ? stats->cur_tag : 0, stream);
-    int rc = msm_pair_offsets(s.keys, s.counts, NB, offA, stream); launches++;
-    if (rc) return rc;
-    const Affine<F>* src = d_bases; uint32_t* in = offA; uint32_t* out = offB;
-    uint64_t ubr = s.total;
+    ProfScope prof(stats, stats && stats->cur_tag == PROF_ACC_G1 ? PROF_PAIR_G1 : PROF_PAIR_G2, stream);
+    const Affine<F>* src = d_bases; const uint32_t* keys = s.keys; const uint64_t* cin = s.counts;
     for (int r = 0; r < R; r++) {
-        rc = msm_pair_next_offsets(in, NB, sizes, out, base + o_tmp, scan_tmp, stream); launches += 3;
+        uint64_t* cout = (uint64_t*)(base + (size_t)r * 128);
+        const unsigned grid = (unsigned)(T[r] / PAIR_THREADS), igrid = (unsigned)((T[r] / PAIR_LANE_PRODUCTS + 127) / 128);
+        if (r == 0) k_pair_prefix<F, true><<<grid, PAIR_THREADS, 0, stream>>>(src, s.vals, keys, cin, Jub[r], K[r], pre, tprod, outc);
+        else k_pair_prefix<F, false><<<grid, PAIR_THREADS, 0, stream>>>(src, nullptr, keys, cin, Jub[r], K[r], pre, tprod, outc);
+        int rc = msm_pair_scan(outc, pos, Jub[r] + 1, base + o_tmp, scan_tmp, stream);
         if (rc) return rc;
-        ubr = (ubr + NB + 1) / 2;
-        const unsigned grid = (unsigned)(((ubr + PAIR_K - 1) / PAIR_K + PAIR_THREADS - 1) / PAIR_THREADS);
-        if (r == 0) k_pair_round<F, true><<<grid, PAIR_THREADS, 0, stream>>>(src, s.vals, in, out, NB, P[0], K[0], Ls);
-        else k_pair_round<F, false><<<grid, PAIR_THREADS, 0, stream>>>(src, nullptr, in, out, NB, P[r & 1], K[r & 1], Ls);
-        launches++;
-        src = P[r & 1]; s2.keys = K[r & 1];
-        uint32_t* t = in; in = out; out = t;
-    }
-    rc = msm_pair_counts(in, NB, counts2, stream); launches++;
-    if (rc) return rc;
-    s2.counts = counts2;
+        k_pair_invert<F><<<igrid, 128, 0, stream>>>(tprod, T[r], invp, pos, Jub[r], cout, wave);
+        if (r == 0) k_pair_apply<F, true><<<grid, PAIR_THREADS, 0, stream>>>(src, s.vals, keys, cin, K[r], pre, invp, pos, P[0], Kb[0]);
+        else k_pair_apply<F, false><<<grid, PAIR_THREADS, 0, stream>>>(src, nullptr, keys, cin, K[r], pre, invp, pos, P[r & 1], Kb[r & 1]);
+        launches += 5;
+        src = P[r & 1]; keys = Kb[r & 1]; cin = cout;
+    }
     prof.end();
     if (stats) stats->launches += launches;
-    cudaEvent_t* sev = stats ? stats->ev : nullptr; if (stats) stats->ev = nullptr;
-    rc = msm_buckets_impl<F>(src, s2, scratch, o_rest, stream, d_wsum, stats, tail_stream, ev_acc);
-    if (stats) stats->ev = sev;
-    return rc;
+    s2.keys = keys; s2.counts = cin;
+    return msm_buckets_impl<F>(src, s2, scratch, o_rest, stream, d_wsum, stats, tail_stream, ev_acc);
 }
 
 template <class F>
@@ -613,27 +650,20 @@
     const MsmGeom g = s.g;
     const uint32_t NW = g.windows();
     const uint64_t nbuckets = (uint64_t)NW * g.B;
-    const uint64_t heads0 = (s.total + s.seg_lo - 1) / s.seg_lo;
-    const uint64_t heads1 = (heads0 + MSM_SEG - 1) / MSM_SEG;
     const uint32_t L = g.B < (uint32_t)MSM_RED_CHUNK ? g.B : MSM_RED_CHUNK;
     const uint32_t chunks = g.B / L;
     const uint32_t red_threads = 128;
     const uint32_t ctas_per_window = (chunks + red_threads - 1) / red_threads;
-    auto al = [](size_t x) { return (x + 255) & ~(size_t)255; };
-    size_t o_buckets = 0;
-    size_t o_headsA = o_buckets + al(nbuckets * sizeof(XYZZ<F>)), o_hkA = o_headsA + al(heads0 * sizeof(XYZZ<F>));
-    size_t o_headsB = o_hkA + al(heads0 * 4), o_hkB = o_headsB + al(heads1 * sizeof(XYZZ<F>));
-    size_t o_hkM = o_hkB + al(heads1 * 4);
-    size_t o_part = o_hkM + al(heads0 * 4);
-    size_t bytes = o_part + al(msm_reduce_scratch_elems(g) * sizeof(XYZZ<F>));
-    uint8_t* base = (uint8_t*)scratch.get(scratch_off + bytes);
+    const MsmBucketLayout lay = msm_bucket_layout<F>(g, s.total, s.seg_lo);
+    const uint64_t heads0 = lay.heads0;
+    uint8_t* base = (uint8_t*)scratch.get(scratch_off + lay.bytes);
     if (!base) return (int)cudaErrorMemoryAllocation;
     base += scratch_off;
-    XYZZ<F>* buckets = (XYZZ<F>*)(base + o_buckets);
-    XYZZ<F>* headsA = (XYZZ<F>*)(base + o_headsA); uint32_t* hkA = (uint32_t*)(base + o_hkA);
-    XYZZ<F>* headsB = (XYZZ<F>*)(base + o_headsB); uint32_t* hkB = (uint32_t*)(base + o_hkB);
-    XYZZ<F>* partials = (XYZZ<F>*)(base + o_part);
-    uint32_t* hkM = (uint32_t*)(base + o_hkM);
+    XYZZ<F>* buckets = (XYZZ<F>*)base;
+    XYZZ<F>* headsA = (XYZZ<F>*)(base + lay.headsA); uint32_t* hkA = (uint32_t*)(base + lay.hkA);
+    XYZZ<F>* headsB = (XYZZ<F>*)(base + lay.headsB); uint32_t* hkB = (uint32_t*)(base + lay.hkB);
+    XYZZ<F>* partials = (XYZZ<F>*)(base + lay.part);
+    uint32_t* hkM = (uint32_t*)(base + lay.hkM);
     int launches = 0;
     cudaMemsetAsync(buckets, 0, nbuckets * sizeof(XYZZ<F>), stream);
     if (heads0) {
diff --git a/snarkjs_b200/csrc/msm_pair.cuh b/snarkjs_b200/csrc/msm_pair.cuh
--- a/snarkjs_b200/csrc/msm_pair.cuh
+++ b/snarkjs_b200/csrc/msm_pair.cuh
@@ -1,141 +1,158 @@
 #pragma once
-#include <cuda_runtime.h>
 #include "ec.cuh"
-#include "msm_geom.h"
 
 namespace sb {
 
-static constexpr int PAIR_K = 32;
-static constexpr int PAIR_THREADS = 128;
+enum { PAIR_COPY = 0, PAIR_ADD = 1, PAIR_DBL = 2, PAIR_INF = 3, PAIR_TAKE2 = 4 };
 
-__global__ void k_bucket_offsets(const uint32_t* __restrict__ keys, const uint64_t* __restrict__ counts, uint32_t NB, uint32_t* __restrict__ off);
-__global__ void k_halve_sizes(const uint32_t* __restrict__ off, uint32_t NB, uint32_t* __restrict__ sizes);
-__global__ void k_counts_from_offsets(const uint32_t* __restrict__ off, uint32_t NB, uint64_t* __restrict__ counts);
-
-template <class F> struct PairInv;
-template <class P> struct PairInv<Fp<P>> { __device__ static Fp<P> inv(const Fp<P>& a) { return Fp<P>::inv_binary(a); } };
-template <class P> struct PairInv<Fp2<P>> { __device__ static Fp2<P> inv(const Fp2<P>& a) { return Fp2<P>::inv(a); } };
-
-template <class F> __device__ __forceinline__ F pair_load_x(const Affine<F>* p) { return load_vec(&p->x); }
-template <class F> __device__ __forceinline__ F pair_load_y(const Affine<F>* p) { return load_vec(&p->y); }
-
-enum { PAIR_COPY = 0, PAIR_ADD = 1, PAIR_DBL = 2, PAIR_INF = 3, PAIR_TAKE2 = 4, PAIR_NONE = 5 };
-
-template <class F, bool FIRST>
-__device__ __forceinline__ const Affine<F>* pair_src(const Affine<F>* __restrict__ pts, const uint32_t* __restrict__ vals, uint32_t s, bool& neg) {
-    if (FIRST) { uint32_t v = vals[s]; neg = (v >> 31) != 0; return pts + (v & 0x7fffffffu); }
-    neg = false; return pts + s;
-}
-
-template <class F, bool FIRST>
-__device__ __forceinline__ int pair_classify(const Affine<F>* __restrict__ pts, const uint32_t* __restrict__ vals, uint32_t s0, bool has_pair, F& den) {
+template <class F> SB_HD int pair_kind(const F& x1, const F& y1, const F& x2, const F& y2, F& den) {
     den = F::one();
-    if (!has_pair) return PAIR_COPY;
-    bool n1, n2;
-    const Affine<F>* p1 = pair_src<F, FIRST>(pts, vals, s0, n1);
-    const Affine<F>* p2 = pair_src<F, FIRST>(pts, vals, s0 + 1, n2);
-    F x1 = pair_load_x<F>(p1), x2 = pair_load_x<F>(p2);
-    if (x1.is_zero()) { if (pair_load_y<F>(p1).is_zero()) return PAIR_TAKE2; }
-    if (x2.is_zero()) { if (pair_load_y<F>(p2).is_zero()) return PAIR_COPY; }
+    if (x1.is_zero() & y1.is_zero()) return PAIR_TAKE2;
+    if (x2.is_zero() & y2.is_zero()) return PAIR_COPY;
     if (x1 == x2) {
-        F y1 = F::cneg(pair_load_y<F>(p1), n1), y2 = F::cneg(pair_load_y<F>(p2), n2);
-        if (y1 == y2 && !y1.is_zero()) { den = F::dbl(y1); return PAIR_DBL; }
+        if ((y1 == y2) & !y1.is_zero()) { den = F::dbl(y1); return PAIR_DBL; }
         return PAIR_INF;
     }
     den = F::sub(x2, x1);
     return PAIR_ADD;
 }
+template <class F> SB_HD Affine<F> pair_sum(int kind, const F& x1, const F& y1, const F& x2, const F& y2, const F& inv) {
+    Affine<F> r;
+    if (kind == PAIR_ADD || kind == PAIR_DBL) {
+        F lam;
+        if (kind == PAIR_ADD) lam = F::mul_i(F::sub(y2, y1), inv);
+        else { F xx = F::sqr_i(x1); lam = F::mul_i(F::add(F::dbl(xx), xx), inv); }
+        r.x = F::sub(F::sub(F::sqr_i(lam), x1), x2);
+        r.y = F::sub(F::mul_i(lam, F::sub(x1, r.x)), y1);
+    } else if (kind == PAIR_INF) { r.x = F::zero(); r.y = F::zero(); }
+    else if (kind == PAIR_TAKE2) { r.x = x2; r.y = y2; }
+    else { r.x = x1; r.y = y1; }
+    return r;
+}
+
+#ifdef __CUDACC__
+static constexpr int PAIR_THREADS = 128;
+static constexpr int PAIR_LANE_PRODUCTS = PAIR_THREADS / 32;
+
+template <class F, bool FIRST>
+__device__ __forceinline__ uint64_t pair_index(const uint32_t* __restrict__ vals, uint64_t s, bool& neg) {
+    if (FIRST) { const uint32_t v = vals[s]; neg = (v >> 31) != 0; return v & 0x7fffffffu; }
+    neg = false; return s;
+}
+template <class F, bool FIRST>
+__device__ __forceinline__ void pair_load(const Affine<F>* __restrict__ pts, const uint32_t* __restrict__ vals, uint64_t s, F& x, F& y) {
+    bool neg; const uint64_t i = pair_index<F, FIRST>(vals, s, neg);
+    load_affine<F>(pts + i, 0, x, y);
+    y = F::cneg(y, neg);
+}
+
+template <class F, int MODE> __device__ __forceinline__ F shfl_f(const F& v, int d) {
+    constexpr int NW = sizeof(F) / 4;
+    union U { F f; uint32_t w[NW]; __device__ U() {} };
+    U a, r; a.f = v;
+#pragma unroll
+    for (int k = 0; k < NW; k++)
+        r.w[k] = MODE == 0 ? __shfl_up_sync(0xffffffffu, a.w[k], d) : MODE == 1 ? __shfl_down_sync(0xffffffffu, a.w[k], d) : __shfl_sync(0xffffffffu, a.w[k], d);
+    return r.f;
+}
 
 template <class F, bool FIRST>
 __global__ void __launch_bounds__(PAIR_THREADS)
-k_pair_round(const Affine<F>* __restrict__ src, const uint32_t* __restrict__ vals, const uint32_t* __restrict__ off_in,
-             const uint32_t* __restrict__ off_out, uint32_t NB, Affine<F>* __restrict__ dst, uint32_t* __restrict__ dst_keys,
-             F* __restrict__ scratch) {
-    __shared__ F sP[PAIR_THREADS];
-    __shared__ F sS[PAIR_THREADS];
-    __shared__ F sInv;
-    const uint32_t total_out = off_out[NB];
-    const uint32_t tid = threadIdx.x;
-    const uint64_t gt = blockIdx.x * (uint64_t)blockDim.x + tid;
-    const uint64_t nthreads = gridDim.x * (uint64_t)blockDim.x;
-    const uint64_t o0 = gt * PAIR_K;
-    if ((uint64_t)blockIdx.x * blockDim.x * PAIR_K >= total_out) return;
-    uint32_t b0 = 0;
-    if (o0 < total_out) {
-        uint32_t lo = 0, hi = NB;
-        while (hi - lo > 1) { uint32_t mid = (lo + hi) >> 1; if (off_out[mid] <= o0) lo = mid; else hi = mid; }
-        b0 = lo;
+k_pair_prefix(const Affine<F>* __restrict__ src, const uint32_t* __restrict__ vals, const uint32_t* __restrict__ keys,
+              const uint64_t* __restrict__ counts, uint64_t Jub, uint32_t K, F* __restrict__ pre, F* __restrict__ tprod,
+              uint32_t* __restrict__ outc) {
+    const uint64_t n = counts[0], J = (n + 1) / 2;
+    const uint64_t T = (uint64_t)gridDim.x * blockDim.x, t = blockIdx.x * (uint64_t)blockDim.x + threadIdx.x;
+    F acc = F::one();
+    for (uint32_t k = 0; k < K; k++) {
+        const uint64_t j = k * T + t;
+        if (j > Jub) break;
+        uint32_t c = 0;
+        if (j < J) {
+            const uint64_t s = 2 * j;
+            c = 1;
+            if (s + 1 < n) {
+                if (keys[s] != keys[s + 1]) c = 2;
+                else {
+                    bool n1, n2;
+                    const uint64_t i1 = pair_index<F, FIRST>(vals, s, n1), i2 = pair_index<F, FIRST>(vals, s + 1, n2);
+                    const F x1 = load_vec(&src[i1].x), x2 = load_vec(&src[i2].x);
+                    F den; int kind = PAIR_ADD;
+                    if (x1.is_zero() | x2.is_zero() | (x1 == x2))
+                        kind = pair_kind<F>(x1, F::cneg(load_vec(&src[i1].y), n1), x2, F::cneg(load_vec(&src[i2].y), n2), den);
+                    else den = F::sub(x2, x1);
+                    if (kind == PAIR_ADD || kind == PAIR_DBL) { store_vec(pre + j, acc); acc = F::mul_i(acc, den); }
+                }
+            }
+        }
+        outc[j] = c;
     }
-    F pre = F::one();
-    {
-        uint32_t b = b0;
-        for (int k = 0; k < PAIR_K; k++) {
-            uint64_t o = o0 + k;
-            F den = F::one();
-            if (o < total_out) {
-                while (off_out[b + 1] <= o) b++;
-                uint32_t j = (uint32_t)o - off_out[b], s0 = off_in[b] + 2 * j, m = off_in[b + 1] - off_in[b];
-                pair_classify<F, FIRST>(src, vals, s0, 2 * j + 1 < m, den);
-            }
-            store_vec(scratch + (uint64_t)k * nthreads + gt, pre);
-            pre = F::mul(pre, den);
-        }
+    store_vec(tprod + t, acc);
+}
+
+template <class F>
+__global__ void __launch_bounds__(128)
+k_pair_invert(const F* __restrict__ tprod, uint64_t T, F* __restrict__ invp, const uint32_t* __restrict__ pos, uint64_t Jub,
+              uint64_t* __restrict__ counts_out, uint64_t wave) {
+    const uint64_t gid = blockIdx.x * (uint64_t)blockDim.x + threadIdx.x;
+    if (gid == 0) msm_fill_counts(counts_out, pos[Jub], MSM_SEG, MSM_SEG / 2, wave);
+    const uint32_t lane = threadIdx.x & 31;
+    const uint64_t w = gid >> 5;
+    if (w * PAIR_THREADS >= T) return;
+    const F* p = tprod + w * PAIR_THREADS + lane * PAIR_LANE_PRODUCTS;
+    F q[PAIR_LANE_PRODUCTS], l = F::one();
+#pragma unroll
+    for (int i = 0; i < PAIR_LANE_PRODUCTS; i++) { q[i] = l; l = F::mul_i(l, load_vec(p + i)); }
+    F inc = l, suf = l;
+#pragma unroll 1
+    for (int d = 1; d < 32; d <<= 1) {
+        F a = shfl_f<F, 0>(inc, d), b = shfl_f<F, 1>(suf, d);
+        if (lane >= (uint32_t)d) inc = F::mul_i(a, inc);
+        if (lane + d < 32) suf = F::mul_i(suf, b);
     }
-    store_vec(&sP[tid], pre); store_vec(&sS[tid], pre);
-    __syncthreads();
-    for (int d = 1; d < PAIR_THREADS; d <<= 1) {
-        F a, c; bool ha = tid >= (uint32_t)d, hc = tid + d < PAIR_THREADS;
-        if (ha) a = F::mul(load_vec(&sP[tid - d]), load_vec(&sP[tid]));
-        if (hc) c = F::mul(load_vec(&sS[tid]), load_vec(&sS[tid + d]));
-        __syncthreads();
-        if (ha) store_vec(&sP[tid], a);
-        if (hc) store_vec(&sS[tid], c);
-        __syncthreads();
-    }
-    if (tid < 32) {
-        F t = PairInv<F>::inv(load_vec(&sP[PAIR_THREADS - 1]));
-        if (tid == 0) store_vec(&sInv, t);
-    }
-    __syncthreads();
-    F running = load_vec(&sInv);
-    if (tid > 0) running = F::mul(running, load_vec(&sP[tid - 1]));
-    if (tid + 1 < PAIR_THREADS) running = F::mul(running, load_vec(&sS[tid + 1]));
-    if (o0 >= total_out) return;
-    uint32_t b = b0;
-    {
-        uint64_t olast = o0 + PAIR_K - 1; if (olast >= total_out) olast = total_out - 1;
-        while (off_out[b + 1] <= olast) b++;
-    }
-    for (int k = PAIR_K - 1; k >= 0; k--) {
-        uint64_t o = o0 + k;
-        if (o >= total_out) continue;
-        while (off_out[b] > o) b--;
-        uint32_t j = (uint32_t)o - off_out[b], s0 = off_in[b] + 2 * j, m = off_in[b + 1] - off_in[b];
-        F den;
-        int kind = pair_classify<F, FIRST>(src, vals, s0, 2 * j + 1 < m, den);
-        Affine<F> out;
-        bool n1, n2;
-        if (kind == PAIR_ADD || kind == PAIR_DBL) {
-            F inv = F::mul(running, load_vec(scratch + (uint64_t)k * nthreads + gt));
-            running = F::mul(running, den);
-            const Affine<F>* p1 = pair_src<F, FIRST>(src, vals, s0, n1);
-            const Affine<F>* p2 = pair_src<F, FIRST>(src, vals, s0 + 1, n2);
-            F x1 = pair_load_x<F>(p1), y1 = F::cneg(pair_load_y<F>(p1), n1);
-            F x2 = pair_load_x<F>(p2);
-            F lam;
-            if (kind == PAIR_ADD) { F y2 = F::cneg(pair_load_y<F>(p2), n2); lam = F::mul(F::sub(y2, y1), inv); }
-            else { F xx = F::sqr(x1); lam = F::mul(F::add(F::dbl(xx), xx), inv); }
-            F x3 = F::sub(F::sub(F::sqr(lam), x1), x2);
-            out.x = x3; out.y = F::sub(F::mul(lam, F::sub(x1, x3)), y1);
-        } else if (kind == PAIR_INF) {
-            out.x = F::zero(); out.y = F::zero();
-        } else {
-            const Affine<F>* p = pair_src<F, FIRST>(src, vals, kind == PAIR_TAKE2 ? s0 + 1 : s0, n1);
-            out.x = pair_load_x<F>(p); out.y = F::cneg(pair_load_y<F>(p), n1);
-        }
-        store_vec(dst + o, out);
-        dst_keys[o] = b;
+    const F total = shfl_f<F, 2>(inc, 31);
+    F before = shfl_f<F, 0>(inc, 1), after = shfl_f<F, 1>(suf, 1);
+    if (lane == 0) before = F::one();
+    if (lane == 31) after = F::one();
+    F r = F::mul_i(F::mul_i(PairInvF(total), before), after);
+    F* o = invp + w * PAIR_THREADS + lane * PAIR_LANE_PRODUCTS;
+#pragma unroll
+    for (int i = PAIR_LANE_PRODUCTS - 1; i >= 0; i--) {
+        store_vec(o + i, F::mul_i(r, q[i]));
+        if (i) r = F::mul_i(r, load_vec(p + i));
     }
 }
 
+template <class F, bool FIRST>
+__global__ void __launch_bounds__(PAIR_THREADS)
+k_pair_apply(const Affine<F>* __restrict__ src, const uint32_t* __restrict__ vals, const uint32_t* __restrict__ keys,
+             const uint64_t* __restrict__ counts, uint32_t K, const F* __restrict__ pre, const F* __restrict__ invp,
+             const uint32_t* __restrict__ pos, Affine<F>* __restrict__ dst, uint32_t* __restrict__ dst_keys) {
+    const uint64_t n = counts[0], J = (n + 1) / 2;
+    const uint64_t T = (uint64_t)gridDim.x * blockDim.x, t = blockIdx.x * (uint64_t)blockDim.x + threadIdx.x;
+    F running = load_vec(invp + t);
+    for (int k = (int)K - 1; k >= 0; k--) {
+        const uint64_t j = (uint64_t)k * T + t;
+        if (j >= J) continue;
+        const uint64_t s = 2 * j;
+        const uint32_t o = pos[j], key = keys[s];
+        Affine<F> a, b;
+        pair_load<F, FIRST>(src, vals, s, a.x, a.y);
+        if (s + 1 < n) {
+            pair_load<F, FIRST>(src, vals, s + 1, b.x, b.y);
+            const uint32_t key2 = keys[s + 1];
+            if (key2 != key) { store_vec(dst + o + 1, b); dst_keys[o + 1] = key2; }
+            else {
+                F den;
+                const int kind = pair_kind<F>(a.x, a.y, b.x, b.y, den);
+                F inv = den;
+                if (kind == PAIR_ADD || kind == PAIR_DBL) { inv = F::mul_i(running, load_vec(pre + j)); running = F::mul_i(running, den); }
+                a = pair_sum<F>(kind, a.x, a.y, b.x, b.y, inv);
+            }
+        }
+        store_vec(dst + o, a); dst_keys[o] = key;
+    }
 }
+#endif
+
+}
diff --git a/snarkjs_b200/csrc/msm_sort.cu b/snarkjs_b200/csrc/msm_sort.cu
--- a/snarkjs_b200/csrc/msm_sort.cu
+++ b/snarkjs_b200/csrc/msm_sort.cu
@@ -42,59 +42,23 @@
     if (blockIdx.x | threadIdx.x) return;
     uint64_t lo = 0, hi = total;
     while (lo < hi) { uint64_t mid = (lo + hi) >> 1; if (keys[mid] == MSM_INVALID_KEY) hi = mid; else lo = mid + 1; }
-    out[0] = lo;
-    uint64_t seg = T;
-    if (wave) {
-        const uint64_t k = (lo + wave * T - 1) / (wave * T);
-        if (k && k <= 3) seg = (lo + k * wave - 1) / (k * wave);
-        if (seg < seg_lo) seg = seg_lo;
-        if (seg > T) seg = T;
-    }
-    out[MSM_COUNTS_SEG] = seg;
-    uint64_t m = (lo + seg - 1) / seg;
-    out[1] = m;
-    for (int l = 2; l < 8; l++) { m = (m <= MSM_SEG) ? 0 : (m + MSM_SEG - 1) / MSM_SEG; out[l] = m; }
+    msm_fill_counts(out, lo, T, seg_lo, wave);
 }
 
+int msm_sm_count() {
+    static int sm_count = 0;
+    if (!sm_count) { int dev = 0; cudaGetDevice(&dev); if (cudaDeviceGetAttribute(&sm_count, cudaDevAttrMultiProcessorCount, dev) != cudaSuccess || sm_count <= 0) sm_count = 148; }
+    return sm_count;
+}
 
-__global__ void k_bucket_offsets(const uint32_t* __restrict__ keys, const uint64_t* __restrict__ counts, uint32_t NB, uint32_t* __restrict__ off) {
-    uint32_t b = blockIdx.x * blockDim.x + threadIdx.x;
-    if (b > NB) return;
-    const uint64_t M = counts[0];
-    uint64_t lo = 0, hi = M;
-    while (lo < hi) { uint64_t mid = (lo + hi) >> 1; if (keys[mid] < b) lo = mid + 1; else hi = mid; }
-    off[b] = (uint32_t)lo;
-}
-__global__ void k_halve_sizes(const uint32_t* __restrict__ off, uint32_t NB, uint32_t* __restrict__ sizes) {
-    uint32_t b = blockIdx.x * blockDim.x + threadIdx.x;
-    if (b > NB) return;
-    sizes[b] = b < NB ? (off[b + 1] - off[b] + 1) / 2 : 0;
-}
-__global__ void k_counts_from_offsets(const uint32_t* __restrict__ off, uint32_t NB, uint64_t* __restrict__ counts) {
-    if (blockIdx.x | threadIdx.x) return;
-    uint64_t m = off[NB];
-    counts[0] = m;
-    m = (m + MSM_SEG - 1) / MSM_SEG; counts[1] = m;
-    for (int l = 2; l < 8; l++) { m = (m <= (uint64_t)MSM_SEG) ? 0 : (m + MSM_SEG - 1) / MSM_SEG; counts[l] = m; }
-    counts[MSM_COUNTS_SEG] = MSM_SEG;
-}
-size_t msm_pair_scan_tmp_bytes(uint32_t NB) {
+size_t msm_pair_scan_tmp_bytes(uint64_t items) {
     size_t bytes = 0;
-    cub::DeviceScan::ExclusiveSum(nullptr, bytes, (const uint32_t*)nullptr, (uint32_t*)nullptr, (int)(NB + 1));
+    cub::DeviceScan::ExclusiveSum(nullptr, bytes, (const uint32_t*)nullptr, (uint32_t*)nullptr, (int)items);
     return bytes;
 }
-int msm_pair_offsets(const uint32_t* keys, const uint64_t* counts, uint32_t NB, uint32_t* off, cudaStream_t stream) {
-    k_bucket_offsets<<<(NB + 1 + 255) / 256, 256, 0, stream>>>(keys, counts, NB, off);
-    return (int)cudaGetLastError();
-}
-int msm_pair_next_offsets(const uint32_t* off_in, uint32_t NB, uint32_t* sizes, uint32_t* off_out, void* tmp, size_t tmp_bytes, cudaStream_t stream) {
-    k_halve_sizes<<<(NB + 1 + 255) / 256, 256, 0, stream>>>(off_in, NB, sizes);
-    cudaError_t e = cub::DeviceScan::ExclusiveSum(tmp, tmp_bytes, sizes, off_out, (int)(NB + 1), stream);
+int msm_pair_scan(const uint32_t* counts, uint32_t* pos, uint64_t items, void* tmp, size_t tmp_bytes, cudaStream_t stream) {
+    cudaError_t e = cub::DeviceScan::ExclusiveSum(tmp, tmp_bytes, counts, pos, (int)items, stream);
     return (int)(e != cudaSuccess ? e : cudaGetLastError());
-}
-int msm_pair_counts(const uint32_t* off, uint32_t NB, uint64_t* counts, cudaStream_t stream) {
-    k_counts_from_offsets<<<1, 1, 0, stream>>>(off, NB, counts);
-    return (int)cudaGetLastError();
 }
 
 int msm_sort_entries(const uint8_t* d_scalars, uint32_t sbytes, uint64_t n, MsmGeom g, MsmScratch& scratch,
@@ -126,9 +90,7 @@
     const bool adaptive = g_msm_tuning[5] >= 0 && g_msm_tuning[7] <= 0;
     if (adaptive) { const uint64_t avg = nbuckets ? total / nbuckets : 0; while (T < 256 && avg > 2ull * T) T <<= 1; }
     if (g_msm_tuning[7] > 0) T = (uint32_t)g_msm_tuning[7];
-    static int sm_count = 0;
-    if (!sm_count) { int dev = 0; cudaGetDevice(&dev); if (cudaDeviceGetAttribute(&sm_count, cudaDevAttrMultiProcessorCount, dev) != cudaSuccess || sm_count <= 0) sm_count = 148; }
-    const uint64_t wave = adaptive ? (uint64_t)sm_count * 4 * MSM_ACC_THREADS : 0;
+    const uint64_t wave = adaptive ? (uint64_t)msm_sm_count() * 4 * MSM_ACC_THREADS : 0;
     const uint32_t seg_lo = adaptive ? (T == (uint32_t)MSM_SEG ? 16u : T / 2) : T;
     k_count_valid<<<1, 1, 0, stream>>>(kb.Current(), total, counts, T, seg_lo, wave); launches++;
     prof.end();
```

Result: faster. 47.94, median of 6 (+6.1%).
